# YuliangXiu/ICON

Hardware: AMD Instinct MI355X
Metric: query-points/sec at 256^3 grid (higher is better)
Workload: dtype f32 via 3x f16 split MFMA (22-bit operands, f32 accumulate)

## Files before the change

### icon_amd/_lib.py

```python
from __future__ import annotations

import ctypes as C
import os
import subprocess

_HERE = os.path.dirname(os.path.abspath(__file__))
LIB_PATH = os.environ.get("ICON_AMD_LIB") or os.path.join(_HERE, "libicon_amd.so")
CSRC = os.path.join(_HERE, "csrc")

PRIOR = {"icon": 0, "pamir": 1, "pifu": 2}
CMAP = {"reference": 0, "local": 1}
SEARCH = {"bvh": 0, "brute": 1}
PRECISION = {"f32": 0, "f16x3": 1}

SYMBOLS = [
    "icon_last_error", "icon_version", "icon_device_count",
    "icon_mesh_create", "icon_mesh_destroy", "icon_mesh_vertex_normals", "icon_mesh_stats",
    "icon_mesh_arena_bytes", "icon_mesh_create_arena", "icon_mesh_status", "icon_debug_set_mesh_build", "icon_debug_mesh_layout", "icon_debug_host_mesh_build",
    "icon_sdf_query",
    "icon_feat_create", "icon_feat_destroy", "icon_feat_set_smpl_feats",
    "icon_mlp_create", "icon_mlp_destroy", "icon_mlp_forward", "icon_mlp_set_last_op",
    "icon_work_create", "icon_work_destroy", "icon_work_profile", "icon_work_stage_ms", "icon_work_profile_detail", "icon_work_profile_workgroups", "icon_work_set_steal", "icon_work_set_reserve_cus",
    "icon_query_points", "icon_query_points_dcalib", "icon_query_rows", "icon_grid_rows",
    "icon_volume_any_above", "icon_adaptive_eval", "icon_adaptive_counts", "icon_adaptive_reruns", "icon_grid_eval_slab", "icon_grid_slab_features", "icon_grid_slab_finish", "icon_grid_slab_features_msg",
    "icon_grid_slab_finish_gathered", "icon_debug_set_shell_skip", "icon_debug_set_option", "icon_work_status", "icon_sdf_query_ties", "icon_work_set_tie_rule",
    "icon_export_mesh", "icon_mc_count", "icon_mc_emit", "icon_mc_count_range", "icon_mc_emit_keyed", "icon_debug_traversal_stats", "icon_debug_set_unfused",
    "icon_visibility", "icon_mesh_components", "icon_clean_mesh", "icon_semantic_voxelize",
    "icon_mesh_batch_create", "icon_mesh_batch_destroy", "icon_mesh_batch_status", "icon_feat_create_batch", "icon_query_points_batch",
    "icon_feat_batch_set_volume", "icon_semantic_voxelize_batch",
]

_lib = None


class IconAmdError(RuntimeError):
    pass


def build(force: bool = False) -> str:
    args = ["make", "-j8", "-C", CSRC] + (["-B"] if force else [])
    proc = subprocess.run(args, stdout=subprocess.PIPE, stderr=subprocess.STDOUT, text=True)
    if proc.returncode != 0:
        raise IconAmdError("building libicon_amd.so failed:\n" + proc.stdout[-4000:])
    return LIB_PATH


def lib():
    global _lib
    if _lib is not None:
        return _lib
    if not os.path.exists(LIB_PATH):
        raise IconAmdError(f"{LIB_PATH} not found - run `python -c 'import __graft_entry__ as g; g.build()'` "
                           "or `make -C icon_amd/csrc` (needs hipcc); there is no CPU fallback")
    import torch
    L = C.CDLL(LIB_PATH)
    L.icon_last_error.restype = C.c_char_p
    for name in SYMBOLS:
        if name != "icon_last_error":
            getattr(L, name).restype = C.c_int
    _lib = L
    return L


def check(rc: int, what: str = "") -> None:
    if rc != 0:
        msg = lib().icon_last_error().decode("utf-8", "replace")
        raise IconAmdError(f"{what or 'icon_amd'} failed (code {rc}): {msg}")


def device_count() -> int:
    return int(lib().icon_device_count())


def require_device() -> None:
    if device_count() < 1:
        raise IconAmdError("icon_amd needs a HIP device (MI355X); none is visible and there is no CPU fallback")


def ptr(t) -> C.c_void_p:
    if t is None:
        return C.c_void_p(0)
    if hasattr(t, "data_ptr"):
# ... 4 lines not shown
```

### icon_amd/csrc/adaptive.hip

```cpp
#pragma clang fp contract(off)

#include "geom_device.h"

#include <algorithm>
#include <vector>

constexpr int kAdMaxLevels = 8;

struct icon_adaptive {
    int n_levels = 0;
    int res[kAdMaxLevels] = {0};
    float *occ[kAdMaxLevels] = {nullptr};
    uint8_t *P = nullptr;
    uint8_t *M1 = nullptr;
    uint8_t *D[kAdMaxLevels] = {nullptr};
    int32_t *map = nullptr;
    float *pts = nullptr;
    int32_t *blk_count = nullptr;
    int32_t *blk_list = nullptr;
    int *h_counters = nullptr;
    int *h_counters_dev = nullptr;
    int *counters = nullptr;
    int *counters_base = nullptr;
    int cur_set = 0;
// ... 410 lines not shown
        bk.P = examined ? a->P : nullptr;
        bk.D = (examined && l >= 2) ? a->D[l - 1] : nullptr;
        bk.C = a->M1;
        bk.Dprev = l >= 3 ? a->D[l - 2] : nullptr;
        bk.rpp = l >= 2 ? resolutions[l - 2] : 0;
        bk.balance = balance;
        bk.any_pos = l == 1 ? a->counters + 9 : nullptr;
        bk.zero = examined ? a->blk_count : nullptr;
        bk.n_zero = examined ? nb_l + nsup_l : 0;
        if (l == n_levels - 1) {
            bk.zero_set = other_set;
            a->other_clean = true;
            if (n_levels >= 3 && h_counts) { bk.mirror_src = a->counters; bk.mirror_dst = a->h_counters_dev; mirrored = true; }
        }
        const int64_t book = (bk.P || bk.any_pos) ? (nsrc + 255) / 256 : 0;
        const int64_t grid_up = std::max<int64_t>(std::max<int64_t>(((int64_t)r * r + 3) / 4, book), (bk.n_zero + 255) / 256);
        hipLaunchKernelGGL(k_ad_up, dim3((unsigned)grid_up), dim3(256), 0, st, a->occ[l - 1], rp, a->occ[l], r,
                           examined ? a->counters + 8 : (int *)nullptr, bk);
        if (!examined) break;
        const int rad = l == 1 ? 4 : (l == 2 ? 3 : 1);
        const unsigned nt = (unsigned)((r + kMaskTX - 1) / kMaskTX) * (unsigned)((r + kMaskTY - 1) / kMaskTY) * (unsigned)((r + kMaskTZ - 1) / kMaskTZ);
        uint8_t *C = a->M1;
        const bool icon_prior = prior_type == ICON_PRIOR_ICON;
        const int P = lattice_packet();
        const int shift = P == 4 ? 2 : 1;
        const int nbk = (r + P - 1) / P;
        hipLaunchKernelGGL(k_ad_mask, dim3(nt), dim3(256), 0, st, a->P, rp, (const uint8_t *)(l >= 2 ? a->D[l - 1] : nullptr), C, r, rad,
                           shift, nbk, icon_prior ? a->blk_list : (int32_t *)nullptr, a->counters + 8, a->blk_count, a->blk_count + nb_l);
        hipLaunchKernelGGL(k_ad_scatter, dim3(nbv), dim3(256), 0, st, C, r, a->blk_count, a->blk_count + nb_l, nsup_l, a->map, a->pts, a->counters + l);
        ICON_HIP(hipGetLastError());
        debug_sync("adaptive: upsample + boundary + dilate + compact", st);
        if ((rc = ensure_work_points(work, std::max<int64_t>(n, 1)))) return rc;
        work->q_map = a->map; work->q_n_dev = a->counters + l;
        Calib cal;
        memcpy(cal.m, ident, sizeof(ident)); cal.d = nullptr;
        const bool icon = icon_prior;
        const bool needs_list = icon && cmap_mode == ICON_CMAP_REFERENCE && (feat->dev.smpl_mask & kSmplCmap);
        if (icon) {
            if (mesh->F > kNearLoSlots && work->cap_points_hi < work->cap_points) {
                (void)hipFree(work->d_near_hi); work->d_near_hi = nullptr; work->cap_points_hi = 0;
                ICON_HIP(hipMalloc((void **)&work->d_near_hi, (size_t)work->cap_points));
                work->cap_points_hi = work->cap_points;
            }
            NearRef raw = work_near(work, mesh);
            raw.map = nullptr;
            int n_cu = 0;
            if ((rc = device_cu_count(&n_cu))) return rc;
            const int share_env = share_waves_override();
            const int by_level = r <= 65 ? kShareWavesFew : (r <= 129 ? kShareWavesMany : 4);
            const int nw = (share_env == 1 || share_env == 4 || share_env == 8 || share_env == 16) ? share_env : by_level;
            ShareDbg dbg{};
            if ((rc = work_share_dbg(work, &dbg))) return rc;
#define ICON_AD_NEAREST(PP, NW) hipLaunchKernelGGL((k_ad_nearest<PP, NW>), dim3((unsigned)(n_cu * 32 / (NW == 1 ? 4 : NW))), dim3(NW == 1 ? 256 : NW * 64), 0, st, \
                                                   mesh->dev, r, nbk, a->blk_list, a->counters + 8, C, raw, sdf_clip, dbg)
            if (P == 4 && nw == 16) ICON_AD_NEAREST(4, 16);
            else if (P == 4 && nw == 8) ICON_AD_NEAREST(4, 8);
            else if (P == 4 && nw == 4) ICON_AD_NEAREST(4, 4);
            else if (P == 4) ICON_AD_NEAREST(4, 1);
            else if (nw == 16) ICON_AD_NEAREST(2, 16);
            else if (nw == 8) ICON_AD_NEAREST(2, 8);
            else ICON_AD_NEAREST(2, 1);
#undef ICON_AD_NEAREST
            ICON_HIP(hipGetLastError());
            debug_sync("adaptive: k_ad_nearest", st);
            if ((rc = launch_sign(mesh, cal, r, 0, a->pts, n, sdf_clip, work, false, st))) return rc;
            if (needs_list && (rc = outlier_list_dev(work, a->counters + l, n, st))) return rc;
        }
        FusedSigns fs{};
        fs.mode = needs_list ? kSignSelf : kSignNone;
        fs.list = work->d_signs; fs.k_dev = work->d_total;
        LatticeMap L{};
        rc = launch_fused_f16x3(mesh, feat, mlp, prior_type, cal, L, 0, 0, a->pts, n, sdf_clip, cmap_mode == ICON_CMAP_LOCAL ? 1 : 0, work, fs,
                                a->occ[l], false, st);
        work->q_map = nullptr; work->q_n_dev = nullptr;
        if (rc) return rc;
        debug_sync("adaptive: sign + list + fused", st);
        ICON_HIP(hipGetLastError());
    }
    ICON_HIP(hipGetLastError());
    if (!a->other_clean) {
        ICON_HIP(hipMemsetAsync(other_set, 0, 16 * sizeof(int), st));
        a->other_clean = true;
    }
    if (h_counts) {
        int *host = a->h_counters;
        if (!mirrored) ICON_HIP(hipMemcpyAsync(host, a->counters, 16 * sizeof(int), hipMemcpyDeviceToHost, st));
        ICON_HIP(hipStreamSynchronize(st));
        for (int l = 0; l < n_levels; ++l) h_counts[l] = host[l];
        h_counts[0] = (int64_t)r0 * r0 * r0;
        h_counts[n_levels] = host[9];
        if ((rc = work_check_err(work))) return rc;
    }
    return ICON_OK;
}

extern "C" int icon_adaptive_counts(icon_work_t *work, int n_levels, int64_t *h_counts, void *stream)
{
    ICON_ARG(work && work->ad && h_counts && n_levels == work->ad->n_levels, "icon_adaptive_counts: no matching icon_adaptive_eval on this workspace");
    int *host = work->ad->h_counters;
    ICON_HIP(hipMemcpyAsync(host, work->ad->counters, 16 * sizeof(int), hipMemcpyDeviceToHost, (hipStream_t)stream));
    ICON_HIP(hipStreamSynchronize((hipStream_t)stream));
    for (int l = 0; l < n_levels; ++l) h_counts[l] = host[l];
    h_counts[0] = (int64_t)work->ad->res[0] * work->ad->res[0] * work->ad->res[0];
    h_counts[n_levels] = host[9];
    return work_check_err(work);
}
```

### icon_amd/csrc/batch_query.hip

```cpp
#pragma clang fp contract(off)

#include "batch_device.h"

#include <algorithm>

namespace icon {

constexpr int kBatchBlock = 256;
constexpr int kBatchChecked = 0x100;

__global__ void k_pack_planes_batch(const float *__restrict__ src, int C, int H, int W, int n_select, int csel, int cpad, int64_t stride,
                                    float *__restrict__ dst)
{
    const int64_t n = (int64_t)n_select * H * W * cpad;
    const float *s = src + (int64_t)blockIdx.z * C * H * W;
    float *d = dst + (int64_t)blockIdx.z * stride;
    for (int64_t i = (int64_t)blockIdx.x * blockDim.x + threadIdx.x; i < n; i += (int64_t)gridDim.x * blockDim.x) {
        const int c = (int)(i % cpad);
        const int64_t pix = (i / cpad) % ((int64_t)H * W);
        const int sel = (int)(i / ((int64_t)cpad * H * W));
        d[i] = (c < csel) ? s[((int64_t)(sel * csel + c)) * H * W + pix] : 0.0f;
    }
}

// ... 130 lines not shown
        if (f.smpl_mask & kSmplNorm) { row[hh] = o.nrm.x; row[hh + 1] = o.nrm.y; row[hh + 2] = o.nrm.z; }
    } else {
        gather_planes_dyn(f, 0, p.x, p.y, g);
        const int h = f.csel;
        for (int k = 0; k < h; ++k) row[k] = g[k];
        if (PRIOR == ICON_PRIOR_PAMIR) {
            float v[8];
            if (f.vpad == 8) gather_volume<2>(f, p.x, p.y, p.z, v); else gather_volume<1>(f, p.x, p.y, p.z, v);
            for (int k = 0; k < f.Cv; ++k) row[h + k] = v[k];
        } else {
            row[h] = p.z;
        }
    }
    row[kCodeSlot] = __int_as_float((int)code);
    if (live) { store_row(X, i, row); code8[i] = (uint8_t)code; }
}

}

using namespace icon;

extern "C" int icon_mesh_batch_destroy(icon_mesh_batch_t *mb)
{
    if (!mb) return ICON_OK;
    if (mb->done) (void)hipEventDestroy(mb->done);
    (void)hipFree(mb->d_table);
    if (mb->h_table) (void)hipHostFree(mb->h_table);
    if (mb->h_status) (void)hipHostFree(mb->h_status);
    delete mb;
    return ICON_OK;
}

extern "C" int icon_mesh_batch_create(const icon_mesh_t *const *meshes, int B, void *stream, icon_mesh_batch_t **out)
{
    ICON_ARG(out != nullptr, "icon_mesh_batch_create: out is null");
    *out = nullptr;
    ICON_ARG(meshes != nullptr && B >= 1, "icon_mesh_batch_create: no meshes");
    for (int b = 0; b < B; ++b) {
        ICON_ARG(meshes[b] != nullptr, "icon_mesh_batch_create: a mesh is null");
        ICON_ARG(meshes[b]->V == meshes[0]->V && meshes[b]->F == meshes[0]->F,
                 "icon_mesh_batch_create: the subjects' vertex / face counts differ (check_sign takes subject 0's faces for every subject, "
                 "lib/dataset/mesh_util.py:393)");
    }
    hipStream_t st = (hipStream_t)stream;
    icon_mesh_batch *mb = new icon_mesh_batch();
    mb->B = B; mb->V = meshes[0]->V; mb->F = meshes[0]->F;
    for (int b = 0; b < B; ++b) { mb->subj.push_back(meshes[b]); mb->depth_bound = std::max(mb->depth_bound, meshes[b]->depth_bound); }
    const size_t tab_bytes = (size_t)B * sizeof(MeshDev), bytes = tab_bytes + sizeof(int);
    hipError_t e = hipMalloc((void **)&mb->d_table, bytes);
    if (e == hipSuccess) e = hipHostMalloc((void **)&mb->h_table, bytes, hipHostMallocPortable);
    if (e == hipSuccess) e = hipHostMalloc((void **)&mb->h_status, sizeof(int), hipHostMallocPortable);
    if (e == hipSuccess) e = hipEventCreateWithFlags(&mb->done, hipEventDisableTiming);
    if (e != hipSuccess) { icon_mesh_batch_destroy(mb); return fail(ICON_ERR_HIP, std::string("icon_mesh_batch_create: ") + hipGetErrorString(e)); }
    for (int b = 0; b < B; ++b) mb->h_table[b] = meshes[b]->dev;
    int *h_word = reinterpret_cast<int *>(reinterpret_cast<char *>(mb->h_table) + tab_bytes);
    int *d_word = reinterpret_cast<int *>(reinterpret_cast<char *>(mb->d_table) + tab_bytes);
    *h_word = kBatchChecked;
    *(volatile int *)mb->h_status = 0;
    e = hipMemcpyAsync(mb->d_table, mb->h_table, bytes, hipMemcpyHostToDevice, st);
    if (e == hipSuccess && B > 1 && mb->F > 0) {
        const int64_t n = (int64_t)(B - 1) * mb->F;
        hipLaunchKernelGGL(k_faces_match, dim3((unsigned)((n + kBatchBlock - 1) / kBatchBlock)), dim3(kBatchBlock), 0, st, mb->d_table, B, mb->F, d_word);
        e = hipGetLastError();
    }
    if (e == hipSuccess) e = hipMemcpyAsync(mb->h_status, d_word, sizeof(int), hipMemcpyDeviceToHost, st);
    if (e == hipSuccess) e = hipEventRecord(mb->done, st);
    if (e != hipSuccess) { icon_mesh_batch_destroy(mb); return fail(ICON_ERR_HIP, std::string("icon_mesh_batch_create: ") + hipGetErrorString(e)); }
    *out = mb;
    return ICON_OK;
}

extern "C" int icon_mesh_batch_status(const icon_mesh_batch_t *mb, int wait, int *bits)
{
    ICON_ARG(mb != nullptr, "icon_mesh_batch_status: batch is null");
    if (wait) ICON_HIP(hipEventSynchronize(mb->done));
    const int st = *reinterpret_cast<const volatile int *>(mb->h_status);
    if (!(st & kBatchChecked)) { if (bits) *bits = -1; return ICON_OK; }
    if (bits) *bits = st & ~kBatchChecked;
    if (st & ICON_MESH_BATCH_FACES_DIFFER)
        return fail(ICON_ERR_ARG, "icon_mesh_batch: the subjects' faces differ - check_sign(verts, faces[0], points) (lib/dataset/mesh_util.py:393) "
                                  "tests every subject against subject 0's faces; bind subjects of one topology");
    return ICON_OK;
}

extern "C" int icon_feat_create_batch(const float *d_planes, int B, int C, int H, int W, int n_select, void *stream, icon_feat_t **out)
{
    ICON_ARG(out != nullptr, "icon_feat_create_batch: out is null");
    *out = nullptr;
    ICON_ARG(d_planes && B >= 1 && C > 0 && H > 1 && W > 1, "icon_feat_create_batch: bad planes");
    ICON_ARG(n_select == 1 || n_select == 2, "icon_feat_create_batch: n_select must be 1 or 2");
    ICON_ARG(C % n_select == 0, "icon_feat_create_batch: C not divisible by n_select");
    ICON_ARG(B <= 65535, "icon_feat_create_batch: more than 65,535 subjects");
    const int csel = C / n_select;
    const int cpad = (csel + 3) & ~3;
    if (cpad > 16) return fail(ICON_ERR_UNSUPPORTED, "icon_feat_create_batch: more than 16 channels per tap");
    hipStream_t st = (hipStream_t)stream;
    icon_feat *f = new icon_feat();
    const int64_t stride = (int64_t)n_select * H * W * cpad;
    hipError_t e = hipMalloc((void **)&f->d_planes, (size_t)stride * B * sizeof(float));
    if (e != hipSuccess) { delete f; return fail(ICON_ERR_HIP, std::string("hipMalloc planes: ") + hipGetErrorString(e)); }
    hipLaunchKernelGGL(k_pack_planes_batch, dim3((unsigned)std::max(1, 1024 / B), 1, (unsigned)B), dim3(256), 0, st, d_planes, C, H, W, n_select,
                       csel, cpad, stride, f->d_planes);
    FeatDev &d = f->dev;
    d.planes = f->d_planes; d.C = C; d.H = H; d.W = W; d.n_select = n_select; d.csel = csel; d.cpad = cpad;
    d.smpl_mask = kSmplCmap | kSmplNorm;
    d.vol = nullptr; d.Cv = 0; d.Dv = d.Hv = d.Wv = 0; d.vpad = 0;
    f->batch = B; f->plane_stride = stride;
// ... 131 lines not shown
```

### icon_amd/csrc/common.h

```cpp
#pragma once
#include <hip/hip_runtime.h>
#include <stdint.h>
#include <functional>
#include <string>
#include <vector>

#include "../../include/icon_amd.h"

namespace icon {
constexpr int kWgRec = 6;
constexpr int kMaxProfGrid = 1024;

void set_error(const std::string &msg);
int fail(int code, const std::string &msg);

#define ICON_HIP(expr)                                                                          \
    do {                                                                                        \
        hipError_t _e = (expr);                                                                 \
        if (_e != hipSuccess)                                                                   \
            return ::icon::fail(ICON_ERR_HIP, std::string(#expr) + ": " + hipGetErrorString(_e)); \
    } while (0)

#define ICON_ARG(cond, msg)                                                  \
    do {                                                                     \
        if (!(cond)) return ::icon::fail(ICON_ERR_ARG, std::string(msg));    \
    } while (0)

struct alignas(64) BvhNode {
    float lo[3][2], hi[3][2];
    int32_t child0, child1;
    int32_t pad[2];
};
static_assert(sizeof(BvhNode) == 64, "BvhNode must be 64 bytes");

struct alignas(16) TriRec {
    float a[3], b[3], c[3];
    int32_t ia, ib, ic;
};
static_assert(sizeof(TriRec) == 48, "TriRec must be 48 bytes");

struct alignas(16) TriAttr {
    float n[3][3];
    float cm[3][3];
    float vis[3];
    int32_t face;
    int32_t pad[2];
};
static_assert(sizeof(TriAttr) == 96, "TriAttr must be 96 bytes");

struct alignas(32) TriPre {
    float a[3], b[3], ab[3], ac[3], bc[3];
    float i00, i11, ibc, a00, a01, a11, inn;
    int32_t face;
    int32_t pad;
};
static_assert(sizeof(TriPre) == 96, "TriPre must be 96 bytes");

struct alignas(32) LeafRec {
    float pair[2][24][2];
};
static_assert(sizeof(LeafRec) == 384, "LeafRec must be 384 bytes");

constexpr int kLeafMax = 4;
constexpr int kShareWavesMany = 8, kShareWavesFew = 16;
inline int share_waves(int64_t packets) { return packets <= 1500 ? kShareWavesFew : (packets <= 8000 ? kShareWavesMany : 1); }
constexpr int kStackDepth = 48;
constexpr int kXRow = 16;
constexpr int kCodeSlot = 15;

constexpr uint32_t kCodeOutlier = 1u;
constexpr uint32_t kCodeSignShift = 1;
constexpr uint32_t kCodeInCube = 8u;
constexpr uint32_t kCodeInside = 16u;

constexpr int kScanBlock = 256;
constexpr int kMaxWorld = 64;

struct MeshDyn {
    int32_t root;
    int32_t gy, gz;
    float bin_y0, bin_z0, bin_y1, bin_z1, bin_inv_y, bin_inv_z;
    float box_lo[3], box_hi[3];
    int32_t n_nodes, n_leaves, depth, bin_entries, max_bin;
    int32_t status;
    int32_t pad[11];
};
static_assert(sizeof(MeshDyn) == 128, "MeshDyn layout");
constexpr int kMeshBadFace = 1;
constexpr int kMeshBadVertex = 2;
constexpr int kMeshBinOverflow = 4;
constexpr int kMeshInternal = 8;
constexpr int kMeshBuilt = 0x100;

struct MeshDev {
    const BvhNode *nodes;
    const TriRec *tris;
    const TriAttr *attr;
    const int32_t *slot2face;
    const int32_t *face2slot;
    const LeafRec *leaves;
    const MeshDyn *dyn;
    int32_t n_tris;
    const int32_t *bin_start;
    const int32_t *bin_slots;
};

struct FeatDev {
    const float *planes;
    const float *vol;
    int32_t C, H, W, n_select, csel, cpad;
    int32_t Cv, Dv, Hv, Wv, vpad;
    int32_t smpl_mask;
};
constexpr int kSmplCmap = 1, kSmplNorm = 2;

struct Calib { float m[12]; const float *d; };

struct Lattice {
    int32_t res, z0, z1;
};

struct LatticeMap {
    int res, z0, nz;
    int tx, ty, tz;
    int remap;
    int off;
    int zs, nzi;
    int sx0, sx1, sy0, sy1;
    int sz0, sz1;
    int trim;
    float trim_need;
    int pk;
};

__device__ __forceinline__ bool not_finite(float y)
{
    uint32_t u = __float_as_uint(y);
    asm volatile("" : "+v"(u));
    return (u & 0x7f800000u) == 0x7f800000u;
}

__device__ __forceinline__ float apply_last_op(float y, int last_op)
{
    return last_op == ICON_LASTOP_SIGMOID ? 1.0f / (1.0f + expf(-y)) : y;
}

struct NearRef { uint16_t *lo; uint8_t *hi; float *d2; const int32_t *map; };

enum { kSignNone = 0, kSignSelf = 1, kSignGlobal = 2, kSignSeg = 3 };
struct FusedSigns {
    int mode;
    const int8_t *list;
    const int64_t *k_dev;
// ... 64 lines not shown
namespace icon {
void parallel_for(int n, const std::function<void(int)> &fn);
void debug_sync(const char *what, hipStream_t st);
struct MeshLayout;
int mesh_host_state_get(MeshDyn **h, hipEvent_t *ev);
void mesh_host_state_put(MeshDyn *h, hipEvent_t ev);
void mesh_bind_arena(icon_mesh *m, const MeshLayout &L);
int mesh_build_device(icon_mesh *m, const float *d_verts, const int64_t *d_faces, const float *d_cmap, const float *d_vis, hipStream_t st);
void adaptive_destroy(icon_adaptive *a);
inline int lattice_packet()
{
    static const int pk_env = getenv("ICON_AMD_PACKET") ? atoi(getenv("ICON_AMD_PACKET")) : 0;
    return pk_env == 2 ? 2 : 4;
}
int outlier_list_dev(icon_work *w, const int *n_dev, int64_t n_max, hipStream_t st);
int ensure_work_points(icon_work *w, int64_t n_points);
struct McDevState;
void mc_destroy(McDevState *s);
struct CleanState;
void clean_destroy(CleanState *s);
int morton_order(icon_work *w, const float *d_points, const float *calib12, const float *d_calib12, int64_t N, hipStream_t st, const int32_t **perm);
int mlp_launch(const icon_mlp *mlp, const float *d_x, int64_t N, float *d_out, int precision, hipStream_t st);
int mlp_launch_ex(const icon_mlp *mlp, const float *d_x, int64_t N, float *d_out, bool mask, hipStream_t st);
int mlp_rescue_rows(const icon_mlp *mlp, const float *d_x, int64_t N, float *d_out, hipStream_t st);
int mlp_flag_reset(const icon_mlp *mlp, hipStream_t st);
int rescue_always();
int mlp_pack_f16x3(icon_mlp *m, const std::vector<std::vector<float>> &W, const std::vector<std::vector<float>> &B, hipStream_t st);
int mlp_launch_f16x3(const icon_mlp *mlp, const float *d_x, int64_t N, float *d_out, bool mask, hipStream_t st);
uint16_t f32_to_f16_rtn(float f);
float f16_to_f32(uint16_t h);
float pick_scale(const std::vector<float> &W);
int launch_sign(const icon_mesh *mesh, const Calib &cal, int res, int z0, const float *d_points, int64_t N, float sdf_clip,
                const icon_work *work, bool lattice, hipStream_t st);
int launch_fused_f16x3(const icon_mesh *mesh, const icon_feat *feat, const icon_mlp *mlp, int prior, const Calib &cal,
                       const LatticeMap &L, int za, int zb, const float *d_points, int64_t N, float sdf_clip, int cmap_local,
                       const icon_work *work, const FusedSigns &fs, float *d_occ, bool lattice, hipStream_t st,
                       const BatchDev *bd = nullptr);
int morton_order_batch(icon_work *w, const float *d_points, const float *d_calibs, int64_t n, int B, hipStream_t st, const int32_t **perm);
int ensure_work_rows(icon_work *w, int64_t n_points, bool need_x);
int outlier_list_counted(icon_work *w, int64_t N, hipStream_t st);
int patch_self_rows(icon_work *w, int64_t N, int cmap_slot, hipStream_t st);
bool fused_path(int precision, int search);
void work_mark(icon_work *w, int k, hipStream_t st);
int device_cu_count(int *n_cu);
int once_per_device(int kernel_id, const std::function<hipError_t()> &set);
struct LatticeFast;
struct ShareDbg {
    int *err;
    int ring, lose, spin_log2;
};
int work_share_dbg(icon_work *w, ShareDbg *out);
int work_check_err(icon_work *w);
int share_waves_override();
}

struct icon_work {
    float *d_x = nullptr;
    int64_t cap_x = 0;
    uint16_t *d_near16 = nullptr;
    uint8_t *d_near_hi = nullptr;
    float *d_near_d2 = nullptr;
    int64_t cap_points_hi = 0;
    uint8_t *d_code8 = nullptr;
    int64_t cap_points = 0;
    uint64_t *d_grp_mask = nullptr;
    int32_t *d_block_counts = nullptr;
    int64_t *d_block_offsets = nullptr;
    int32_t *d_scan_local = nullptr;
    int64_t *d_scan_part = nullptr;
    int64_t cap_blocks = 0;
    int8_t *d_signs = nullptr;
    int64_t cap_signs = 0;
    int64_t *d_total = nullptr;
    int *d_flag = nullptr;
    mutable bool flag_clean = false;
    int64_t *d_seg = nullptr;
    int32_t *d_row_count = nullptr;
    int32_t *d_row_slots = nullptr;
    int64_t cap_rows = 0;
    int *h_err = nullptr;
    icon::LatticeFast *d_lfast = nullptr;
    uint32_t *d_sort_keys = nullptr;
    int32_t *d_sort_idx = nullptr;
    void *d_sort_tmp = nullptr;
    size_t sort_tmp_bytes = 0;
    int64_t cap_sort = 0;
    int slab_res = 0, slab_z0 = 0, slab_z1 = 0, slab_c0 = 0, slab_cmap_slot = 0;
    bool slab_ready = false, slab_needs_patch = false, slab_patched = false;
    int tie_rule = 0, tie_ulps = 0;
    const icon_mesh *q_mesh = nullptr;
    const icon_feat *q_feat = nullptr;
    int q_prior = 0, q_cmap_mode = 0, q_search = 0;
    float q_sdf_clip = 0.f;
    icon::Calib q_cal{};
    icon::LatticeMap q_L{};
    const float *q_points = nullptr;
    int64_t q_N = 0;
    bool q_lattice = false, q_rows_ready = false;
    const int32_t *q_map = nullptr;
    const int *q_n_dev = nullptr;
    int reserve_cus = 0;
    int *h_any = nullptr;
    int *defer_range_flag = nullptr;
    int range_reruns = 0;
    struct icon_adaptive *ad = nullptr;
    icon::McDevState *mc = nullptr;
    icon::CleanState *clean = nullptr;
    bool prof = false;
    hipEvent_t ev[6] = {nullptr, nullptr, nullptr, nullptr, nullptr, nullptr};
    bool ev_search = false;
    unsigned long long *d_clock = nullptr;
    mutable int clock_grid = 0;
    double clock_kernel_ms = 0.0;
    unsigned int *d_steal = nullptr;
    int steal_permille = 150, steal_grp = 2;
    bool ev_valid = false;
};

namespace icon {
constexpr int kNearLoSlots = 32768;
inline NearRef work_near(const icon_work *w, const icon_mesh *mesh)
{
    NearRef r;
    r.lo = w->d_near16; r.d2 = w->d_near_d2;
    r.hi = (mesh && mesh->F > kNearLoSlots) ? w->d_near_hi : nullptr;
    r.map = w->q_map;
    return r;
}
}
```

### icon_amd/csrc/fused_f16x3.hip

```cpp
#pragma clang fp contract(off)

#include "geom_device.h"
#include "batch_device.h"
#include "mlp_f16x3_device.h"
#include "mlp_plain_device.h"

#include <algorithm>
#include <mutex>

namespace icon {

constexpr int kTilePts = kF16Pts;
constexpr int kXsOff = kSideOff + 4352;
constexpr int kFusedLds = kXsOff + kTilePts * kXRow * 4;

struct SignSrc {
    int mode;
    const int8_t *list;
    const int64_t *k_dev;
    int64_t k_host, rank_offset;
    const int8_t *gathered;
    int64_t stride;
    int world, rank;
    const int64_t *seg;
// ... 646 lines not shown
            }
            const float y = mlp_plain_wave(P, s, lane);
            if (lane == b) out[o] = y;
            __builtin_amdgcn_wave_barrier();
        }
    }
}

template <int PRIOR>
__global__ __launch_bounds__(64) void k_rescue_fused_batch(FusedGeom G, float *__restrict__ out, MlpPlain P, const int *flag, int always, BatchDev bd)
{
    __shared__ float s[kPlainLds];
    if (!always && *flag == 0) return;
    const int lane = threadIdx.x;
    int64_t K = 0, rank0 = 0;
    if (PRIOR == ICON_PRIOR_ICON) sign_list_extent(G, K, rank0);
    for (int64_t base = (int64_t)blockIdx.x * 64; base < G.N; base += (int64_t)gridDim.x * 64) {
        const int64_t q = base + lane;
        const int64_t o = q < G.N ? q : 0;
        const float v = q < G.N ? out[o] : 0.0f;
        unsigned long long todo = __ballot(not_finite(v));
        while (todo) {
            const int b = __ffsll((long long)todo) - 1;
            todo &= todo - 1;
            if (lane == b) {
                float row[kXRow];
#pragma unroll
                for (int k = 0; k < kXRow; ++k) row[k] = 0.0f;
                build_row_batch<PRIOR>(G, bd, q, row, K, rank0);
#pragma unroll
                for (int k = 0; k < kXRow; ++k) s[k] = k < P.c0 ? row[k] : 0.0f;
            }
            const float y = mlp_plain_wave(P, s, lane);
            if (lane == b) out[o] = y;
            __builtin_amdgcn_wave_barrier();
        }
    }
}

__global__ void k_seg_offsets(const int8_t *__restrict__ gathered, int64_t stride, int world, int64_t *__restrict__ seg)
{
    if (threadIdx.x != 0 || blockIdx.x != 0) return;
    int64_t a = 0;
    for (int r = 0; r < world; ++r) { seg[r] = a; a += *reinterpret_cast<const int64_t *>(gathered + (int64_t)r * stride); }
    seg[world] = a;
}

int launch_sign(const icon_mesh *mesh, const Calib &cal, int res, int z0, const float *d_points, int64_t N, float sdf_clip,
                const icon_work *work, bool lattice, hipStream_t st)
{
    const int64_t nb = (N + 255) / 256;
    ICON_ARG(nb > 0 && nb < (1ll << 31), "too many workgroups for one launch");
    const float far_box2 = far_box_dist2(sdf_clip);
    if (lattice) hipLaunchKernelGGL(k_sign<true>, dim3((unsigned)nb), dim3(256), 0, st, mesh->dev, cal, res, z0, d_points, N, sdf_clip,
                                    work->d_row_count, work->d_row_slots, work_near(work, mesh), work->d_code8, work->d_block_counts,
                                    (unsigned long long *)work->d_grp_mask, far_box2, (const int *)nullptr, work->d_flag);
    else if (work->q_n_dev || N <= 262144)
        hipLaunchKernelGGL(k_sign_wide, dim3((unsigned)nb), dim3(1024), 0, st, mesh->dev, cal, d_points, N, sdf_clip, work_near(work, mesh), work->d_code8,
                           work->d_block_counts, (unsigned long long *)work->d_grp_mask, far_box2, work->q_n_dev, work->d_flag);
    else hipLaunchKernelGGL(k_sign<false>, dim3((unsigned)nb), dim3(256), 0, st, mesh->dev, cal, res, z0, d_points, N, sdf_clip,
                            (const int32_t *)nullptr, (const int32_t *)nullptr, work_near(work, mesh), work->d_code8, work->d_block_counts,
                            (unsigned long long *)work->d_grp_mask, far_box2, work->q_n_dev, work->d_flag);
    ICON_HIP(hipGetLastError());
    work->flag_clean = work->d_flag != nullptr;
    return ICON_OK;
}

namespace {
constexpr int kMaxDevices = 64, kMaxKernelIds = 16;
std::mutex g_dev_mutex;
int g_n_cu[kMaxDevices];
bool g_attr_set[kMaxKernelIds][kMaxDevices];
}

int device_cu_count(int *n_cu)
{
    int dev = 0;
    ICON_HIP(hipGetDevice(&dev));
    ICON_ARG(dev >= 0 && dev < kMaxDevices, "device index out of range");
    std::lock_guard<std::mutex> lk(g_dev_mutex);
    if (!g_n_cu[dev]) {
        int n = 0;
        ICON_HIP(hipDeviceGetAttribute(&n, hipDeviceAttributeMultiprocessorCount, dev));
        g_n_cu[dev] = n > 0 ? n : 256;
    }
    *n_cu = g_n_cu[dev];
    return ICON_OK;
}

int once_per_device(int kernel_id, const std::function<hipError_t()> &set)
{
    int dev = 0;
    if (hipGetDevice(&dev) != hipSuccess || dev < 0 || dev >= kMaxDevices || kernel_id < 0 || kernel_id >= kMaxKernelIds) {
        const hipError_t e = set();
        return e == hipSuccess ? ICON_OK : fail(ICON_ERR_HIP, std::string("hipFuncSetAttribute: ") + hipGetErrorString(e));
    }
    std::lock_guard<std::mutex> lk(g_dev_mutex);
    if (g_attr_set[kernel_id][dev]) return ICON_OK;
    const hipError_t e = set();
    if (e != hipSuccess) return fail(ICON_ERR_HIP, std::string("hipFuncSetAttribute: ") + hipGetErrorString(e));
    g_attr_set[kernel_id][dev] = true;
    return ICON_OK;
}

int launch_fused_f16x3(const icon_mesh *mesh, const icon_feat *feat, const icon_mlp *mlp, int prior, const Calib &cal,
                       const LatticeMap &L, int za, int zb, const float *d_points, int64_t N, float sdf_clip, int cmap_local,
                       const icon_work *work, const FusedSigns &fs, float *d_occ, bool lattice, hipStream_t st, const BatchDev *bd)
{
    FusedGeom G{};
    if (mesh) G.m = mesh->dev;
    G.f = feat->dev; G.cal = cal; G.pts = d_points; G.sdf_clip = sdf_clip; G.cmap_local = cmap_local;
    if (lattice) {
        const int zs = std::max(za, L.off), ze = std::min(zb, L.res - L.off);
        if (L.off) {
            const int64_t rows = (int64_t)(zb - za) * L.res;
            const int row_wgs = (int)((rows + 255) / 256);
            const int64_t face_rows = 2 * (int64_t)(zb - za) + (int64_t)((za == 0 ? 1 : 0) + (zb == L.res ? 1 : 0)) * L.res;
            if (rows > 0) hipLaunchKernelGGL(k_shell_zero, dim3((unsigned)(row_wgs + (face_rows + 3) / 4)), dim3(256), 0, st, d_occ, L.res, L.z0, za, zb, row_wgs);
        }
        G.res = L.res; G.z0 = L.z0; G.off = L.off; G.nx = L.res - 2 * L.off; G.zs = zs;
        N = (ze > zs) ? (int64_t)(ze - zs) * G.nx * G.nx : 0;
    }
    if (N <= 0) { ICON_HIP(hipGetLastError()); return ICON_OK; }
    ICON_ARG(N < (1ll << 31), "fused: more than 2^31 points in one call");
    G.N = N;
    G.near = work_near(work, mesh); G.code8 = work->d_code8;
    if (!lattice) { G.n_dev = work->q_n_dev; G.out_map = work->q_map; }
    G.clock = work->prof ? work->d_clock : nullptr;
    G.steal = nullptr; G.steal_static = 0; G.steal_grp = 1; G.steal_ngrp = 0;
    G.block_offsets = work->d_block_offsets; G.grp_mask = (const unsigned long long *)work->d_grp_mask;
    G.sg.mode = fs.mode; G.sg.list = fs.list; G.sg.k_dev = fs.k_dev; G.sg.k_host = fs.k_host; G.sg.rank_offset = fs.rank_offset;
    G.sg.gathered = fs.gathered; G.sg.stride = fs.stride; G.sg.world = fs.world; G.sg.rank = fs.rank; G.sg.seg = nullptr;
    if (fs.mode == kSignSeg) {
        if (!work->d_seg) return fail(ICON_ERR_STATE, "fused: segment offsets buffer missing");
        hipLaunchKernelGGL(k_seg_offsets, dim3(1), dim3(64), 0, st, fs.gathered, fs.stride, fs.world, work->d_seg);
        G.sg.seg = work->d_seg;
    }
    MlpF16Dev w;
    w.image = mlp->d_f16;
    w.side = reinterpret_cast<const float *>(mlp->d_f16 + kImageBytes);
    w.b3 = mlp->b3; w.inv0 = mlp->f16_inv[0]; w.inv1 = mlp->f16_inv[1]; w.inv2 = mlp->f16_inv[2]; w.c0 = mlp->c0; w.last_op = mlp->last_op;
    w.p0 = 0.505f * w.inv0; w.q0 = 0.495f * w.inv0; w.p1 = 0.505f * w.inv1; w.q1 = 0.495f * w.inv1; w.p2 = 0.505f * w.inv2; w.q2 = 0.495f * w.inv2;
    w.flag = work->d_flag ? work->d_flag : reinterpret_cast<int *>(mlp->d_blob + mlp->off_flag);
    const bool defer = work->defer_range_flag != nullptr;
    if (defer) w.flag = work->defer_range_flag;

    int n_cu = 0;
    int rc = device_cu_count(&n_cu);
    if (rc) return rc;
    if (defer) {}
    else if (work->d_flag) { if (!work->flag_clean) ICON_HIP(hipMemsetAsync(work->d_flag, 0, sizeof(int), st)); }
    else if ((rc = mlp_flag_reset(mlp, st))) return rc;
    work->flag_clean = false;
    const MlpPlain plain = mlp_plain_of(mlp);
    const int64_t n_resc = std::min<int64_t>((N + 63) / 64, 2048);
    const bool small = prior == ICON_PRIOR_ICON && (work->q_n_dev != nullptr || N <= 262144);
    const int64_t ntiles = small ? (N + kTilePts / 2 - 1) / (kTilePts / 2) : (N + kTilePts - 1) / kTilePts;
    const unsigned grid = (unsigned)std::min<int64_t>(ntiles, std::max(n_cu - work->reserve_cus, 1));
    {
        const int per = (int)(ntiles / grid);
        const int pool_len = (int)((int64_t)per * work->steal_permille / 1000);
        if (!small && work->d_steal && pool_len > 0 && ntiles > (int64_t)grid) {
            G.steal = work->d_steal; G.steal_grp = std::min(work->steal_grp, kMaxStealGroup);
// ... 44 lines not shown
```

### icon_amd/csrc/geom_device.h

```cpp
#pragma once
#pragma clang fp contract(off)

#include "common.h"
#include "mesh_rules.h"

#include <cstdlib>
#include <cstring>

namespace icon {

struct f3 { float x, y, z; };
__device__ __forceinline__ f3 mk3(float x, float y, float z) { f3 r; r.x = x; r.y = y; r.z = z; return r; }
__device__ __forceinline__ f3 sub3(f3 a, f3 b) { return mk3(a.x - b.x, a.y - b.y, a.z - b.z); }
__device__ __forceinline__ float dot3(f3 a, f3 b) { return fmaf(a.z, b.z, fmaf(a.y, b.y, a.x * b.x)); }
__device__ __forceinline__ f3 cross3(f3 a, f3 b)
{
    return mk3(fmaf(a.y, b.z, -(a.z * b.y)), fmaf(a.z, b.x, -(a.x * b.z)), fmaf(a.x, b.y, -(a.y * b.x)));
}

struct TriC {
    f3 a, b, ab, ac, bc;
    float i00, i11, ibc, a00, a01, a11, inn;
};

// ... 2 lines not shown
    const float t = fminf(fmaxf(dot_e_po * inv_len2, 0.0f), 1.0f);
    const f3 d = mk3(fmaf(-t, e.x, po.x), fmaf(-t, e.y, po.y), fmaf(-t, e.z, po.z));
    return dot3(d, d);
}

__device__ __forceinline__ float tri_dist2(f3 p, const TriC &t)
{
    const f3 ap = sub3(p, t.a), bp = sub3(p, t.b);
    const float d1 = dot3(t.ab, ap), d2 = dot3(t.ac, ap), d3 = dot3(t.bc, bp);
    const float s = fmaf(t.a11, d1, -(t.a01 * d2)) * t.inn;
    const float u = fmaf(t.a00, d2, -(t.a01 * d1)) * t.inn;
    const bool inside = (s >= 0.0f) & (u >= 0.0f) & (s + u <= 1.0f);
    const f3 df = mk3(fmaf(-u, t.ac.x, fmaf(-s, t.ab.x, ap.x)), fmaf(-u, t.ac.y, fmaf(-s, t.ab.y, ap.y)),
                      fmaf(-u, t.ac.z, fmaf(-s, t.ab.z, ap.z)));
    float d_face = dot3(df, df);
    const float e0 = seg_dist2(ap, t.ab, d1, t.i00);
    const float e1 = seg_dist2(ap, t.ac, d2, t.i11);
    const float e2 = seg_dist2(bp, t.bc, d3, t.ibc);
    float d_edge = fminf(fminf(e0, e1), e2);
    asm volatile("" : "+v"(d_face), "+v"(d_edge));
    return inside ? d_face : d_edge;
}

template <class Ptr>
__device__ __forceinline__ TriC load_tric(Ptr q)
{
    TriC t;
    t.a = mk3(q[0], q[1], q[2]); t.b = mk3(q[3], q[4], q[5]); t.ab = mk3(q[6], q[7], q[8]);
    t.ac = mk3(q[9], q[10], q[11]); t.bc = mk3(q[12], q[13], q[14]);
    t.i00 = q[15]; t.i11 = q[16]; t.ibc = q[17]; t.a00 = q[18]; t.a01 = q[19]; t.a11 = q[20]; t.inn = q[21];
    return t;
}

typedef float f2 __attribute__((ext_vector_type(2)));
typedef __attribute__((address_space(4))) const f2 cf2;
struct f3x2 { f2 x, y, z; };
__device__ __forceinline__ f2 bc2(float v) { f2 r; r.x = v; r.y = v; return r; }
__device__ __forceinline__ f2 fma2(f2 a, f2 b, f2 c) { return __builtin_elementwise_fma(a, b, c); }
__device__ __forceinline__ f3x2 sub3x2(f3x2 a, f3x2 b) { f3x2 r; r.x = a.x - b.x; r.y = a.y - b.y; r.z = a.z - b.z; return r; }
__device__ __forceinline__ f2 dot3x2(f3x2 a, f3x2 b) { return fma2(a.z, b.z, fma2(a.y, b.y, a.x * b.x)); }
__device__ __forceinline__ f2 clamp01x2(f2 v)
{
    f2 r; r.x = fminf(fmaxf(v.x, 0.0f), 1.0f); r.y = fminf(fmaxf(v.y, 0.0f), 1.0f); return r;
}
__device__ __forceinline__ f2 seg_dist2x2(f3x2 po, f3x2 e, f2 dot_e_po, f2 inv_len2)
{
    f2 t;
    asm("v_pk_mul_f32 %0, %1, %2 clamp" : "=v"(t) : "v"(dot_e_po), "s"(inv_len2));
    const f2 nt = -t;
    f3x2 d; d.x = fma2(nt, e.x, po.x); d.y = fma2(nt, e.y, po.y); d.z = fma2(nt, e.z, po.z);
    return dot3x2(d, d);
}

__device__ __forceinline__ f2 tri_dist2_pair(f3 p1, cf2 *q)
{
    f3x2 p; p.x = bc2(p1.x); p.y = bc2(p1.y); p.z = bc2(p1.z);
    f3x2 a, b, ab, ac, bc;
    a.x = q[0]; a.y = q[1]; a.z = q[2]; b.x = q[3]; b.y = q[4]; b.z = q[5];
    ab.x = q[6]; ab.y = q[7]; ab.z = q[8]; ac.x = q[9]; ac.y = q[10]; ac.z = q[11]; bc.x = q[12]; bc.y = q[13]; bc.z = q[14];
    const f2 i00 = q[15], i11 = q[16], ibc = q[17], a00 = q[18], a01 = q[19], a11 = q[20], inn = q[21];
    const f3x2 ap = sub3x2(p, a), bp = sub3x2(p, b);
    const f2 d1 = dot3x2(ab, ap), d2 = dot3x2(ac, ap), d3 = dot3x2(bc, bp);
    const f2 s = fma2(a11, d1, -(a01 * d2)) * inn;
    const f2 u = fma2(a00, d2, -(a01 * d1)) * inn;
    const f2 su = s + u;
    const bool in0 = (s.x >= 0.0f) & (u.x >= 0.0f) & (su.x <= 1.0f);
    const bool in1 = (s.y >= 0.0f) & (u.y >= 0.0f) & (su.y <= 1.0f);
    const f2 e0 = seg_dist2x2(ap, ab, d1, i00);
    const f2 e1 = seg_dist2x2(ap, ac, d2, i11);
    const f2 e2 = seg_dist2x2(bp, bc, d3, ibc);
    f2 r; r.x = fminf(fminf(e0.x, e1.x), e2.x); r.y = fminf(fminf(e0.y, e1.y), e2.y);
    if (__any(in0 | in1)) {
        const f2 ns = -s, nu = -u;
        f3x2 df; df.x = fma2(nu, ac.x, fma2(ns, ab.x, ap.x)); df.y = fma2(nu, ac.y, fma2(ns, ab.y, ap.y)); df.z = fma2(nu, ac.z, fma2(ns, ab.z, ap.z));
        const f2 d_face = dot3x2(df, df);
        float f0 = d_face.x, f1 = d_face.y, g0 = r.x, g1 = r.y;
        asm volatile("" : "+v"(f0), "+v"(f1), "+v"(g0), "+v"(g1));
        r.x = in0 ? f0 : g0; r.y = in1 ? f1 : g1;
    }
    return r;
}

__device__ __forceinline__ float edge_fn(float yi, float zi, float yj, float zj, float qy, float qz)
{
    const float t1 = (yi - qy) * (zj - qz);
    return fmaf(-(zi - qz), (yj - qy), t1);
}
__device__ __forceinline__ bool edge_side(float yi, float zi, float yj, float zj, float e)
{
    if (e > 0.0f) return true;
    if (e < 0.0f) return false;
    const float dz = zj - zi, dy = yj - yi;
    if (dz != 0.0f) return dz < 0.0f;
    return dy > 0.0f;
}
__device__ __forceinline__ void oriented_edge(int ia, f3 a, int ib, f3 b, float qy, float qz, float &val, bool &pos)
{
    if (ia < ib) { const float e = edge_fn(a.y, a.z, b.y, b.z, qy, qz); val = e; pos = edge_side(a.y, a.z, b.y, b.z, e); }
    else         { const float e = edge_fn(b.y, b.z, a.y, a.z, qy, qz); val = -e; pos = !edge_side(b.y, b.z, a.y, a.z, e); }
}
__device__ __forceinline__ int ray_hit(f3 p, f3 a, f3 b, f3 c, int ia, int ib, int ic)
{
    float e_ab, e_bc, e_ca; bool s_ab, s_bc, s_ca;
    oriented_edge(ia, a, ib, b, p.y, p.z, e_ab, s_ab);
    oriented_edge(ib, b, ic, c, p.y, p.z, e_bc, s_bc);
    oriented_edge(ic, c, ia, a, p.y, p.z, e_ca, s_ca);
    if (!(s_ab == s_bc && s_bc == s_ca)) return 0;
    const float num = fmaf(e_ab, c.x - p.x, fmaf(e_ca, b.x - p.x, e_bc * (a.x - p.x)));
    return s_ab ? (num > 0.0f) : (num < 0.0f);
}

typedef __attribute__((address_space(4))) const float cfloat;
__device__ __forceinline__ cfloat *as_const(const void *p) { return (cfloat *)(uintptr_t)p; }

__device__ __forceinline__ void load_tri_pos_uniform(const TriRec *t, f3 &a, f3 &b, f3 &c)
// ... 10 lines not shown
    a = mk3(q0.x, q0.y, q0.z); b = mk3(q0.w, q1.x, q1.y); c = mk3(q1.z, q1.w, q2);
}
__device__ __forceinline__ void load_tri_full(const TriRec *t, f3 &a, f3 &b, f3 &c, int &ia, int &ib, int &ic)
{
    const float4 *q = reinterpret_cast<const float4 *>(t);
    const float4 q0 = q[0], q1 = q[1], q2 = q[2];
    a = mk3(q0.x, q0.y, q0.z); b = mk3(q0.w, q1.x, q1.y); c = mk3(q1.z, q1.w, q2.x);
    ia = __float_as_int(q2.y); ib = __float_as_int(q2.z); ic = __float_as_int(q2.w);
}

__host__ __device__ inline float far_box_dist2(float sdf_clip)
{
    const float cb = (sdf_clip > 0.0f ? sdf_clip : 0.0f) * 1.7320508f;
    return cb * cb * 1.0001f + 1e-6f;
}

__device__ __forceinline__ float box_dist2(float lx, float ly, float lz, float hx, float hy, float hz, f3 p)
{
    const float dx = fmaxf(fmaxf(lx - p.x, p.x - hx), 0.0f);
    const float dy = fmaxf(fmaxf(ly - p.y, p.y - hy), 0.0f);
    const float dz = fmaxf(fmaxf(lz - p.z, p.z - hz), 0.0f);
    return fmaf(dz, dz, fmaf(dy, dy, dx * dx));
}

__device__ __forceinline__ f2 box_dist2_pair(cf2 *q, f3 p)
{
    const f2 px = bc2(p.x), py = bc2(p.y), pz = bc2(p.z);
    const f2 ax = q[0] - px, bx = px - q[3];
    const f2 ay = q[1] - py, by = py - q[4];
    const f2 az = q[2] - pz, bz = pz - q[5];
    f2 dx, dy, dz;
    dx.x = fmaxf(fmaxf(ax.x, bx.x), 0.0f); dx.y = fmaxf(fmaxf(ax.y, bx.y), 0.0f);
    dy.x = fmaxf(fmaxf(ay.x, by.x), 0.0f); dy.y = fmaxf(fmaxf(ay.y, by.y), 0.0f);
    dz.x = fmaxf(fmaxf(az.x, bz.x), 0.0f); dz.y = fmaxf(fmaxf(az.y, bz.y), 0.0f);
    return fma2(dz, dz, fma2(dy, dy, dx * dx));
}

struct Nearest { float d2; int slot; int face; };

__device__ __forceinline__ int mesh_root(const MeshDev &m)
{
    return __builtin_amdgcn_readfirstlane(*reinterpret_cast<__attribute__((address_space(4))) const int *>((uintptr_t)&m.dyn->root));
}

__device__ __forceinline__ float prune_threshold(float best)
{
    return fmaf(best, 1.000083f, 2.1e-7f);
}

template <bool STATS = false, bool TIES = false>
__device__ __forceinline__ Nearest nearest_packet(const MeshDev &m, f3 p, bool live, int *wstack ,
                                                  int *n_nodes = nullptr, int *n_tris = nullptr, float thr0 = INFINITY,
                                                  unsigned long long *runner_up = nullptr, int center_lane = 21,
                                                  bool have_root = false, int root = 0)
{
    Nearest nr; nr.d2 = INFINITY; nr.slot = 0; nr.face = 0x7fffffff;
    unsigned long long key = 0x7f8000007fffffffull;
    unsigned long long key2 = 0x7f8000007fffffffull;
    float thr = live ? thr0 : -INFINITY;
    int sp = 0;
    int cur = have_root ? root : mesh_root(m);
    while (true) {
        if (cur < 0) {
            const int code = ~cur;
            const int leaf = code >> 2, cnt = (code & 3) + 1;
            if (STATS) *n_tris += cnt;
            const int npairs = __builtin_amdgcn_readfirstlane((cnt + 1) >> 1);
            for (int pr = 0; pr < npairs; ++pr) {
                cf2 *q = reinterpret_cast<cf2 *>(as_const(&m.leaves[leaf].pair[pr]));
                const f2 d2 = tri_dist2_pair(p, q);
                const f2 fc = q[22];
                const unsigned long long k0 = ((unsigned long long)(unsigned)__float_as_int(d2.x) << 32) | (unsigned)__float_as_int(fc.x);
                const unsigned long long k1 = ((unsigned long long)(unsigned)__float_as_int(d2.y) << 32) | (unsigned)__float_as_int(fc.y);
                if (TIES) {
                    if (k0 < key) { key2 = key; key = k0; } else if (k0 != key && k0 < key2) key2 = k0;
                    if (k1 < key) { key2 = key; key = k1; } else if (k1 != key && k1 < key2) key2 = k1;
                } else {
                    key = (k0 < key) ? k0 : key;
                    key = (k1 < key) ? k1 : key;
                }
            }
            nr.d2 = __int_as_float((int)(key >> 32));
            thr = live ? prune_threshold(nr.d2) : thr;
            if (sp == 0) break;
            cur = __builtin_amdgcn_readfirstlane(wstack[--sp]);
        } else {
            if (STATS) ++*n_nodes;
            cf2 *q = reinterpret_cast<cf2 *>(as_const(m.nodes + cur));
            const f2 dd = box_dist2_pair(q, p);
            const float d0 = dd.x, d1 = dd.y;
            const f2 ids = q[6];
            const int c0 = __float_as_int(ids.x), c1 = __float_as_int(ids.y);
            const bool v0 = __any(d0 <= thr), v1 = __any(d1 <= thr);
            if (v0 && v1) {
                const int e0 = __builtin_amdgcn_readlane(__float_as_int(d0), center_lane);
                const int e1 = __builtin_amdgcn_readlane(__float_as_int(d1), center_lane);
                const bool first0 = e0 <= e1;
                wstack[sp++] = first0 ? c1 : c0;
                cur = first0 ? c0 : c1;
            } else if (v0) cur = c0;
            else if (v1) cur = c1;
            else {
                if (sp == 0) break;
                cur = __builtin_amdgcn_readfirstlane(wstack[--sp]);
            }
        }
    }
    nr.d2 = __int_as_float((int)(key >> 32)); nr.face = (int)(key & 0xffffffffu);
    nr.slot = (nr.face != 0x7fffffff) ? m.face2slot[nr.face] : 0;
    if (TIES) *runner_up = key2;
    return nr;
}

constexpr int kRing = 64, kRingEmpty = 0x7fffffff;
constexpr int kShareSpinLog2 = 18;
constexpr int kShareErrPop = 1;
constexpr int kShareErrPush = 2;
constexpr int kShareErrIdle = 3;
struct ShareLds {
    unsigned thr[64];
    int head, tail, avail, active;
    int mask, lose, spins, pad1;
    int pad[8];
// ... 58 lines not shown
    }
    return __builtin_amdgcn_readfirstlane(ok) != 0;
}

template <int NW>
__device__ __forceinline__ Nearest nearest_shared(const MeshDev &m, f3 p, bool live, int *wstack, char *smem , int center_lane,
                                                  const ShareDbg &dbg)
{
    ShareLds &S = *reinterpret_cast<ShareLds *>(smem);
    const int lane = threadIdx.x & 63, wave = threadIdx.x >> 6;
    __syncthreads();
    if (threadIdx.x < 64) { S.thr[lane] = 0x7f800000u; S.ring[lane] = lane == 0 ? mesh_root(m) : kRingEmpty; }
    if (threadIdx.x == 0) {
        S.head = 0; S.tail = 1; S.avail = 1; S.active = NW;
        S.mask = (dbg.ring >= 2 && dbg.ring <= kRing ? dbg.ring : kRing) - 1;
        S.lose = dbg.lose > 0 ? dbg.lose : -1;
        S.spins = 1 << (dbg.spin_log2 > 0 && dbg.spin_log2 < 30 ? dbg.spin_log2 : kShareSpinLog2);
    }
    __syncthreads();
    unsigned long long key = 0x7f8000007fffffffull;
    float thr = live ? INFINITY : -INFINITY;
    int sp = 0;
    while (true) {
        int cur;
        if (sp > 0) cur = __builtin_amdgcn_readfirstlane(wstack[--sp]);
        else {
            cur = share_pop(S, lane, dbg);
            if (cur == kRingEmpty) {
                if (lane == 0) atomicSub(&S.active, 1);
                int spins = 0;
                while (true) {
                    const int av = __builtin_amdgcn_readfirstlane(*(volatile int *)&S.avail);
                    const int ac = __builtin_amdgcn_readfirstlane(*(volatile int *)&S.active);
                    if (av > 0) {
                        if (lane == 0) atomicAdd(&S.active, 1);
                        cur = share_pop(S, lane, dbg);
                        if (cur != kRingEmpty) break;
                        if (lane == 0) atomicSub(&S.active, 1);
                    } else if (ac <= 0) break;
                    if (++spins > (4 << kShareSpinLog2)) { if (lane == 0) share_report(dbg, kShareErrIdle, spins, S); break; }
                    __builtin_amdgcn_s_sleep(2);
                }
                if (cur == kRingEmpty) break;
            }
            thr = live ? prune_threshold(__uint_as_float(S.thr[lane])) : thr;
        }
        while (true) {
            if (cur < 0) {
                const int code = ~cur;
                const int leaf = code >> 2, cnt = (code & 3) + 1;
                const int npairs = __builtin_amdgcn_readfirstlane((cnt + 1) >> 1);
                for (int pr = 0; pr < npairs; ++pr) {
                    cf2 *q = reinterpret_cast<cf2 *>(as_const(&m.leaves[leaf].pair[pr]));
                    const f2 d2 = tri_dist2_pair(p, q);
                    const f2 fc = q[22];
                    const unsigned long long k0 = ((unsigned long long)(unsigned)__float_as_int(d2.x) << 32) | (unsigned)__float_as_int(fc.x);
                    const unsigned long long k1 = ((unsigned long long)(unsigned)__float_as_int(d2.y) << 32) | (unsigned)__float_as_int(fc.y);
                    key = (k0 < key) ? k0 : key;
                    key = (k1 < key) ? k1 : key;
                }
                const unsigned mine = (unsigned)(key >> 32);
                const unsigned old = atomicMin(&S.thr[lane], mine);
                thr = live ? prune_threshold(__uint_as_float(min(old, mine))) : thr;
                break;
            }
            cf2 *q = reinterpret_cast<cf2 *>(as_const(m.nodes + cur));
            const f2 dd = box_dist2_pair(q, p);
            const float d0 = dd.x, d1 = dd.y;
            const f2 ids = q[6];
            const int c0 = __float_as_int(ids.x), c1 = __float_as_int(ids.y);
            const bool v0 = __any(d0 <= thr), v1 = __any(d1 <= thr);
            if (v0 && v1) {
                const int e0 = __builtin_amdgcn_readlane(__float_as_int(d0), center_lane);
                const int e1 = __builtin_amdgcn_readlane(__float_as_int(d1), center_lane);
                const bool first0 = e0 <= e1;
                const int far = first0 ? c1 : c0;
                const int av = __builtin_amdgcn_readfirstlane(*(volatile int *)&S.avail);
                if (av >= NW || !share_push(S, lane, far, dbg)) wstack[sp++] = far;
                cur = first0 ? c0 : c1;
            } else if (v0) cur = c0;
            else if (v1) cur = c1;
            else break;
        }
    }
    S.keys[wave * 64 + lane] = key;
    __syncthreads();
    Nearest nr; nr.d2 = INFINITY; nr.slot = 0; nr.face = 0x7fffffff;
    if (wave == 0) {
#pragma unroll
        for (int w = 1; w < NW; ++w) { const unsigned long long k = S.keys[w * 64 + lane]; key = (k < key) ? k : key; }
        nr.d2 = __int_as_float((int)(key >> 32)); nr.face = (int)(key & 0xffffffffu);
        nr.slot = (nr.face != 0x7fffffff) ? m.face2slot[nr.face] : 0;
    }
    return nr;
}

__device__ __forceinline__ Nearest nearest_packet_alt(const MeshDev &m, f3 p, bool live, int *wstack, uint32_t best_bits, uint32_t ulps)
{
    const float thr = live ? prune_threshold(__int_as_float((int)best_bits)) : -INFINITY;
    const uint32_t lim = best_bits + ulps;
    int face = -1;
    uint32_t fbits = best_bits;
    int sp = 0, cur = mesh_root(m);
    while (true) {
        if (cur < 0) {
            const int code = ~cur;
            const int leaf = code >> 2, cnt = (code & 3) + 1;
            const int npairs = __builtin_amdgcn_readfirstlane((cnt + 1) >> 1);
            for (int pr = 0; pr < npairs; ++pr) {
                cf2 *q = reinterpret_cast<cf2 *>(as_const(&m.leaves[leaf].pair[pr]));
                const f2 d2 = tri_dist2_pair(p, q);
                const f2 fc = q[22];
                const uint32_t b0 = (uint32_t)__float_as_int(d2.x), b1 = (uint32_t)__float_as_int(d2.y);
                const int f0 = __float_as_int(fc.x), f1 = __float_as_int(fc.y);
                if (b0 <= lim && f0 > face) { face = f0; fbits = b0; }
                if (b1 <= lim && f1 > face) { face = f1; fbits = b1; }
            }
            if (sp == 0) break;
            cur = __builtin_amdgcn_readfirstlane(wstack[--sp]);
        } else {
            cf2 *q = reinterpret_cast<cf2 *>(as_const(m.nodes + cur));
            const f2 dd = box_dist2_pair(q, p);
            const f2 ids = q[6];
            const int c0 = __float_as_int(ids.x), c1 = __float_as_int(ids.y);
            const bool v0 = __any(dd.x <= thr), v1 = __any(dd.y <= thr);
            if (v0 && v1) { wstack[sp++] = c1; cur = c0; }
            else if (v0) cur = c0;
            else if (v1) cur = c1;
            else {
                if (sp == 0) break;
                cur = __builtin_amdgcn_readfirstlane(wstack[--sp]);
            }
        }
    }
    Nearest nr;
    nr.face = face >= 0 ? face : 0x7fffffff;
    nr.d2 = __int_as_float((int)fbits);
    nr.slot = face >= 0 ? m.face2slot[face] : 0;
    return nr;
}

constexpr int64_t kPacketMinPoints = 98304;
constexpr int kCoopWaves = 4;
constexpr int kCoopLeaves = 256;
struct CoopLds {
    int *frontier; int cap;
    int *leaf_ref; float *leaf_d;
    unsigned long long *best; int *best_slot;
};
__host__ __device__ inline int coop_cap(int depth) { return 64 * (depth + 3); }
__host__ __device__ inline size_t coop_wave_bytes(int cap) { return (size_t)cap * 4 + kCoopLeaves * 8 + 16; }
__device__ __forceinline__ CoopLds coop_lds(char *smem, int wave, int cap)
{
    char *b = smem + (size_t)wave * coop_wave_bytes(cap);
    CoopLds S;
    S.best = reinterpret_cast<unsigned long long *>(b);
    S.best_slot = reinterpret_cast<int *>(b + 8);
    S.leaf_ref = reinterpret_cast<int *>(b + 16);
    S.leaf_d = reinterpret_cast<float *>(b + 16 + kCoopLeaves * 4);
    S.frontier = reinterpret_cast<int *>(b + 16 + kCoopLeaves * 8);
    S.cap = cap;
    return S;
}

__device__ __forceinline__ Nearest nearest_coop(const MeshDev &m, f3 p, const CoopLds &S)
{
    const int lane = threadIdx.x & 63;
    const unsigned long long lt_mask = (lane == 0) ? 0ull : (~0ull >> (64 - lane));
    unsigned long long key = 0x7f8000007fffffffull;
    int slot = 0;
    auto tri_key = [&](int leaf, int t, int cnt, int &out_slot) -> unsigned long long {
        if (t >= cnt) return 0x7f8000007fffffffull;
        const float *q = reinterpret_cast<const float *>(m.leaves + leaf) + (t >> 1) * 48 + (t & 1);
        TriC tc;
        tc.a = mk3(q[0], q[2], q[4]); tc.b = mk3(q[6], q[8], q[10]); tc.ab = mk3(q[12], q[14], q[16]);
        tc.ac = mk3(q[18], q[20], q[22]); tc.bc = mk3(q[24], q[26], q[28]);
        tc.i00 = q[30]; tc.i11 = q[32]; tc.ibc = q[34]; tc.a00 = q[36]; tc.a01 = q[38]; tc.a11 = q[40]; tc.inn = q[42];
        const float d2 = tri_dist2(p, tc);
        out_slot = leaf + t;
        return ((unsigned long long)(unsigned)__float_as_int(d2) << 32) | (unsigned)__float_as_int(q[44]);
    };
    auto wave_min = [&](unsigned long long k, int sl) {
        if (lane == 0) { *reinterpret_cast<volatile unsigned long long *>(S.best) = key; *reinterpret_cast<volatile int *>(S.best_slot) = slot; }
        __builtin_amdgcn_wave_barrier();
        if (k < key) atomicMin(S.best, k);
        __builtin_amdgcn_wave_barrier();
        const unsigned long long b = *reinterpret_cast<volatile unsigned long long *>(S.best);
        if (k == b && b != key) *reinterpret_cast<volatile int *>(S.best_slot) = sl;
        __builtin_amdgcn_wave_barrier();
        if (b != key) { key = b; slot = *reinterpret_cast<volatile int *>(S.best_slot); }
        __builtin_amdgcn_wave_barrier();
    };

    const int root = mesh_root(m);
    int cur = root;
    while (cur >= 0) {
        const float4 *q4 = reinterpret_cast<const float4 *>(m.nodes + cur);
        const float4 n0 = q4[0], n1 = q4[1], n2 = q4[2];
        const float2 ids = *reinterpret_cast<const float2 *>(reinterpret_cast<const float *>(m.nodes + cur) + 12);
        const float d0 = box_dist2(n0.x, n0.z, n1.x, n1.z, n2.x, n2.z, p);
        const float d1 = box_dist2(n0.y, n0.w, n1.y, n1.w, n2.y, n2.w, p);
        cur = __builtin_amdgcn_readfirstlane(d0 <= d1 ? __float_as_int(ids.x) : __float_as_int(ids.y));
    }
    {
        const int code = ~cur, leaf = code >> 2, cnt = (code & 3) + 1;
        int sl = 0;
        const unsigned long long k = tri_key(leaf, lane & 3, cnt, sl);
        wave_min(k, sl);
    }
    float thr = prune_threshold(__int_as_float((int)(key >> 32)));

    int nf = root >= 0 ? 1 : 0, nl = 0;
    if (lane == 0) S.frontier[0] = root;
    __builtin_amdgcn_wave_barrier();
    while (nf > 0 || nl > 0) {
        if (nl >= 16 || nf == 0) {
            const int take = min(nl, 16);
            const int e = nl - take + (lane >> 2);
            unsigned long long k = 0x7f8000007fffffffull;
            int sl = 0;
            if ((lane >> 2) < take) {
                const int code = ~reinterpret_cast<volatile int *>(S.leaf_ref)[e];
                if (reinterpret_cast<volatile float *>(S.leaf_d)[e] <= thr) k = tri_key(code >> 2, lane & 3, (code & 3) + 1, sl);
            }
            nl -= take;
            const unsigned long long before = key;
            wave_min(k, sl);
            if (key != before) thr = prune_threshold(__int_as_float((int)(key >> 32)));
            continue;
        }
        const int take = min(min(nf, 64), min(S.cap - nf, (kCoopLeaves - nl) / 2));
        const int e = nf - take + lane;
        bool v0 = false, v1 = false;
        int c0 = 0, c1 = 0;
        float d0 = 0.f, d1 = 0.f;
        if (lane < take) {
            const int node = reinterpret_cast<volatile int *>(S.frontier)[e];
            const float4 *q4 = reinterpret_cast<const float4 *>(m.nodes + node);
            const float4 n0 = q4[0], n1 = q4[1], n2 = q4[2];
            const float2 ids = *reinterpret_cast<const float2 *>(reinterpret_cast<const float *>(m.nodes + node) + 12);
            d0 = box_dist2(n0.x, n0.z, n1.x, n1.z, n2.x, n2.z, p);
            d1 = box_dist2(n0.y, n0.w, n1.y, n1.w, n2.y, n2.w, p);
            c0 = __float_as_int(ids.x); c1 = __float_as_int(ids.y);
            v0 = d0 <= thr; v1 = d1 <= thr;
        }
        nf -= take;
        __builtin_amdgcn_wave_barrier();
        const unsigned long long bi0 = __ballot(v0 && c0 >= 0), bi1 = __ballot(v1 && c1 >= 0);
        const unsigned long long bl0 = __ballot(v0 && c0 < 0), bl1 = __ballot(v1 && c1 < 0);
        if (v0 && c0 >= 0) S.frontier[nf + __popcll(bi0 & lt_mask)] = c0;
        if (v1 && c1 >= 0) S.frontier[nf + __popcll(bi0) + __popcll(bi1 & lt_mask)] = c1;
        if (v0 && c0 < 0) { const int o = nl + __popcll(bl0 & lt_mask); S.leaf_ref[o] = c0; S.leaf_d[o] = d0; }
        if (v1 && c1 < 0) { const int o = nl + __popcll(bl0) + __popcll(bl1 & lt_mask); S.leaf_ref[o] = c1; S.leaf_d[o] = d1; }
        nf += __popcll(bi0) + __popcll(bi1);
        nl += __popcll(bl0) + __popcll(bl1);
        __builtin_amdgcn_wave_barrier();
    }
    Nearest nr;
    nr.d2 = __int_as_float((int)(key >> 32)); nr.slot = slot; nr.face = (int)(key & 0xffffffffu);
    return nr;
}

constexpr int kBruteTile = 128;
template <int BLOCK>
__device__ __forceinline__ Nearest nearest_brute(const MeshDev &m, f3 p, float *tile )
{
    Nearest nr; nr.d2 = INFINITY; nr.slot = 0; nr.face = 0x7fffffff;
    for (int base = 0; base < m.n_tris; base += kBruteTile) {
        __syncthreads();
        const int n = min(kBruteTile, m.n_tris - base);
        for (int k = threadIdx.x; k < n; k += BLOCK) {
            const TriRec &tr = m.tris[base + k];
            TriPre pre;
            tri_setup(tr.a, tr.b, tr.c, m.slot2face[base + k], pre);
            const float *src = reinterpret_cast<const float *>(&pre);
            for (int fld = 0; fld < 24; ++fld) tile[k * 24 + fld] = src[fld];
// ... 415 lines not shown
```

### icon_amd/csrc/mesh_build.cpp

```cpp
#include <algorithm>
#include <chrono>
#include <cmath>
#include <cstdio>
#include <cstdlib>
#include <cstring>
#include <limits>
#include <atomic>
#include <condition_variable>
#include <mutex>
#include <numeric>
#include <thread>

#include "common.h"
#include "mesh_rules.h"

namespace icon {

static thread_local std::string g_err;
void set_error(const std::string &msg) { g_err = msg; }
int fail(int code, const std::string &msg) { g_err = msg; return code; }
const char *last_error_cstr() { return g_err.c_str(); }

void debug_sync(const char *what, hipStream_t st)
{
// ... 144 lines not shown
                    for (int k = 0; k < 3; ++k) {
                        bb[b][k] = fminf(bb[b][k], tbox[6 * (size_t)e + k]); bb[b][3 + k] = fmaxf(bb[b][3 + k], tbox[6 * (size_t)e + 3 + k]);
                        bc[b][k] = fminf(bc[b][k], cen[3 * (size_t)e + k]); bc[b][3 + k] = fmaxf(bc[b][3 + k], cen[3 * (size_t)e + k]);
                    }
                }
                for (int b = 0; b < kSahBins - 1; ++b) {
                    float sb[2][6], sc[2][6];
                    int c2[2] = {0, 0};
                    for (int s = 0; s < 2; ++s)
                        for (int k = 0; k < 3; ++k) { sb[s][k] = INFINITY; sb[s][3 + k] = -INFINITY; sc[s][k] = INFINITY; sc[s][3 + k] = -INFINITY; }
                    for (int q = 0; q < kSahBins; ++q) {
                        if (!cnt[q]) continue;
                        const int s = q <= b ? 0 : 1;
                        c2[s] += cnt[q];
                        for (int k = 0; k < 3; ++k) {
                            sb[s][k] = fminf(sb[s][k], bb[q][k]); sb[s][3 + k] = fmaxf(sb[s][3 + k], bb[q][3 + k]);
                            sc[s][k] = fminf(sc[s][k], bc[q][k]); sc[s][3 + k] = fmaxf(sc[s][3 + k], bc[q][3 + k]);
                        }
                    }
                    if (!c2[0] || !c2[1]) continue;
                    const double cost = box_area(sb[0], sb[0] + 3) * c2[0] + box_area(sb[1], sb[1] + 3) * c2[1];
                    if (cost < best) {
                        best = cost; valid = true; best_axis = ax; best_bin = b; nleft = c2[0];
                        memcpy(cbox, sb, sizeof(sb)); memcpy(ccb, sc, sizeof(sc));
                    }
                }
            }
        }
        if (valid) {
            int l = begin, r = 0;
            for (int i = begin; i < end; ++i) {
                const int e = order[i];
                if (sah_bin(cen[3 * (size_t)e + best_axis], lo[best_axis], ext[best_axis]) <= best_bin) order[l++] = e; else tmp[r++] = e;
            }
            for (int i = 0; i < r; ++i) order[l + i] = tmp[i];
        } else {
            nleft = n / 2;
            bounds(begin, begin + nleft, cbox[0], ccb[0]);
            bounds(begin + nleft, end, cbox[1], ccb[1]);
        }
        const int mid = begin + nleft, id = mid - 1;
        link(parent, side, id, box);
        dyn.n_nodes++;
        build(begin, mid, depth + 1, id, 0, cbox[0], ccb[0]);
        build(mid, end, depth + 1, id, 1, cbox[1], ccb[1]);
    }
};

struct HostArrays {
    MeshDyn dyn{};
    std::vector<float> vn;
    std::vector<BvhNode> nodes;
    std::vector<LeafRec> leafrec;
    std::vector<TriRec> tris;
    std::vector<TriAttr> attr;
    std::vector<int32_t> order, face2slot, bin_start, bin_slots;
};

int host_build(const std::vector<float> &verts, const std::vector<int64_t> &faces, const std::vector<float> &cmap, const std::vector<float> &vis,
               int64_t V, int64_t F, int bound, HostArrays &out)
{
    for (int64_t i = 0; i < 3 * F; ++i)
        ICON_ARG(faces[i] >= 0 && faces[i] < V, "icon_mesh_create: face index out of range");
    for (int64_t i = 0; i < 3 * V; ++i)
        ICON_ARG(!bad_coord(verts[i]), "icon_mesh_create: non-finite (or absurdly large) vertex coordinate");
    HostBuild hb;
    hb.V = V; hb.F = F; hb.bound = bound;

    std::vector<float> &vn = out.vn;
    vn.assign(3 * V, 0.f);
    for (int64_t f = 0; f < F; ++f) {
        const int64_t id[3] = {faces[3 * f], faces[3 * f + 1], faces[3 * f + 2]};
        const V3 a{verts[3 * id[0]], verts[3 * id[0] + 1], verts[3 * id[0] + 2]};
        const V3 b{verts[3 * id[1]], verts[3 * id[1] + 1], verts[3 * id[1] + 2]};
        const V3 c{verts[3 * id[2]], verts[3 * id[2] + 1], verts[3 * id[2] + 2]};
        const V3 n = cross(sub(b, a), sub(c, a));
        for (int k = 0; k < 3; ++k) { vn[3 * id[k]] += n.x; vn[3 * id[k] + 1] += n.y; vn[3 * id[k] + 2] += n.z; }
    }
    for (int64_t v = 0; v < V; ++v) {
        const float x = vn[3 * v], y = vn[3 * v + 1], z = vn[3 * v + 2];
        float len = sqrtf(fmaf(z, z, fmaf(y, y, x * x)));
        if (len < 1e-6f) len = 1e-6f;
        vn[3 * v] = x / len; vn[3 * v + 1] = y / len; vn[3 * v + 2] = z / len;
    }

    hb.tbox.resize(6 * F); hb.cen.resize(3 * F); hb.order.resize(F); hb.tmp.resize(F);
    hb.nodes.assign(F, BvhNode{}); hb.leaf_cnt.assign(F, 0);
    std::iota(hb.order.begin(), hb.order.end(), 0);
    float box[6], cb[6];
    for (int64_t f = 0; f < F; ++f)
        for (int a = 0; a < 3; ++a) {
            const float p0 = verts[3 * faces[3 * f] + a], p1 = verts[3 * faces[3 * f + 1] + a], p2 = verts[3 * faces[3 * f + 2] + a];
            const float lo = canon(fminf(fminf(p0, p1), p2)), hi = canon(fmaxf(fmaxf(p0, p1), p2));
            hb.tbox[6 * f + a] = lo; hb.tbox[6 * f + 3 + a] = hi; hb.cen[3 * f + a] = canon(0.5f * (lo + hi));
        }
    hb.bounds(0, (int)F, box, cb);
    hb.build(0, (int)F, 0, -1, 0, box, cb);
    MeshDyn &dyn = hb.dyn;
    for (int a = 0; a < 3; ++a) { dyn.box_lo[a] = box[a]; dyn.box_hi[a] = box[3 + a]; }
    const BinGrid g = bin_grid(dyn.box_lo, dyn.box_hi, F);
    dyn.gy = g.gy; dyn.gz = g.gz; dyn.bin_y0 = g.y0; dyn.bin_z0 = g.z0; dyn.bin_y1 = g.y1; dyn.bin_z1 = g.z1; dyn.bin_inv_y = g.inv_y; dyn.bin_inv_z = g.inv_z;

    const std::vector<int32_t> &order = hb.order;
    std::vector<TriRec> &tris = out.tris;
    std::vector<TriAttr> &attr = out.attr;
    std::vector<int32_t> &face2slot = out.face2slot;
    std::vector<LeafRec> &leafrec = out.leafrec;
    tris.resize(F); attr.resize(F); face2slot.resize(F); leafrec.resize(F);
    memset((void *)leafrec.data(), 0, sizeof(LeafRec) * F);
    for (int64_t p = 0; p < F; ++p) {
        const int64_t f = order[p];
        const int64_t id[3] = {faces[3 * f], faces[3 * f + 1], faces[3 * f + 2]};
        TriRec &tr = tris[p];
        for (int k = 0; k < 3; ++k) { tr.a[k] = verts[3 * id[0] + k]; tr.b[k] = verts[3 * id[1] + k]; tr.c[k] = verts[3 * id[2] + k]; }
        tr.ia = (int32_t)id[0]; tr.ib = (int32_t)id[1]; tr.ic = (int32_t)id[2];
        TriAttr &a = attr[p];
        for (int c = 0; c < 3; ++c) {
            for (int k = 0; k < 3; ++k) { a.n[c][k] = vn[3 * id[c] + k]; a.cm[c][k] = cmap[3 * id[c] + k]; }
            a.vis[c] = vis[id[c]];
        }
        a.face = (int32_t)f; a.pad[0] = a.pad[1] = 0;
        face2slot[f] = (int32_t)p;
    }
    for (int64_t L = 0; L < F; ++L) {
        const int cnt = hb.leaf_cnt[L];
        for (int t = 0; t < (cnt ? kLeafMax : 0); ++t) {
            const int64_t p = L + std::min(t, cnt - 1);
            TriPre pre;
            tri_setup(tris[p].a, tris[p].b, tris[p].c, order[p], pre);
            const float *src = reinterpret_cast<const float *>(&pre);
            for (int fld = 0; fld < 24; ++fld) leafrec[L].pair[t >> 1][fld][t & 1] = src[fld];
        }
    }

    const int64_t n_cells = (int64_t)g.gy * g.gz;
    std::vector<int32_t> &bin_start = out.bin_start;
    std::vector<int32_t> &bin_slots = out.bin_slots;
    bin_start.assign(n_cells + 1, 0);
    auto range = [&](int64_t p, int &cy0, int &cy1, int &cz0, int &cz1) {
        const float *tb = &hb.tbox[6 * (size_t)order[p]];
        cy0 = bin_cell_of(tb[1] - kBinEps, g.y0, g.inv_y, g.gy); cy1 = bin_cell_of(tb[4] + kBinEps, g.y0, g.inv_y, g.gy);
        cz0 = bin_cell_of(tb[2] - kBinEps, g.z0, g.inv_z, g.gz); cz1 = bin_cell_of(tb[5] + kBinEps, g.z0, g.inv_z, g.gz);
    };
    for (int64_t p = 0; p < F; ++p) {
        int cy0, cy1, cz0, cz1; range(p, cy0, cy1, cz0, cz1);
        for (int cz = cz0; cz <= cz1; ++cz)
            for (int cy = cy0; cy <= cy1; ++cy) bin_start[(size_t)cz * g.gy + cy + 1]++;
    }
    int64_t max_bin = 0, total = 0;
    for (int64_t i = 1; i <= n_cells; ++i) { max_bin = std::max<int64_t>(max_bin, bin_start[i]); total += bin_start[i]; }
    bin_slots.clear();
    if (total <= bin_entries_cap(F)) {
        for (int64_t i = 1; i <= n_cells; ++i) bin_start[i] += bin_start[i - 1];
        bin_slots.resize(total);
        std::vector<int32_t> fill(bin_start.begin(), bin_start.end() - 1);
        for (int64_t p = 0; p < F; ++p) {
            int cy0, cy1, cz0, cz1; range(p, cy0, cy1, cz0, cz1);
            for (int cz = cz0; cz <= cz1; ++cz)
                for (int cy = cy0; cy <= cy1; ++cy) bin_slots[fill[(size_t)cz * g.gy + cy]++] = (int32_t)p;
        }
        dyn.bin_entries = (int32_t)total; dyn.max_bin = (int32_t)max_bin;
    } else {
        std::fill(bin_start.begin(), bin_start.end(), 0);
        dyn.gy = dyn.gz = 0; dyn.status |= kMeshBinOverflow;
    }
    dyn.status |= kMeshBuilt;
    out.dyn = dyn;
    out.nodes.swap(hb.nodes);
    out.order.swap(hb.order);
    return ICON_OK;
}

template <class Put>
int emit_arena(const HostArrays &h, const MeshLayout &Ly, Put put_fn)
{
    int rc;
    std::vector<MeshDyn> dynv(1, h.dyn);
    if ((rc = put_fn(Ly.dyn, dynv.data(), sizeof(MeshDyn))) || (rc = put_fn(Ly.vnormals, h.vn.data(), h.vn.size() * 4)) ||
        (rc = put_fn(Ly.nodes, h.nodes.data(), h.nodes.size() * sizeof(BvhNode))) ||
        (rc = put_fn(Ly.leaves, h.leafrec.data(), h.leafrec.size() * sizeof(LeafRec))) ||
        (rc = put_fn(Ly.tris, h.tris.data(), h.tris.size() * sizeof(TriRec))) || (rc = put_fn(Ly.attr, h.attr.data(), h.attr.size() * sizeof(TriAttr))) ||
        (rc = put_fn(Ly.slot2face, h.order.data(), h.order.size() * 4)) || (rc = put_fn(Ly.face2slot, h.face2slot.data(), h.face2slot.size() * 4)) ||
        (rc = put_fn(Ly.bin_start, h.bin_start.data(), h.bin_start.size() * 4)) || (rc = put_fn(Ly.bin_slots, h.bin_slots.data(), h.bin_slots.size() * 4)))
        return rc;
    return ICON_OK;
}

int mesh_build_host(icon_mesh *m, const float *d_verts, const int64_t *d_faces, const float *d_cmap, const float *d_vis, hipStream_t st)
{
    const int64_t V = m->V, F = m->F;
    std::vector<float> verts(3 * V), cmap(3 * V), vis(V);
    std::vector<int64_t> faces(3 * F);
    ICON_HIP(hipMemcpyAsync(verts.data(), d_verts, sizeof(float) * 3 * V, hipMemcpyDeviceToHost, st));
    ICON_HIP(hipMemcpyAsync(faces.data(), d_faces, sizeof(int64_t) * 3 * F, hipMemcpyDeviceToHost, st));
    ICON_HIP(hipMemcpyAsync(cmap.data(), d_cmap, sizeof(float) * 3 * V, hipMemcpyDeviceToHost, st));
    ICON_HIP(hipMemcpyAsync(vis.data(), d_vis, sizeof(float) * V, hipMemcpyDeviceToHost, st));
    ICON_HIP(hipStreamSynchronize(st));
    HostArrays h;
    int rc = host_build(verts, faces, cmap, vis, V, F, m->depth_bound, h);
    if (rc) return rc;
    char *ar = m->arena;
    rc = emit_arena(h, mesh_layout(V, F), [&](size_t off, const void *src, size_t bytes) -> int {
        if (bytes) ICON_HIP(hipMemcpyAsync(ar + off, src, bytes, hipMemcpyHostToDevice, st));
        return ICON_OK;
    });
    if (rc) return rc;
    ICON_HIP(hipStreamSynchronize(st));
    *m->h_dyn = h.dyn;
    ICON_HIP(hipEventRecord(m->built, st));
    return ICON_OK;
}

int g_mesh_build_host = -1;

int mesh_create_common(const float *d_verts, int64_t V, const int64_t *d_faces, int64_t F, const float *d_cmap, const float *d_vis,
                       void *d_arena, size_t arena_bytes, bool owns, hipStream_t st, icon_mesh_t **out)
{
    icon_mesh *m = new icon_mesh();
    m->V = V; m->F = F; m->arena = (char *)d_arena; m->arena_bytes = arena_bytes; m->owns_arena = owns;
    m->depth_bound = depth_bound(F);
    int rc = mesh_host_state_get(&m->h_dyn, &m->built);
    if (rc) { icon_mesh_destroy(m); return rc; }
    mesh_bind_arena(m, mesh_layout(V, F));
    if (g_mesh_build_host < 0) { const char *e = getenv("ICON_AMD_MESH_BUILD"); g_mesh_build_host = (e && !strcmp(e, "host")) ? 1 : 0; }
    rc = g_mesh_build_host ? mesh_build_host(m, d_verts, d_faces, d_cmap, d_vis, st) : mesh_build_device(m, d_verts, d_faces, d_cmap, d_vis, st);
    if (rc) { icon_mesh_destroy(m); return rc; }
    *out = m;
    return ICON_OK;
}

int mesh_check_args(const float *d_verts, int64_t V, const int64_t *d_faces, int64_t F, const float *d_cmap, const float *d_vis, icon_mesh_t **out)
{
    ICON_ARG(out != nullptr, "icon_mesh_create: out is null");
// ... 59 lines not shown
}

extern "C" int icon_debug_set_mesh_build(int host)
{
    icon::g_mesh_build_host = host ? 1 : 0;
    return ICON_OK;
}

extern "C" int icon_mesh_vertex_normals(const icon_mesh_t *m, float *d_out, void *stream)
{
    ICON_ARG(m && d_out, "icon_mesh_vertex_normals: null argument");
    ICON_HIP(hipMemcpyAsync(d_out, m->d_vnormals, sizeof(float) * 3 * m->V, hipMemcpyDeviceToDevice, (hipStream_t)stream));
    return ICON_OK;
}

extern "C" int icon_mesh_status(const icon_mesh_t *m, int wait, int *bits)
{
    ICON_ARG(m != nullptr, "icon_mesh_status: mesh is null");
    if (wait) ICON_HIP(hipEventSynchronize(m->built));
    const int st = *reinterpret_cast<const volatile int32_t *>(&m->h_dyn->status);
    if (!(st & kMeshBuilt)) { if (bits) *bits = -1; return ICON_OK; }
    if (bits) *bits = st & ~kMeshBuilt;
    if (st & kMeshBadFace) return fail(ICON_ERR_ARG, "icon_mesh_create: face index out of range");
    if (st & kMeshBadVertex) return fail(ICON_ERR_ARG, "icon_mesh_create: non-finite (or absurdly large) vertex coordinate");
    if (st & kMeshInternal) return fail(ICON_ERR_STATE, "icon_mesh_create: the device BVH build failed an internal check");
    return ICON_OK;
}

extern "C" int icon_mesh_stats(const icon_mesh_t *m, int64_t out[6])
{
    ICON_ARG(m && out, "icon_mesh_stats: null argument");
    ICON_HIP(hipEventSynchronize(m->built));
    const MeshDyn &d = *m->h_dyn;
    out[0] = d.n_nodes; out[1] = d.depth; out[2] = d.bin_entries; out[3] = d.max_bin; out[4] = d.n_leaves; out[5] = m->F;
    return ICON_OK;
}

extern "C" int icon_debug_host_mesh_build(const float *h_verts, int64_t V, const int64_t *h_faces, int64_t F,
                                          const float *h_cmap, const float *h_vis, void *h_arena, int64_t arena_bytes)
{
    ICON_ARG(h_verts && h_faces && h_cmap && h_vis && h_arena, "icon_debug_host_mesh_build: null argument");
    ICON_ARG(V >= 3 && F >= 1 && F <= (1 << 23), "icon_debug_host_mesh_build: bad sizes");
    const MeshLayout Ly = mesh_layout(V, F);
    ICON_ARG(arena_bytes >= (int64_t)Ly.total, "icon_debug_host_mesh_build: arena too small");
    std::vector<float> verts(h_verts, h_verts + 3 * V), cmap(h_cmap, h_cmap + 3 * V), vis(h_vis, h_vis + V);
    std::vector<int64_t> faces(h_faces, h_faces + 3 * F);
    HostArrays h;
    int rc = host_build(verts, faces, cmap, vis, V, F, depth_bound(F), h);
    if (rc) return rc;
    char *ar = (char *)h_arena;
    return emit_arena(h, Ly, [&](size_t off, const void *src, size_t bytes) -> int { if (bytes) memcpy(ar + off, src, bytes); return ICON_OK; });
}

extern "C" int icon_debug_mesh_layout(int64_t V, int64_t F, int64_t out[12])
{
    ICON_ARG(out && V >= 3 && F >= 1 && F <= (1 << 23), "icon_debug_mesh_layout: bad argument");
    const MeshLayout L = mesh_layout(V, F);
    const size_t v[12] = {L.dyn, L.vnormals, L.nodes, L.leaves, L.tris, L.attr, L.slot2face, L.face2slot, L.bin_start, L.bin_slots, L.tbox, L.total};
    for (int k = 0; k < 12; ++k) out[k] = (int64_t)v[k];
    return ICON_OK;
}
```

### icon_amd/csrc/mesh_device.hip

```cpp
#pragma clang fp contract(off)

#include "common.h"
#include "mesh_rules.h"

#include <cstring>
#include <mutex>
#include <vector>

namespace icon {

namespace {

struct BuildCtx {
    const float *verts; const int64_t *faces; const float *cmap; const float *vis;
    int32_t V, F, bound;
    MeshDyn *dyn; BuildHdr *hdr;
    int32_t *valence; uint8_t *leaf_cnt; BTask *tasks; uint32_t *hist; int32_t *cell_count, *cell_cursor;
    float *vnormals; BvhNode *nodes; LeafRec *leaves; TriRec *tris; TriAttr *attr; int32_t *slot2face, *face2slot;
    int32_t *bin_start, *bin_slots;
    float *tbox, *cen; int32_t *order[2]; int32_t *adj; int32_t *chunkcnt; int32_t *subq; struct STask *sublist; uint32_t *bounds_part;
    int32_t nck; int64_t cells_cap, entries_cap;
};

__device__ __forceinline__ uint32_t enc(float f) { const uint32_t u = __float_as_uint(f); return (u & 0x80000000u) ? ~u : (u | 0x80000000u); }
__device__ __forceinline__ float dec(uint32_t u) { return __uint_as_float((u & 0x80000000u) ? (u & 0x7fffffffu) : ~u); }
__device__ __forceinline__ uint32_t enc_min(float f) { return ~enc(f); }
__device__ __forceinline__ float dec_min(uint32_t u) { return dec(~u); }

template <bool GLOBAL = false>
__device__ __forceinline__ void wave_sync()
{
    if (GLOBAL) asm volatile("s_waitcnt vmcnt(0) lgkmcnt(0)" ::: "memory");
    else asm volatile("s_waitcnt lgkmcnt(0)" ::: "memory");
    __builtin_amdgcn_wave_barrier();
}

__device__ __forceinline__ float sane(float v, int *bad) { if (bad_coord(v)) { *bad = 1; return 0.0f; } return v; }

__device__ __forceinline__ void load_face(const BuildCtx &c, int f, int id[3], float p[3][3], int *bad_face, int *bad_vert)
{
    for (int k = 0; k < 3; ++k) {
        int64_t v = c.faces[3 * (int64_t)f + k];
        if (v < 0 || v >= c.V) { *bad_face = 1; v = 0; }
        id[k] = (int)v;
        for (int a = 0; a < 3; ++a) p[k][a] = sane(c.verts[3 * v + a], bad_vert);
    }
}

__global__ __launch_bounds__(256) void k_face_prep(BuildCtx c)
{
    const int f = blockIdx.x * 256 + threadIdx.x;
    const bool live = f < c.F;
    float lo[3] = {INFINITY, INFINITY, INFINITY}, hi[3] = {-INFINITY, -INFINITY, -INFINITY}, ce[3] = {0.f, 0.f, 0.f};
    int bf = 0, bv = 0;
    if (live) {
        int id[3]; float p[3][3];
        load_face(c, f, id, p, &bf, &bv);
        for (int a = 0; a < 3; ++a) {
            lo[a] = canon(fminf(fminf(p[0][a], p[1][a]), p[2][a]));
            hi[a] = canon(fmaxf(fmaxf(p[0][a], p[1][a]), p[2][a]));
            ce[a] = canon(0.5f * (lo[a] + hi[a]));
            c.tbox[6 * f + a] = lo[a]; c.tbox[6 * f + 3 + a] = hi[a]; c.cen[3 * f + a] = ce[a];
        }
        c.order[0][f] = f;
        if (!bf)
            for (int k = 0; k < 3; ++k) {
                const int pos = atomicAdd(&c.valence[id[k]], 1);
                if (pos < kAdjCap) c.adj[(size_t)id[k] * kAdjCap + pos] = 3 * f + k;
            }
        if (bf | bv) atomicOr(&c.dyn->status, (bf ? kMeshBadFace : 0) | (bv ? kMeshBadVertex : 0));
    }
// ... 503 lines not shown
            for (int a = 0; a < 3; ++a) S->cen[i * 3 + a] = c.cen[3 * (size_t)e + a];
            for (int q = 0; q < 6; ++q) S->tbox[i * 6 + q] = c.tbox[6 * (size_t)e + q];
        }
        LdsAcc acc{S, T.begin};
        sub_levels(c, acc, S, S->list[0], S->list[1], kListCap, wave, lane, kSubWaves);
    } else {
        GlbAcc acc{{c.order[0], c.order[1]}, c.cen, c.tbox};
        STask *base = c.sublist + (size_t)(T.begin / 5) * 2;
        const int cap = n / 5;
        sub_levels(c, acc, S, base, base + cap, cap, wave, lane, kSubWaves);
    }
    if (threadIdx.x == 0) {
        if (S->n_nodes) atomicAdd(&c.dyn->n_nodes, S->n_nodes);
        atomicAdd(&c.dyn->n_leaves, S->n_leaves);
        atomicMax(&c.dyn->depth, S->depth);
    }
}

__device__ __forceinline__ BinGrid grid_of(const BuildCtx &c) { return bin_grid(c.dyn->box_lo, c.dyn->box_hi, c.F); }
__device__ __forceinline__ void cell_range(const BinGrid &g, const float *tb, int &cy0, int &cy1, int &cz0, int &cz1)
{
    cy0 = bin_cell_of(tb[1] - kBinEps, g.y0, g.inv_y, g.gy); cy1 = bin_cell_of(tb[4] + kBinEps, g.y0, g.inv_y, g.gy);
    cz0 = bin_cell_of(tb[2] - kBinEps, g.z0, g.inv_z, g.gz); cz1 = bin_cell_of(tb[5] + kBinEps, g.z0, g.inv_z, g.gz);
}

__global__ __launch_bounds__(256) void k_tri_records(BuildCtx c)
{
    const int p = blockIdx.x * 256 + threadIdx.x;
    if (p >= c.F) return;
    const int f = c.slot2face[p];
    int id[3]; float v[3][3]; int bf = 0, bv = 0;
    load_face(c, f, id, v, &bf, &bv);
    c.face2slot[f] = p;
    TriRec &tr = c.tris[p];
    for (int k = 0; k < 3; ++k) { tr.a[k] = v[0][k]; tr.b[k] = v[1][k]; tr.c[k] = v[2][k]; }
    tr.ia = id[0]; tr.ib = id[1]; tr.ic = id[2];
    TriAttr &at = c.attr[p];
    for (int q = 0; q < 3; ++q) {
        for (int k = 0; k < 3; ++k) { at.n[q][k] = c.vnormals[3 * (size_t)id[q] + k]; at.cm[q][k] = c.cmap[3 * (size_t)id[q] + k]; }
        at.vis[q] = c.vis[id[q]];
    }
    at.face = f; at.pad[0] = at.pad[1] = 0;
    int leaf = -1, myt = 0, cnt = 0;
    for (int t = 0; t < kLeafMax; ++t) {
        const int q = p - t;
        if (q >= 0 && c.leaf_cnt[q] > t) { leaf = q; myt = t; cnt = c.leaf_cnt[q]; break; }
    }
    if (leaf < 0) { atomicOr(&c.dyn->status, kMeshInternal); return; }
    TriPre pre;
    tri_setup(v[0], v[1], v[2], f, pre);
    const float *src = reinterpret_cast<const float *>(&pre);
    LeafRec &lr = c.leaves[leaf];
    const int tend = (myt == cnt - 1) ? kLeafMax : myt + 1;
    for (int t = myt; t < tend; ++t)
        for (int fld = 0; fld < 24; ++fld) lr.pair[t >> 1][fld][t & 1] = src[fld];
    const BinGrid g = grid_of(c);
    int cy0, cy1, cz0, cz1;
    cell_range(g, c.tbox + 6 * (size_t)f, cy0, cy1, cz0, cz1);
    for (int cz = cz0; cz <= cz1; ++cz)
        for (int cy = cy0; cy <= cy1; ++cy) atomicAdd(&c.cell_count[(size_t)cz * g.gy + cy], 1);
}

__global__ __launch_bounds__(1024) void k_scan_cells(BuildCtx c)
{
    __shared__ int wtot[16];
    const BinGrid g = grid_of(c);
    const int n = g.gy * g.gz;
    const int lane = threadIdx.x & 63, w = threadIdx.x >> 6;
    int64_t carry = 0;
    for (int base = 0; base < n; base += 4096) {
        const int i = base + (int)threadIdx.x * 4;
        int v[4];
#pragma unroll
        for (int k = 0; k < 4; ++k) v[k] = (i + k < n) ? c.cell_count[i + k] : 0;
        const int mine = v[0] + v[1] + v[2] + v[3];
        int incl = mine;
        for (int d = 1; d < 64; d <<= 1) { const int up = __shfl_up(incl, d); if (lane >= d) incl += up; }
        __syncthreads();
        if (lane == 63) wtot[w] = incl;
        __syncthreads();
        int before = 0, all = 0;
#pragma unroll
        for (int q = 0; q < 16; ++q) { const int t = wtot[q]; before += q < w ? t : 0; all += t; }
        int64_t run = carry + before + incl - mine;
#pragma unroll
        for (int k = 0; k < 4; ++k) { if (i + k < n) c.bin_start[i + k] = (int32_t)run; run += v[k]; }
        carry += all;
    }
    const bool fits = carry <= c.entries_cap;
    __syncthreads();
    if (!fits)
        for (int i = threadIdx.x; i <= n; i += 1024) c.bin_start[i] = 0;
    if (threadIdx.x == 0) {
        if (fits) c.bin_start[n] = (int32_t)carry;
        c.dyn->bin_entries = fits ? (int32_t)carry : 0;
        if (!fits) { c.dyn->gy = 0; c.dyn->gz = 0; atomicOr(&c.dyn->status, kMeshBinOverflow); }
    }
}

__global__ __launch_bounds__(256) void k_bin_fill(BuildCtx c)
{
    const int t = blockIdx.x * 256 + threadIdx.x;
    const int p = t >> 3, sub = t & 7;
    if (p >= c.F || (c.dyn->status & kMeshBinOverflow)) return;
    const BinGrid g = grid_of(c);
    int cy0, cy1, cz0, cz1;
    cell_range(g, c.tbox + 6 * (size_t)c.slot2face[p], cy0, cy1, cz0, cz1);
    int q = 0;
// ... 58 lines not shown
std::vector<hipEvent_t> g_free_ev;
std::vector<std::pair<MeshDyn *, hipEvent_t>> g_in_flight;

}

int mesh_host_state_get(MeshDyn **h, hipEvent_t *ev)
{
    std::lock_guard<std::mutex> lk(g_pool_mu);
    for (size_t i = 0; i < g_in_flight.size();) {
        if (hipEventQuery(g_in_flight[i].second) != hipErrorNotReady) {
            g_free_dyn.push_back(g_in_flight[i].first); g_free_ev.push_back(g_in_flight[i].second);
            g_in_flight[i] = g_in_flight.back(); g_in_flight.pop_back();
        } else ++i;
    }
    (void)hipGetLastError();
    if (g_free_dyn.empty()) {
        constexpr int kBatch = 32;
        MeshDyn *blk = nullptr;
        ICON_HIP(hipHostMalloc((void **)&blk, sizeof(MeshDyn) * kBatch, hipHostMallocDefault));
        for (int i = 0; i < kBatch; ++i) g_free_dyn.push_back(blk + i);
    }
    if (g_free_ev.empty()) {
        hipEvent_t e;
        ICON_HIP(hipEventCreateWithFlags(&e, hipEventDisableTiming));
        g_free_ev.push_back(e);
    }
    *h = g_free_dyn.back(); g_free_dyn.pop_back();
    *ev = g_free_ev.back(); g_free_ev.pop_back();
    memset(*h, 0, sizeof(MeshDyn));
    return ICON_OK;
}

void mesh_host_state_put(MeshDyn *h, hipEvent_t ev)
{
    std::lock_guard<std::mutex> lk(g_pool_mu);
    if (h && ev && hipEventQuery(ev) == hipErrorNotReady) { g_in_flight.emplace_back(h, ev); (void)hipGetLastError(); return; }
    (void)hipGetLastError();
    if (h) g_free_dyn.push_back(h);
    if (ev) g_free_ev.push_back(ev);
}

void mesh_bind_arena(icon_mesh *m, const MeshLayout &L)
{
    char *b = m->arena;
    m->d_dyn = reinterpret_cast<MeshDyn *>(b + L.dyn);
    m->d_vnormals = reinterpret_cast<float *>(b + L.vnormals);
    MeshDev &d = m->dev;
    d.nodes = reinterpret_cast<const BvhNode *>(b + L.nodes);
    d.tris = reinterpret_cast<const TriRec *>(b + L.tris);
    d.attr = reinterpret_cast<const TriAttr *>(b + L.attr);
    d.slot2face = reinterpret_cast<const int32_t *>(b + L.slot2face);
    d.face2slot = reinterpret_cast<const int32_t *>(b + L.face2slot);
    d.leaves = reinterpret_cast<const LeafRec *>(b + L.leaves);
    d.dyn = m->d_dyn;
    d.n_tris = (int32_t)m->F;
    d.bin_start = reinterpret_cast<const int32_t *>(b + L.bin_start);
    d.bin_slots = reinterpret_cast<const int32_t *>(b + L.bin_slots);
}

int mesh_build_device(icon_mesh *m, const float *d_verts, const int64_t *d_faces, const float *d_cmap, const float *d_vis, hipStream_t st)
{
    const MeshLayout L = mesh_layout(m->V, m->F);
    char *b = m->arena;
    BuildCtx c{};
    c.verts = d_verts; c.faces = d_faces; c.cmap = d_cmap; c.vis = d_vis;
    c.V = (int32_t)m->V; c.F = (int32_t)m->F; c.bound = m->depth_bound;
    c.dyn = reinterpret_cast<MeshDyn *>(b + L.dyn); c.hdr = reinterpret_cast<BuildHdr *>(b + L.hdr);
    c.valence = reinterpret_cast<int32_t *>(b + L.valence); c.leaf_cnt = reinterpret_cast<uint8_t *>(b + L.leaf_cnt);
    c.tasks = reinterpret_cast<BTask *>(b + L.tasks); c.hist = reinterpret_cast<uint32_t *>(b + L.hist);
    c.cell_count = reinterpret_cast<int32_t *>(b + L.cell_count); c.cell_cursor = reinterpret_cast<int32_t *>(b + L.cell_cursor);
    c.vnormals = reinterpret_cast<float *>(b + L.vnormals); c.nodes = reinterpret_cast<BvhNode *>(b + L.nodes);
    c.leaves = reinterpret_cast<LeafRec *>(b + L.leaves); c.tris = reinterpret_cast<TriRec *>(b + L.tris);
    c.attr = reinterpret_cast<TriAttr *>(b + L.attr); c.slot2face = reinterpret_cast<int32_t *>(b + L.slot2face);
    c.face2slot = reinterpret_cast<int32_t *>(b + L.face2slot); c.bin_start = reinterpret_cast<int32_t *>(b + L.bin_start);
    c.bin_slots = reinterpret_cast<int32_t *>(b + L.bin_slots); c.tbox = reinterpret_cast<float *>(b + L.tbox);
    c.cen = reinterpret_cast<float *>(b + L.cen); c.order[0] = reinterpret_cast<int32_t *>(b + L.order0);
    c.order[1] = reinterpret_cast<int32_t *>(b + L.order1); c.adj = reinterpret_cast<int32_t *>(b + L.adj);
    c.chunkcnt = reinterpret_cast<int32_t *>(b + L.chunkcnt); c.subq = reinterpret_cast<int32_t *>(b + L.subq);
    c.sublist = reinterpret_cast<STask *>(b + L.sublist); c.bounds_part = reinterpret_cast<uint32_t *>(b + L.bounds_part);
    c.nck = (int32_t)L.nck; c.cells_cap = bin_cells_cap(m->F); c.entries_cap = bin_entries_cap(m->F);

    ICON_HIP(hipMemsetAsync(b + L.dyn, 0, L.zero_end - L.dyn, st));
    const unsigned nbF = (unsigned)((m->F + 255) / 256), nbV = (unsigned)((m->V + 255) / 256);
    hipLaunchKernelGGL(k_face_prep, dim3(nbF), dim3(256), 0, st, c);
    debug_sync("k_face_prep", st);
    hipLaunchKernelGGL(k_vertex_normals, dim3(nbV), dim3(256), 0, st, c);
    debug_sync("k_vertex_normals", st);
    if (m->F > kSubMax) {
        for (int lv = 0; lv < kTopLevels; ++lv) {
            const unsigned nb = (unsigned)(m->F / kChunk + (1 << lv) + 1);
            hipLaunchKernelGGL(k_bvh_bin, dim3(nb), dim3(kChunk), 0, st, c, lv);
            hipLaunchKernelGGL(k_bvh_part, dim3(nb), dim3(kChunk), 0, st, c, lv);
            debug_sync("k_bvh_bin + k_bvh_part", st);
        }
    }
    static_assert(sizeof(SubLds) <= 160 * 1024 - 2048, "k_bvh_sub: LDS");
    {
        const int rc = once_per_device(8, [] { return hipFuncSetAttribute(reinterpret_cast<const void *>(k_bvh_sub), hipFuncAttributeMaxDynamicSharedMemorySize, (int)sizeof(SubLds)); });
        if (rc) return rc;
    }
    hipLaunchKernelGGL(k_bvh_sub, dim3((unsigned)(m->F > kSubMax ? kTaskSlots + 1 : 1)), dim3(kSubWaves * 64), sizeof(SubLds), st, c);
    debug_sync("k_bvh_sub", st);
    hipLaunchKernelGGL(k_tri_records, dim3(nbF), dim3(256), 0, st, c);
    debug_sync("k_tri_records", st);
    hipLaunchKernelGGL(k_scan_cells, dim3(1), dim3(1024), 0, st, c);
    hipLaunchKernelGGL(k_bin_fill, dim3((unsigned)((m->F * 8 + 255) / 256)), dim3(256), 0, st, c);
    hipLaunchKernelGGL(k_bin_sort, dim3((unsigned)((c.cells_cap + 255) / 256)), dim3(256), 0, st, c);
    debug_sync("ray bins", st);
    ICON_HIP(hipGetLastError());
    ICON_HIP(hipMemcpyAsync(m->h_dyn, c.dyn, sizeof(MeshDyn), hipMemcpyDeviceToHost, st));
    ICON_HIP(hipEventRecord(m->built, st));
    return ICON_OK;
}

}
```

### icon_amd/csrc/mesh_rules.h

```cpp
#pragma once
#include "common.h"

namespace icon {

__host__ __device__ inline int ilog2_ceil(int64_t n) { int l = 0; while (((int64_t)1 << l) < n) ++l; return l; }
__host__ __device__ inline int median_levels(int n) { int l = 0; while (n > kLeafMax) { n = (n + 1) / 2; ++l; } return l; }
__host__ __device__ inline int depth_bound(int64_t F)
{
    const int b = ilog2_ceil(F < 2 ? 2 : F) + 10;
    return b < kStackDepth - 2 ? b : kStackDepth - 2;
}
__host__ __device__ inline bool force_median(int depth, int n, int bound) { return depth + 1 + median_levels(n - 1) > bound; }

__host__ __device__ inline bool bad_coord(float v) { return !(v >= -1e6f && v <= 1e6f); }
__host__ __device__ inline float canon(float v) { return v + 0.0f; }

constexpr int kSahBins = 16;
__host__ __device__ inline int sah_bin(float c, float lo, float ext)
{
    int b = (int)((c - lo) / ext * (float)kSahBins);
    return b < 0 ? 0 : (b > kSahBins - 1 ? kSahBins - 1 : b);
}
struct BoxD { float lo[3], hi[3]; };
__host__ __device__ inline double box_area(const float lo[3], const float hi[3])
{
    const double dx0 = (double)hi[0] - lo[0], dy0 = (double)hi[1] - lo[1], dz0 = (double)hi[2] - lo[2];
    const double dx = dx0 > 0.0 ? dx0 : 0.0, dy = dy0 > 0.0 ? dy0 : 0.0, dz = dz0 > 0.0 ? dz0 : 0.0;
    return 2.0 * (dx * dy + dy * dz + dz * dx);
}

struct BinGrid { float y0, z0, y1, z1, inv_y, inv_z; int gy, gz; };
constexpr float kBinEps = 1e-5f;
__host__ __device__ inline BinGrid bin_grid(const float box_lo[3], const float box_hi[3], int64_t F)
{
    BinGrid g;
    g.y0 = box_lo[1] - 4 * kBinEps; g.y1 = box_hi[1] + 4 * kBinEps;
    g.z0 = box_lo[2] - 4 * kBinEps; g.z1 = box_hi[2] + 4 * kBinEps;
    const float ey = g.y1 - g.y0, ez = g.z1 - g.z0;
    float a = ey * ez;
    if (!(a > 1e-12f)) a = 1e-12f;
    const float cell = sqrtf(a / (2.0f * (float)F));
    int gy = (int)ceilf(ey / cell), gz = (int)ceilf(ez / cell);
    g.gy = gy < 1 ? 1 : (gy > 2048 ? 2048 : gy);
    g.gz = gz < 1 ? 1 : (gz > 2048 ? 2048 : gz);
    g.inv_y = (float)g.gy / ey; g.inv_z = (float)g.gz / ez;
    return g;
}
__host__ __device__ inline int bin_cell_of(float v, float v0, float inv, int g)
{
    const int c = (int)floorf((v - v0) * inv);
    return c < 0 ? 0 : (c > g - 1 ? g - 1 : c);
}
__host__ __device__ inline int64_t bin_cells_cap(int64_t F) { return 2 * F + 4100; }
__host__ __device__ inline int64_t bin_entries_cap(int64_t F) { return 48 * F + 2 * bin_cells_cap(F); }

__host__ __device__ inline float dot3r(const float *a, const float *b) { return fmaf(a[2], b[2], fmaf(a[1], b[1], a[0] * b[0])); }
__host__ __device__ inline void tri_setup(const float *a, const float *b, const float *c, int32_t face, TriPre &t)
{
    for (int k = 0; k < 3; ++k) { t.a[k] = a[k]; t.b[k] = b[k]; t.ab[k] = b[k] - a[k]; t.ac[k] = c[k] - a[k]; t.bc[k] = c[k] - b[k]; }
    t.a00 = dot3r(t.ab, t.ab); t.a01 = dot3r(t.ab, t.ac); t.a11 = dot3r(t.ac, t.ac);
    const float b11 = dot3r(t.bc, t.bc);
    t.i00 = (t.a00 > 0.0f) ? 1.0f / t.a00 : 0.0f;
    t.i11 = (t.a11 > 0.0f) ? 1.0f / t.a11 : 0.0f;
    t.ibc = (b11 > 0.0f) ? 1.0f / b11 : 0.0f;
    const float nn = fmaf(t.a00, t.a11, -(t.a01 * t.a01));
    t.inn = (nn > 0.0f) ? 1.0f / nn : __builtin_nanf("");
    t.face = face; t.pad = 0;
}

constexpr int kTopLevels = 7;
constexpr int kSubMax = 256;
constexpr int kChunk = 256;
constexpr int kAdjCap = 16;
constexpr int kHistWords = 3 * kSahBins * 13;
constexpr int kTaskSlots = (1 << (kTopLevels + 1)) - 1;

struct BTask {
    int32_t begin, end, depth, parent, side, kind, buf, from_atomics;
    float box[6], cb[6];
    uint32_t ubox[12];
};
static_assert(sizeof(BTask) == 128, "BTask layout");

struct BuildHdr {
    int32_t n_sub;
    int32_t pad[3];
};

struct MeshLayout {
    size_t dyn, hdr, valence, leaf_cnt, tasks, hist, cell_count, cell_cursor, zero_end;
    size_t vnormals, nodes, leaves, tris, attr, slot2face, face2slot, bin_start, bin_slots;
    size_t tbox, cen, order0, order1, adj, chunkcnt, subq, sublist, bounds_part, total;
    int64_t nck;
};
inline size_t align_up(size_t v, size_t a = 256) { return (v + a - 1) / a * a; }
inline MeshLayout mesh_layout(int64_t V, int64_t F)
{
    MeshLayout L{};
    size_t o = 0;
    auto take = [&](size_t bytes) { const size_t at = o; o = align_up(o + bytes); return at; };
    const int64_t cells = bin_cells_cap(F);
    L.nck = F / kChunk + (1 << kTopLevels) + 2;
    L.dyn = take(sizeof(MeshDyn));
    L.hdr = take(sizeof(BuildHdr));
    L.valence = take(sizeof(int32_t) * V);
    L.leaf_cnt = take((size_t)F);
    L.tasks = take(sizeof(BTask) * kTaskSlots);
    L.hist = take(sizeof(uint32_t) * kHistWords * ((1 << kTopLevels) - 1));
    L.cell_count = take(sizeof(int32_t) * (cells + 1));
    L.cell_cursor = take(sizeof(int32_t) * cells);
    L.zero_end = o;
    L.vnormals = take(sizeof(float) * 3 * V);
    L.nodes = take(sizeof(BvhNode) * F);
    L.leaves = take(sizeof(LeafRec) * F);
    L.tris = take(sizeof(TriRec) * F);
    L.attr = take(sizeof(TriAttr) * F);
    L.slot2face = take(sizeof(int32_t) * F);
    L.face2slot = take(sizeof(int32_t) * F);
    L.bin_start = take(sizeof(int32_t) * (cells + 1));
    L.bin_slots = take(sizeof(int32_t) * bin_entries_cap(F));
    L.tbox = take(sizeof(float) * 6 * F);
    L.cen = take(sizeof(float) * 3 * F);
    L.order0 = take(sizeof(int32_t) * F);
    L.order1 = take(sizeof(int32_t) * F);
    L.adj = take(sizeof(int32_t) * kAdjCap * V);
    L.chunkcnt = take(sizeof(int32_t) * 3 * kSahBins * L.nck * kTopLevels);
    L.subq = take(sizeof(int32_t) * (kTaskSlots + 1));
    L.sublist = take((size_t)80 * 2 * (F / 5 + 4));
    L.bounds_part = take(sizeof(uint32_t) * 12 * ((size_t)F / 256 + 1));
    L.total = o;
    return L;
}

}
```

### icon_amd/csrc/query_kernels.hip

```cpp
#pragma clang fp contract(off)

#include "geom_device.h"

namespace icon {

constexpr int kBlock = 256;

template <bool BRUTE>
__global__ __launch_bounds__(kBlock) void k_sdf_query(MeshDev m, const float *__restrict__ pts, int64_t N,
                                                      float *sdf, float *nrm, float *cm, float *vis,
                                                      int64_t *face, uint8_t *inside_out, const int32_t *__restrict__ perm)
{
    __shared__ int lds[kBruteTile * 24];
    int64_t i = (int64_t)blockIdx.x * kBlock + threadIdx.x;
    const bool live = i < N;
    if (live && perm) i = perm[i];
    const int64_t ic = live ? i : (N - 1);
    const f3 p = clamp_raw(mk3(pts[3 * ic], pts[3 * ic + 1], pts[3 * ic + 2]));
    Nearest nr;
    bool ins;
    if (BRUTE) { nr = nearest_brute<kBlock>(m, p, reinterpret_cast<float *>(lds)); ins = inside_brute(m, p); }
    else       { nr = nearest_packet(m, p, live, lds + (threadIdx.x >> 6) * kStackDepth); ins = inside_bins(m, p); }
    if (!live) return;
    const SdfOut o = sdf_attrs(m, p, nr, ins);
// ... 157 lines not shown
        f3 cmv;
        SdfOut o;
        if (BRUTE) {
            nr = nearest_brute<kBlock>(m, p, reinterpret_cast<float *>(lds)); ins = inside_brute(m, p);
            o = sdf_attrs(m, p, nr, ins);
            code = sign_code(p, nr.d2, ins, sdf_clip);
        } else {
            code = code8[i];
            nr.slot = near_slot_of(near, i); nr.face = 0;
            nr.d2 = (code & kCodeOutlier) ? 0.0f : near_d2(near, i);
            ins = (code & kCodeInside) != 0;
            o = sdf_attrs(m, p, nr, ins);
        }
        s = o.sdf;
        cmv = o.cm;
        if (code & kCodeOutlier) {
            s = (float)((int)((code >> kCodeSignShift) & 3u) - 1);
            if (cmap_local) cmv = mk3(s, s, s);
        }
        float g[16];
        gather_planes_dyn(f, (f.n_select == 2 && o.vis == 0.0f) ? 1 : 0, p.x, p.y, g);
        const int h = f.csel;
        for (int k = 0; k < h; ++k) row[k] = g[k];
        int hh = h;
        row[hh++] = s;
        if (f.smpl_mask & kSmplCmap) { row[hh] = cmv.x; row[hh + 1] = cmv.y; row[hh + 2] = cmv.z; hh += 3; }
        if (f.smpl_mask & kSmplNorm) { row[hh] = o.nrm.x; row[hh + 1] = o.nrm.y; row[hh + 2] = o.nrm.z; }
    } else {
        float g[16];
        gather_planes_dyn(f, 0, p.x, p.y, g);
        const int h = f.csel;
        for (int k = 0; k < h; ++k) row[k] = g[k];
        if (PRIOR == ICON_PRIOR_PAMIR) {
            float v[8];
            if (f.vpad == 8) gather_volume<2>(f, p.x, p.y, p.z, v); else gather_volume<1>(f, p.x, p.y, p.z, v);
            for (int k = 0; k < f.Cv; ++k) row[h + k] = v[k];
        } else {
            row[h] = p.z;
        }
    }
    row[kCodeSlot] = __int_as_float((int)code);
    if (live) { store_row(X, i, row); code8[i] = (uint8_t)code; }
}

__global__ __launch_bounds__(kBlock) void k_traversal_stats(MeshDev m, LatticeMap L, unsigned long long *out , int seeded)
{
    __shared__ int lds[(kBlock / 64) * kStackDepth];
    L = lattice_trim(L, m);
    if ((int)blockIdx.x >= L.tx * L.ty * L.tz) return;
    int ix, iy, iz, cx, cy, cz;
    const bool live = lattice_point(L, ix, iy, iz);
    lattice_clamp(L, ix, iy, iz, cx, cy, cz);
    const f3 p = lattice_world(L.res, cx, cy, cz + L.z0);
    int nn = 0, nt = 0;
    Nearest nr = nearest_packet<true>(m, p, live, lds + (threadIdx.x >> 6) * kStackDepth, &nn, &nt);
    if (seeded) {
        nn = 0; nt = 0;
        float thr0 = prune_threshold(nr.d2);
        if (seeded == 2) {
            const float dc = sqrtf(__int_as_float(__builtin_amdgcn_readlane(__float_as_int(nr.d2), 21)));
            const float h = 2.0f / (float)(L.res - 1);
            const float rad = 2.6f * h;
            thr0 = prune_threshold((dc + rad) * (dc + rad));
        }
        if (seeded == 3) {
            const float h = 2.0f / (float)(L.res - 1);
            int na = 0, nb = 0;
            const Nearest pv = nearest_packet<true>(m, mk3(p.x - 4.0f * h, p.y, p.z), live, lds + (threadIdx.x >> 6) * kStackDepth, &na, &nb);
            const float dn = sqrtf(pv.d2) + 4.0001f * h;
            thr0 = prune_threshold(dn * dn);
        }
        nr = nearest_packet<true>(m, p, live, lds + (threadIdx.x >> 6) * kStackDepth, &nn, &nt, thr0);
    }
    if ((threadIdx.x & 63) == 0) {
        atomicAdd(&out[0], 1ull); atomicAdd(&out[1], (unsigned long long)nn); atomicAdd(&out[2], (unsigned long long)nt);
    }
    if (live && nr.slot < 0) atomicAdd(&out[3], 1ull);
    if ((threadIdx.x & 63) == 0) atomicMax(&out[4], (unsigned long long)(nn + nt));
}

__global__ __launch_bounds__(kBlock) void k_row_crossings(MeshDev m, LatticeMap L, int32_t *row_count, int32_t *row_slots, LatticeFast *lf)
{
    if (lf && blockIdx.x == 0 && threadIdx.x == 0) lattice_fast_write(lf, L, m);
    if (lf) lattice_fast_coords(lf, L.res, (int64_t)blockIdx.x * kBlock + threadIdx.x);
    const int64_t row = (int64_t)blockIdx.x * kBlock + threadIdx.x;
    if (row >= (int64_t)L.nz * L.res) return;
    const int iy = (int)(row % L.res), iz = (int)(row / L.res);
    const f3 p = lattice_world(L.res, 0, iy, iz + L.z0);
    int n = 0;
    const MeshDyn &d = *m.dyn;
    if (d.gy == 0) { row_count[row] = -1; return; }
    if (p.y >= d.bin_y0 && p.y <= d.bin_y1 && p.z >= d.bin_z0 && p.z <= d.bin_z1) {
        const int cy = bin_cell(p.y, d.bin_y0, d.bin_inv_y, d.gy);
        const int cz = bin_cell(p.z, d.bin_z0, d.bin_inv_z, d.gz);
        const int cell = cz * d.gy + cy;
        const int beg = m.bin_start[cell], end = m.bin_start[cell + 1];
        for (int k = beg; k < end; ++k) {
            const int slot = m.bin_slots[k];
            f3 a, b, c; int ia, ib, ic;
            load_tri_full(m.tris + slot, a, b, c, ia, ib, ic);
            if (ray_covers(p, a, b, c, ia, ib, ic)) {
                if (n < kRowCap) row_slots[row * kRowCap + n] = slot;
                ++n;
            }
        }
    }
    row_count[row] = (n <= kRowCap) ? n : -1;
}


__device__ __forceinline__ uint32_t row_code(const float *X, int64_t i)
{
    return (uint32_t)__float_as_int(X[i * kXRow + kCodeSlot]);
}

__global__ __launch_bounds__(kScanBlock) void k_outlier_count(const uint8_t *__restrict__ code8, int64_t N, int32_t *block_counts)
{
    __shared__ int wsum[kScanBlock / 64];
    const int64_t i = (int64_t)blockIdx.x * kScanBlock + threadIdx.x;
    const bool o = (i < N) && (code8[i] & kCodeOutlier);
    const unsigned long long b = __ballot(o);
    if ((threadIdx.x & 63) == 0) wsum[threadIdx.x >> 6] = __popcll(b);
    __syncthreads();
    if (threadIdx.x == 0) {
        int s = 0;
        for (int w = 0; w < kScanBlock / 64; ++w) s += wsum[w];
        block_counts[blockIdx.x] = s;
    }
// ... 182 lines not shown
        for (int k = 0; k < 3; ++k) {
            int64_t mm = 3 * j + k;
            if (mm >= K) mm -= K;
            if (mm >= K) mm -= K;
            int r = 0;
            while (mm >= off[r + 1]) ++r;
            const int64_t e = mm - off[r];
            const uint32_t byte = (uint8_t)gathered[(int64_t)r * stride + 8 + (e >> 2)];
            row[k] = (float)((int)((byte >> (2 * (int)(e & 3))) & 3u) - 1);
        }
    }
}

__global__ __launch_bounds__(256) void k_pack_signs(const int8_t *__restrict__ signs, const int64_t *__restrict__ k_dev, uint8_t *__restrict__ msg, int64_t cap_bytes)
{
    const int64_t K = *k_dev;
    const int64_t t = (int64_t)blockIdx.x * 256 + threadIdx.x;
    if (t == 0) *reinterpret_cast<int64_t *>(msg) = K;
    if (t >= cap_bytes || 4 * t >= K) return;
    uint32_t b = 0;
#pragma unroll
    for (int j = 0; j < 4; ++j)
        if (4 * t + j < K) b |= (uint32_t)(signs[4 * t + j] + 1) << (2 * j);
    msg[8 + t] = (uint8_t)b;
}

__global__ void k_pack_planes(const float *__restrict__ src, int C, int H, int W, int n_select, int csel, int cpad, float *dst)
{
    const int64_t n = (int64_t)n_select * H * W * cpad;
    for (int64_t i = (int64_t)blockIdx.x * blockDim.x + threadIdx.x; i < n; i += (int64_t)gridDim.x * blockDim.x) {
        const int c = (int)(i % cpad);
        const int64_t pix = (i / cpad) % ((int64_t)H * W);
        const int sel = (int)(i / ((int64_t)cpad * H * W));
        dst[i] = (c < csel) ? src[((int64_t)(sel * csel + c)) * H * W + pix] : 0.0f;
    }
}

}

using namespace icon;


extern "C" int icon_sdf_query(const icon_mesh_t *mesh, const float *d_points, int64_t N,
                              float *d_sdf, float *d_norm, float *d_cmap, float *d_vis,
                              int64_t *d_face, uint8_t *d_inside, int search, void *stream)
{
    ICON_ARG(mesh && d_points && d_sdf && d_norm && d_cmap && d_vis, "icon_sdf_query: null argument");
    ICON_ARG(N >= 0, "icon_sdf_query: negative N");
    if (N == 0) return ICON_OK;
    const int64_t nb = (N + kBlock - 1) / kBlock;
    ICON_ARG(nb < (1ll << 31), "icon_sdf_query: N too large for one launch");
    hipStream_t st = (hipStream_t)stream;
    if (search == ICON_SEARCH_BRUTE) {
        hipLaunchKernelGGL(k_sdf_query<true>, dim3((unsigned)nb), dim3(kBlock), 0, st, mesh->dev, d_points, N, d_sdf, d_norm,
                           d_cmap, d_vis, d_face, d_inside, nullptr);
    } else if (N < kPacketMinPoints) {
        const int cap = coop_cap(mesh->depth_bound);
        hipLaunchKernelGGL(k_sdf_query_coop, dim3((unsigned)((N + kCoopWaves - 1) / kCoopWaves)), dim3(kCoopWaves * 64), kCoopWaves * coop_wave_bytes(cap), st,
                           mesh->dev, d_points, N, d_sdf, d_norm, d_cmap, d_vis, d_face, d_inside, cap);
    } else {
        icon_work tmp;
        static const float ident[12] = {1, 0, 0, 0, 0, 1, 0, 0, 0, 0, 1, 0};
        const int32_t *perm = nullptr;
        int rc = morton_order(&tmp, d_points, ident, nullptr, N, st, &perm);
        if (!rc) {
            hipLaunchKernelGGL(k_sdf_query<false>, dim3((unsigned)nb), dim3(kBlock), 0, st, mesh->dev, d_points, N, d_sdf, d_norm,
                               d_cmap, d_vis, d_face, d_inside, perm);
            if (hipGetLastError() != hipSuccess || hipStreamSynchronize(st) != hipSuccess) rc = fail(ICON_ERR_HIP, "icon_sdf_query: launch failed");
        }
        (void)hipFree(tmp.d_sort_keys); (void)hipFree(tmp.d_sort_idx); (void)hipFree(tmp.d_sort_tmp);
        return rc;
    }
    ICON_HIP(hipGetLastError());
    return ICON_OK;
}

extern "C" int icon_feat_create(const float *d_planes, int C, int H, int W, int n_select,
                                const float *d_vol, int Cv, int Dv, int Hv, int Wv,
                                void *stream, icon_feat_t **out)
{
    ICON_ARG(out != nullptr, "icon_feat_create: out is null");
    *out = nullptr;
    ICON_ARG(d_planes && C > 0 && H > 1 && W > 1, "icon_feat_create: bad planes");
    ICON_ARG(n_select == 1 || n_select == 2, "icon_feat_create: n_select must be 1 or 2");
    ICON_ARG(C % n_select == 0, "icon_feat_create: C not divisible by n_select");
    const int csel = C / n_select;
    const int cpad = (csel + 3) & ~3;
    if (cpad > 16) return fail(ICON_ERR_UNSUPPORTED, "icon_feat_create: more than 16 channels per tap");
    if (d_vol) {
        ICON_ARG(Cv > 0 && Dv > 1 && Hv > 1 && Wv > 1, "icon_feat_create: bad volume");
        if (Cv > 8) return fail(ICON_ERR_UNSUPPORTED, "icon_feat_create: more than 8 volume channels");
    }
    hipStream_t st = (hipStream_t)stream;
    icon_feat *f = new icon_feat();
    const size_t n = (size_t)n_select * H * W * cpad;
    hipError_t e = hipMalloc((void **)&f->d_planes, n * sizeof(float));
    if (e != hipSuccess) { delete f; return fail(ICON_ERR_HIP, std::string("hipMalloc planes: ") + hipGetErrorString(e)); }
    hipLaunchKernelGGL(k_pack_planes, dim3(1024), dim3(256), 0, st, d_planes, C, H, W, n_select, csel, cpad, f->d_planes);
    FeatDev &d = f->dev;
    d.planes = f->d_planes; d.C = C; d.H = H; d.W = W; d.n_select = n_select; d.csel = csel; d.cpad = cpad;
    d.smpl_mask = kSmplCmap | kSmplNorm;
    d.vol = nullptr; d.Cv = 0; d.Dv = d.Hv = d.Wv = 0; d.vpad = 0;
    if (d_vol) {
        const int vpad = (Cv + 3) & ~3;
        const size_t nv = (size_t)Dv * Hv * Wv * vpad;
        e = hipMalloc((void **)&f->d_vol, nv * sizeof(float));
        if (e != hipSuccess) { icon_feat_destroy(f); return fail(ICON_ERR_HIP, std::string("hipMalloc vol: ") + hipGetErrorString(e)); }
        hipLaunchKernelGGL(k_pack_planes, dim3(1024), dim3(256), 0, st, d_vol, Cv, Dv * Hv, Wv, 1, Cv, vpad, f->d_vol);
        d.vol = f->d_vol; d.Cv = Cv; d.Dv = Dv; d.Hv = Hv; d.Wv = Wv; d.vpad = vpad;
    }
    e = hipGetLastError();
    if (e != hipSuccess) { icon_feat_destroy(f); return fail(ICON_ERR_HIP, std::string("pack planes: ") + hipGetErrorString(e)); }
    *out = f;
    return ICON_OK;
}

extern "C" int icon_feat_set_smpl_feats(icon_feat_t *f, int has_cmap, int has_norm)
{
    ICON_ARG(f != nullptr, "icon_feat_set_smpl_feats: feat is null");
// ... 132 lines not shown
{
    ICON_ARG(w != nullptr, "icon_work_profile: work is null");
    if (enable && !w->ev[0])
        for (int k = 0; k < 6; ++k) ICON_HIP(hipEventCreate(&w->ev[k]));
    if (enable && !w->d_clock) {
        const size_t bytes = (size_t)(4 + kWgRec * kMaxProfGrid) * sizeof(unsigned long long);
        ICON_HIP(hipMalloc((void **)&w->d_clock, bytes));
        ICON_HIP(hipMemset(w->d_clock, 0, bytes));
    }
    w->clock_grid = 0;
    w->ev_search = false;
    w->prof = enable != 0;
    w->ev_valid = false;
    return ICON_OK;
}

extern "C" int icon_work_stage_ms(icon_work_t *w, float out_ms[3])
{
    ICON_ARG(w && out_ms, "icon_work_stage_ms: null argument");
    if (!w->prof || !w->ev_valid) return fail(ICON_ERR_STATE, "icon_work_stage_ms: no profiled call on this workspace");
    ICON_HIP(hipEventSynchronize(w->ev[3]));
    for (int k = 0; k < 3; ++k) ICON_HIP(hipEventElapsedTime(&out_ms[k], w->ev[k], w->ev[k + 1]));
    return ICON_OK;
}

namespace icon {
__global__ __launch_bounds__(kScanBlock) void k_outlier_patch_self(float *__restrict__ X, const uint8_t *__restrict__ code8, int64_t N, int cmap_slot,
                                                                   const int64_t *block_offsets, const int8_t *signs,
                                                                   const int64_t *k_total_dev)
{
    __shared__ int wsum[kScanBlock / 64];
    const int64_t K = *k_total_dev;
    const int64_t i = (int64_t)blockIdx.x * kScanBlock + threadIdx.x;
    const uint32_t code = (i < N) ? code8[i] : 0u;
    const bool o = code & kCodeOutlier;
    const int64_t j = outlier_rank(o, block_offsets, wsum);
    if (o) {
        float *row = X + i * kXRow + cmap_slot;
#pragma unroll
        for (int k = 0; k < 3; ++k) {
            int64_t mm = 3 * j + k;
            if (mm >= K) mm -= K;
            if (mm >= K) mm -= K;
            row[k] = (float)signs[mm];
        }
    }
}
}

namespace icon {
int g_share_ring = 0, g_share_lose = 0, g_share_spin_log2 = 0;
int g_lattice_fast = -1;
int g_share_waves = -2;
int share_waves_override()
{
    if (g_share_waves == -2) g_share_waves = getenv("ICON_AMD_SHARE") ? atoi(getenv("ICON_AMD_SHARE")) : -1;
    return g_share_waves;
}

int work_share_dbg(icon_work *w, ShareDbg *out)
{
    if (!w->h_err) {
        ICON_HIP(hipHostMalloc((void **)&w->h_err, 8 * sizeof(int), hipHostMallocMapped | hipHostMallocPortable));
        memset(w->h_err, 0, 8 * sizeof(int));
    }
    void *dev = nullptr;
    ICON_HIP(hipHostGetDevicePointer(&dev, w->h_err, 0));
    out->err = (int *)dev;
    out->ring = g_share_ring; out->lose = g_share_lose; out->spin_log2 = g_share_spin_log2;
    return ICON_OK;
}

int work_check_err(icon_work *w)
{
    if (!w || !w->h_err) return ICON_OK;
    volatile int *e = w->h_err;
    const int code = e[0];
    if (code == 0 || code == kShareErrClaimed) return ICON_OK;
    char buf[320];
    static const char *what[] = {"", "a wave waited in vain for the node of its queue ticket (lost or abandoned push)",
                                 "a wave waited in vain for its ring slot to be cleared (ring a full turn behind)",
                                 "an idle wave outlasted its bound while the workgroup was still active"};
    snprintf(buf, sizeof(buf), "shared-walk search: %s [code %d, workgroup %d, wave %d, ticket %d, head %d, tail %d, avail %d, active %d]; the results of "
             "that launch are not to be trusted", what[code >= 1 && code <= 3 ? code : 0], code, e[1], e[7], e[2], e[3], e[4], e[5], e[6]);
    for (int k = 0; k < 8; ++k) e[k] = 0;
    return fail(ICON_ERR_STATE, buf);
}

}

namespace {

inline void mark(icon_work *w, int k, hipStream_t st)
{
    if (w->prof) { (void)hipEventRecord(w->ev[k], st); if (k == 3) w->ev_valid = true; }
}

int ensure_work(icon_work *w, int64_t n_points, bool need_x)
{
    { const int rc = work_check_err(w); if (rc) return rc; }
    if (n_points > w->cap_points) {
        (void)hipFree(w->d_near16); (void)hipFree(w->d_near_d2); w->d_near16 = nullptr; w->d_near_d2 = nullptr; w->cap_points = 0;
        ICON_HIP(hipMalloc((void **)&w->d_near16, (size_t)n_points * sizeof(uint16_t)));
        ICON_HIP(hipMalloc((void **)&w->d_near_d2, (size_t)n_points * sizeof(float)));
        (void)hipFree(w->d_code8); w->d_code8 = nullptr;
        ICON_HIP(hipMalloc((void **)&w->d_code8, (size_t)n_points));
// ... 21 lines not shown
        ICON_HIP(hipMalloc((void **)&w->d_signs, (size_t)n_points));
        w->cap_signs = n_points;
    }
    if (!w->d_total) ICON_HIP(hipMalloc((void **)&w->d_total, sizeof(int64_t)));
    if (!w->d_flag) ICON_HIP(hipMalloc((void **)&w->d_flag, sizeof(int)));
    if (!w->d_steal) {
        ICON_HIP(hipMalloc((void **)&w->d_steal, 9 * sizeof(unsigned int)));
        ICON_HIP(hipMemset(w->d_steal, 0, 9 * sizeof(unsigned int)));
    }
    if (!w->d_seg) ICON_HIP(hipMalloc((void **)&w->d_seg, (kMaxWorld + 1) * sizeof(int64_t)));
    return ICON_OK;
}

int check_prior(const icon_mesh_t *mesh, const icon_feat_t *feat, int prior, int *c0)
{
    ICON_ARG(feat != nullptr, "feature handle is null");
    const FeatDev &f = feat->dev;
    if (prior == ICON_PRIOR_ICON) {
        ICON_ARG(mesh != nullptr, "icon prior needs a mesh handle");
        *c0 = f.csel + 1 + ((f.smpl_mask & kSmplCmap) ? 3 : 0) + ((f.smpl_mask & kSmplNorm) ? 3 : 0);
    } else if (prior == ICON_PRIOR_PAMIR) {
        ICON_ARG(f.n_select == 1 && f.vol != nullptr, "pamir prior needs n_select = 1 and a volume");
        *c0 = f.csel + f.Cv;
    } else if (prior == ICON_PRIOR_PIFU) {
        ICON_ARG(f.n_select == 1, "pifu prior needs n_select = 1");
        *c0 = f.csel + 1;
    } else {
        return fail(ICON_ERR_ARG, "unknown prior_type");
    }
    if (*c0 > kCodeSlot) return fail(ICON_ERR_UNSUPPORTED, "more than 15 MLP input channels");
    return ICON_OK;
}

template <bool LATTICE>
int launch_nearest(const icon_mesh_t *mesh, const Calib &cal, const LatticeMap &L, const float *d_points, int64_t N, float sdf_clip,
                   icon_work *work, hipStream_t st)
{
    LatticeFast *lf = nullptr;
    if (LATTICE) {
        const int64_t rows = (int64_t)L.nz * L.res;
        if (rows > work->cap_rows) {
            (void)hipFree(work->d_row_count); (void)hipFree(work->d_row_slots);
            work->d_row_count = nullptr; work->d_row_slots = nullptr; work->cap_rows = 0;
            ICON_HIP(hipMalloc((void **)&work->d_row_count, (size_t)rows * sizeof(int32_t)));
            ICON_HIP(hipMalloc((void **)&work->d_row_slots, (size_t)rows * kRowCap * sizeof(int32_t)));
            work->cap_rows = rows;
        }
        if (g_lattice_fast < 0) g_lattice_fast = getenv("ICON_AMD_LATTICE_FAST") ? (atoi(getenv("ICON_AMD_LATTICE_FAST")) != 0) : 1;
        if (g_lattice_fast && (L.pk == 0 || L.pk == 4) && L.remap == 0 && L.res <= kLatticeFastMaxRes) {
            if (!work->d_lfast) ICON_HIP(hipMalloc((void **)&work->d_lfast, kLatticeFastBytes));
            lf = work->d_lfast;
        }
        if (rows <= 20000)
            hipLaunchKernelGGL(k_row_crossings_wide, dim3((unsigned)((rows * 16 + kBlock - 1) / kBlock)), dim3(kBlock), 0, st, mesh->dev, L,
                               work->d_row_count, work->d_row_slots, lf);
        else
            hipLaunchKernelGGL(k_row_crossings, dim3((unsigned)((rows + kBlock - 1) / kBlock)), dim3(kBlock), 0, st, mesh->dev, L,
                               work->d_row_count, work->d_row_slots, lf);
    }
    int64_t nb;
    if (LATTICE) nb = (int64_t)L.tx * L.ty * L.tz; else nb = (N + kBlock - 1) / kBlock;
    ICON_ARG(nb >= 0 && nb < (1ll << 31), "too many workgroups for one launch");
    if (mesh->F > kNearLoSlots && work->cap_points_hi < work->cap_points) {
        (void)hipFree(work->d_near_hi); work->d_near_hi = nullptr; work->cap_points_hi = 0;
        ICON_HIP(hipMalloc((void **)&work->d_near_hi, (size_t)work->cap_points));
        work->cap_points_hi = work->cap_points;
    }
    const NearRef near = work_near(work, mesh);
    const int32_t *perm = nullptr;
    static const int mode = getenv("ICON_AMD_POINT_SEARCH") ? atoi(getenv("ICON_AMD_POINT_SEARCH")) : 0;
    const bool alt = work->tie_rule != 0;
    if (!LATTICE && !alt && mode != 3 && (N < kPacketMinPoints || mode == 2)) {
        const int cap = coop_cap(mesh->depth_bound);
        hipLaunchKernelGGL(k_nearest_coop, dim3((unsigned)((N + kCoopWaves - 1) / kCoopWaves)), dim3(kCoopWaves * 64),
                           kCoopWaves * coop_wave_bytes(cap), st, mesh->dev, cal, d_points, N, near, cap, sdf_clip);
    } else if (nb > 0) {
        if (!LATTICE) {
            const int rc = morton_order(work, d_points, cal.m, cal.d, N, st, &perm);
            if (rc) return rc;
        }
        const int share_env = share_waves_override();
        const int nw = (!LATTICE || alt) ? 1 : ((share_env == 1 || share_env == 8 || share_env == 16) ? share_env : share_waves(nb * 4));
        ShareDbg dbg{};
        if (nw > 1) { const int rc = work_share_dbg(work, &dbg); if (rc) return rc; }
        if (work->prof) (void)hipEventRecord(work->ev[4], st);
        if (nw == 16) hipLaunchKernelGGL(k_nearest_shared<16>, dim3((unsigned)nb * 4), dim3(16 * 64), 0, st, mesh->dev, L, near, sdf_clip, dbg);
        else if (nw == 8) hipLaunchKernelGGL(k_nearest_shared<8>, dim3((unsigned)nb * 4), dim3(8 * 64), 0, st, mesh->dev, L, near, sdf_clip, dbg);
        else if (alt) hipLaunchKernelGGL((k_nearest<LATTICE, true>), dim3((unsigned)nb), dim3(kBlock), 0, st, mesh->dev, cal, L, d_points, N, near, perm, sdf_clip, work->tie_ulps, lf);
        else hipLaunchKernelGGL((k_nearest<LATTICE, false>), dim3((unsigned)nb), dim3(kBlock), 0, st, mesh->dev, cal, L, d_points, N, near, perm, sdf_clip, 0, lf);
        if (work->prof) { (void)hipEventRecord(work->ev[5], st); work->ev_search = true; }
    }
    ICON_HIP(hipGetLastError());
    debug_sync(LATTICE ? "k_row_crossings + k_nearest<lattice>" : "nearest (points)", st);
    const int rc_sign = launch_sign(mesh, cal, L.res, L.z0, d_points, N, sdf_clip, work, LATTICE, st);
    debug_sync("k_sign", st);
    return rc_sign;
}

template <bool LATTICE>
int launch_features(const icon_mesh_t *mesh, const icon_feat_t *feat, int prior, float sdf_clip, int cmap_mode,
                    const Calib &cal, const LatticeMap &L, const float *d_points, int64_t N, int search,
                    icon_work *work, hipStream_t st)
{
    LatticeMap Lf = L;
    const int skip_shell = L.off;
    if (LATTICE) {
        Lf.sx0 = Lf.sy0 = Lf.sz0 = 0; Lf.sx1 = Lf.sy1 = L.res; Lf.sz1 = L.nz;
        Lf.tx = (L.res + 15) / 16; Lf.ty = (L.res + 3) / 4; Lf.tz = (L.nz + 3) / 4; Lf.pk = 4; Lf.trim = 0;
    }
    int64_t nb;
    if (LATTICE) nb = (int64_t)Lf.tx * Lf.ty * Lf.tz; else nb = (N + kBlock - 1) / kBlock;
    ICON_ARG(nb > 0 && nb < (1ll << 31), "too many workgroups for one launch");
    const dim3 grid((unsigned)nb), block(kBlock);
    const MeshDev md = mesh ? mesh->dev : MeshDev{};
    const int local = (cmap_mode == ICON_CMAP_LOCAL) ? 1 : 0;
    const bool brute = (search == ICON_SEARCH_BRUTE);
#define ICON_LAUNCH(P, B) hipLaunchKernelGGL((k_features<P, LATTICE, B>), grid, block, 0, st, md, feat->dev, cal, Lf, d_points, N, sdf_clip, local, work->d_row_count, work->d_row_slots, work_near(work, mesh), work->d_x, work->d_code8, skip_shell)
    if (prior == ICON_PRIOR_ICON) { if (brute) ICON_LAUNCH(ICON_PRIOR_ICON, true); else ICON_LAUNCH(ICON_PRIOR_ICON, false); }
    else if (prior == ICON_PRIOR_PAMIR) ICON_LAUNCH(ICON_PRIOR_PAMIR, false);
    else ICON_LAUNCH(ICON_PRIOR_PIFU, false);
#undef ICON_LAUNCH
    ICON_HIP(hipGetLastError());
    return ICON_OK;
}

int outlier_list(icon_work *w, int64_t N, int8_t *signs, bool counted, hipStream_t st)
{
    const int64_t nblk = (N + kScanBlock - 1) / kScanBlock;
    if (!counted) hipLaunchKernelGGL(k_outlier_count, dim3((unsigned)nblk), dim3(kScanBlock), 0, st, w->d_code8, N, w->d_block_counts);
    if (nblk <= 1024) {
        hipLaunchKernelGGL(k_outlier_small, dim3((unsigned)std::max<int64_t>(nblk, 1)), dim3(kScanBlock), 0, st, w->d_block_counts, w->d_code8, N, w->d_block_offsets, w->d_total,
                           signs, (const int *)nullptr);
        ICON_HIP(hipGetLastError());
        debug_sync("outlier list (one launch)", st);
        return ICON_OK;
    }
    const int64_t nchunks = (nblk + 1023) / 1024;
    hipLaunchKernelGGL(k_scan_local, dim3((unsigned)nchunks), dim3(1024), 0, st, w->d_block_counts, nblk, w->d_scan_local, w->d_scan_part, (const int *)nullptr);
    hipLaunchKernelGGL(k_scan_apply, dim3((unsigned)nchunks), dim3(1024), 0, st, w->d_scan_local, w->d_scan_part, nchunks, nblk, w->d_block_offsets, w->d_total, (const int *)nullptr);
    hipLaunchKernelGGL(k_outlier_compact, dim3((unsigned)nblk), dim3(kScanBlock), 0, st, w->d_code8, N, w->d_block_offsets, signs, (const int *)nullptr);
    ICON_HIP(hipGetLastError());
    debug_sync("outlier scan + compact", st);
    return ICON_OK;
}

}

namespace icon {
int outlier_list_dev(icon_work *w, const int *n_dev, int64_t n_max, hipStream_t st)
{
    const int64_t nblk = (n_max + kScanBlock - 1) / kScanBlock;
    if (nblk <= kSmallListBlocks) {
        hipLaunchKernelGGL(k_outlier_small, dim3((unsigned)std::max<int64_t>(nblk, 1)), dim3(kScanBlock), 0, st, w->d_block_counts, w->d_code8, n_max, w->d_block_offsets,
                           w->d_total, w->d_signs, n_dev);
        ICON_HIP(hipGetLastError());
        return ICON_OK;
    }
    const int64_t nchunks = (nblk + 1023) / 1024;
    hipLaunchKernelGGL(k_scan_local, dim3((unsigned)nchunks), dim3(1024), 0, st, w->d_block_counts, nblk, w->d_scan_local, w->d_scan_part, n_dev);
    hipLaunchKernelGGL(k_scan_apply, dim3((unsigned)nchunks), dim3(1024), 0, st, w->d_scan_local, w->d_scan_part, nchunks, nblk, w->d_block_offsets, w->d_total, n_dev);
    hipLaunchKernelGGL(k_outlier_compact, dim3((unsigned)nblk), dim3(kScanBlock), 0, st, w->d_code8, n_max, w->d_block_offsets, w->d_signs, n_dev);
    ICON_HIP(hipGetLastError());
    return ICON_OK;
}
int ensure_work_points(icon_work *w, int64_t n_points) { return ensure_work(w, n_points, false); }
}

// ... 285 lines not shown
    }
    return phase2(mlp, fs, d_occ, precision, work, (hipStream_t)stream, za, zb);
}

static int copy_rows_out(icon_work *work, float *d_rows, hipStream_t st)
{
    int rc = materialise_rows(work, self_signs(work), st);
    if (rc) return rc;
    ICON_HIP(hipMemcpyAsync(d_rows, work->d_x, (size_t)work->q_N * kXRow * sizeof(float), hipMemcpyDeviceToDevice, st));
    return ICON_OK;
}

extern "C" int icon_query_rows(const icon_mesh_t *mesh, const icon_feat_t *feat, int prior_type, float sdf_clip, int cmap_mode,
                               const float *h_calib, const float *d_calib, const float *d_points, int64_t N, float *d_rows,
                               int search, icon_work_t *work, void *stream)
{
    ICON_ARG(work && d_points && d_rows, "icon_query_rows: null argument");
    ICON_ARG(N >= 0, "icon_query_rows: negative N");
    int c0 = 0;
    int rc = check_prior(mesh, feat, prior_type, &c0);
    if (rc) return rc;
    if (N == 0) return ICON_OK;
    hipStream_t st = (hipStream_t)stream;
    if ((rc = ensure_work(work, N, false))) return rc;
    Calib cal;
    static const float ident[12] = {1, 0, 0, 0, 0, 1, 0, 0, 0, 0, 1, 0};
    memcpy(cal.m, h_calib ? h_calib : ident, sizeof(cal.m));
    cal.d = d_calib;
    LatticeMap L{};
    work->slab_ready = false;
    if ((rc = phase1<false>(mesh, feat, prior_type, sdf_clip, cmap_mode, cal, L, d_points, N, search, nullptr, work, st))) return rc;
    return copy_rows_out(work, d_rows, st);
}

extern "C" int icon_grid_rows(const icon_mesh_t *mesh, const icon_feat_t *feat, int prior_type, float sdf_clip, int cmap_mode,
                              int res, int z0, int z1, float *d_rows, int search, icon_work_t *work, void *stream)
{
    ICON_ARG(work && d_rows, "icon_grid_rows: null argument");
    int c0 = 0;
    int rc = check_prior(mesh, feat, prior_type, &c0);
    if (rc) return rc;
    LatticeMap L;
    if ((rc = lattice_map(res, z0, z1, nullptr, sdf_clip, false, &L))) return rc;
    hipStream_t st = (hipStream_t)stream;
    const int64_t N = (int64_t)L.nz * res * res;
    ICON_ARG(N < (1ll << 31), "icon_grid_rows: more than 2^31 points in one slab");
    if ((rc = ensure_work(work, N, false))) return rc;
    Calib cal{};
    work->slab_ready = false;
    if ((rc = phase1<true>(mesh, feat, prior_type, sdf_clip, cmap_mode, cal, L, nullptr, N, search, nullptr, work, st))) return rc;
    return copy_rows_out(work, d_rows, st);
}

extern "C" int icon_debug_traversal_stats(const icon_mesh_t *mesh, int res, int z0, int z1, uint64_t out[4])
{
    ICON_ARG(mesh && out, "icon_debug_traversal_stats: null argument");
    LatticeMap L;
    int rc = lattice_map(res, z0, z1, mesh, 0.05f, true, &L);
    if (rc) return rc;
    unsigned long long *d = nullptr;
    ICON_HIP(hipMalloc((void **)&d, 8 * sizeof(unsigned long long)));
    ICON_HIP(hipMemset(d, 0, 8 * sizeof(unsigned long long)));
    hipLaunchKernelGGL(k_traversal_stats, dim3((unsigned)(L.tx * L.ty * L.tz)), dim3(kBlock), 0, 0, mesh->dev, L, d,
                       getenv("ICON_AMD_STATS_SEEDED") ? atoi(getenv("ICON_AMD_STATS_SEEDED")) : 0);
    unsigned long long h[8];
    hipError_t e = hipMemcpy(h, d, sizeof(h), hipMemcpyDeviceToHost);
    (void)hipFree(d);
    if (e != hipSuccess) return fail(ICON_ERR_HIP, std::string("traversal stats: ") + hipGetErrorString(e));
    out[0] = h[0]; out[1] = h[1]; out[2] = h[2]; out[3] = h[4];
    return ICON_OK;
}

extern "C" int icon_grid_eval_slab(const icon_mesh_t *mesh, const icon_feat_t *feat, const icon_mlp_t *mlp,
                                   int prior_type, float sdf_clip, int cmap_mode,
                                   int res, int z0, int z1, float *d_occ,
                                   int search, int precision, icon_work_t *work, void *stream)
{
    ICON_ARG(mlp && work && d_occ, "icon_grid_eval_slab: null argument");
    int rc = icon_grid_slab_features(mesh, feat, prior_type, sdf_clip, cmap_mode, res, z0, z1, nullptr, nullptr, search, work, stream);
    if (rc) return rc;
    ICON_ARG(work->slab_c0 == mlp->c0, "icon_grid_eval_slab: MLP input width does not match the feature layout");
    work->slab_ready = false;
    return phase2(mlp, self_signs(work), d_occ, precision, work, (hipStream_t)stream, z0, z1);
}

extern "C" int icon_work_status(icon_work_t *work)
{
    ICON_ARG(work != nullptr, "icon_work_status: work is null");
    return work_check_err(work);
}

extern "C" int icon_debug_set_option(const char *key, int value)
{
    ICON_ARG(key != nullptr, "icon_debug_set_option: key is null");
    const std::string k(key);
    if (k == "lattice_fast") g_lattice_fast = value ? 1 : 0;
    else if (k == "share_waves") { ICON_ARG(value == -1 || value == 1 || value == 4 || value == 8 || value == 16, "share_waves: -1 (by launch size), 1, 4, 8 or 16"); g_share_waves = value; }
    else if (k == "share_ring") { ICON_ARG(value == 0 || (value >= 2 && value <= 64 && (value & (value - 1)) == 0), "share_ring: 0 or a power of two in 2..64"); g_share_ring = value; }
    else if (k == "share_lose_push") { ICON_ARG(value >= 0, "share_lose_push: a ticket >= 1, or 0"); g_share_lose = value; }
    else if (k == "share_spin_log2") { ICON_ARG(value >= 0 && value < 30, "share_spin_log2: 0..29"); g_share_spin_log2 = value; }
    else return fail(ICON_ERR_ARG, "icon_debug_set_option: unknown key " + k);
    return ICON_OK;
}

extern "C" int icon_debug_set_shell_skip(int on)
{
    g_shell_skip = on ? 1 : 0;
    return ICON_OK;
}

extern "C" int icon_work_set_tie_rule(icon_work_t *work, int rule, int ulps)
{
    ICON_ARG(work != nullptr, "icon_work_set_tie_rule: work is null");
    ICON_ARG(rule == 0 || rule == 1, "icon_work_set_tie_rule: rule must be 0 (definition) or 1 (highest index within ulps)");
    ICON_ARG(ulps >= 0 && ulps <= 255, "icon_work_set_tie_rule: ulps must be 0..255");
    work->tie_rule = rule; work->tie_ulps = ulps;
    return ICON_OK;
}

extern "C" int icon_sdf_query_ties(const icon_mesh_t *mesh, const float *d_points, int64_t N,
                                   int32_t *d_face, int32_t *d_face2, uint8_t *d_ulps, void *stream)
{
    ICON_ARG(mesh && d_points && d_face && d_face2 && d_ulps, "icon_sdf_query_ties: null argument");
    ICON_ARG(N >= 0, "icon_sdf_query_ties: negative N");
    if (N == 0) return ICON_OK;
    const int64_t nb = (N + kBlock - 1) / kBlock;
    ICON_ARG(nb < (1ll << 31), "icon_sdf_query_ties: N too large for one launch");
    hipStream_t st = (hipStream_t)stream;
    icon_work tmp;
    static const float ident[12] = {1, 0, 0, 0, 0, 1, 0, 0, 0, 0, 1, 0};
    const int32_t *perm = nullptr;
    int rc = morton_order(&tmp, d_points, ident, nullptr, N, st, &perm);
    if (!rc) {
        hipLaunchKernelGGL(k_nearest_ties, dim3((unsigned)nb), dim3(kBlock), 0, st, mesh->dev, d_points, N, perm, d_face, d_face2, d_ulps);
        if (hipGetLastError() != hipSuccess || hipStreamSynchronize(st) != hipSuccess) rc = fail(ICON_ERR_HIP, "icon_sdf_query_ties: launch failed");
    }
    (void)hipFree(tmp.d_sort_keys); (void)hipFree(tmp.d_sort_idx); (void)hipFree(tmp.d_sort_tmp);
    return rc;
}
```

### icon_amd/engine.py

```python
from __future__ import annotations

import contextlib
import ctypes as C
from typing import Optional, Sequence

import numpy as np
import torch
import torch.nn as nn

from . import _lib
from ._lib import IconAmdError, check, ptr


def _stream() -> C.c_void_p:
    return C.c_void_p(torch.cuda.current_stream().cuda_stream)


def _on(t: torch.Tensor):
    return torch.cuda.device(t.device) if t.is_cuda else contextlib.nullcontext()


def _key(*tensors) -> tuple:
    return tuple((t.data_ptr(), t._version, t.shape, t.device) for t in tensors)

# ... 23 lines not shown


class MeshHandle(_Handle):
    _destroy = "icon_mesh_destroy"

    def __init__(self, smpl_verts, smpl_faces, smpl_cmap, smpl_vis, validate: bool = True):
        super().__init__()
        _lib.require_device()
        for t, what in ((smpl_verts, "smpl_verts"), (smpl_faces, "smpl_faces"), (smpl_cmap, "smpl_cmap"), (smpl_vis, "smpl_vis")):
            if t.dim() == 3 and t.shape[0] > 1:
                raise IconAmdError(f"{what} has batch size {t.shape[0]}: a MeshHandle holds one subject (MeshBatchHandle for [B,...])")
        v = _dev_f32(smpl_verts, "smpl_verts").reshape(-1, 3)
        f = smpl_faces.detach()
        if not f.is_cuda:
            raise IconAmdError("smpl_faces must be on the HIP device")
        f = f.to(torch.int64).reshape(-1, 3).contiguous()
        cm = _dev_f32(smpl_cmap, "smpl_cmap").reshape(-1, 3)
        vs = _dev_f32(smpl_vis, "smpl_vis").reshape(-1)
        if cm.shape[0] != v.shape[0] or vs.shape[0] != v.shape[0]:
            raise IconAmdError("smpl_cmap / smpl_vis do not match smpl_verts")
        self.V, self.F = int(v.shape[0]), int(f.shape[0])
        self.device = v.device
        self.checked = False
        nbytes = C.c_int64(0)
        check(_lib.lib().icon_mesh_arena_bytes(C.c_int64(self.V), C.c_int64(self.F), C.byref(nbytes)), "icon_mesh_arena_bytes")
        with _on(v):
            self.arena = torch.empty(int(nbytes.value), dtype=torch.uint8, device=v.device)
            check(_lib.lib().icon_mesh_create_arena(ptr(v), C.c_int64(self.V), ptr(f), C.c_int64(self.F), ptr(cm), ptr(vs),
                                                    ptr(self.arena), nbytes, _stream(), C.byref(self.h)), "icon_mesh_create")
        if validate:
            self.status(wait=True)

    def status(self, wait: bool = False) -> Optional[int]:
        if self.checked:
            return 0
        bits = C.c_int(0)
        check(_lib.lib().icon_mesh_status(self.h, C.c_int(int(wait)), C.byref(bits)), "icon_mesh_create")
        if bits.value < 0:
            return None
        self.checked = True
        return int(bits.value)

    def vertex_normals(self) -> torch.Tensor:
        out = torch.empty((self.V, 3), dtype=torch.float32, device=self.device)
        check(_lib.lib().icon_mesh_vertex_normals(self.h, ptr(out), _stream()), "icon_mesh_vertex_normals")
        return out

    def stats(self) -> dict:
        arr = (C.c_int64 * 6)()
        check(_lib.lib().icon_mesh_stats(self.h, arr), "icon_mesh_stats")
        return dict(nodes=arr[0], depth=arr[1], bin_entries=arr[2], max_bin=arr[3], leaves=arr[4], slots=arr[5])

    def traversal_stats(self, res: int, z0: int = 0, z1: Optional[int] = None) -> dict:
        arr = (C.c_uint64 * 4)()
        check(_lib.lib().icon_debug_traversal_stats(self.h, C.c_int(res), C.c_int(z0), C.c_int(res if z1 is None else z1), arr),
              "icon_debug_traversal_stats")
        return dict(waves=arr[0], nodes=arr[1], tris=arr[2], nodes_per_wave=arr[1] / max(arr[0], 1),
                    tris_per_wave=arr[2] / max(arr[0], 1), longest_walk=arr[3])

    def sdf_query(self, points: torch.Tensor, search: str = "bvh"):
        p = _dev_f32(points, "points").reshape(-1, 3)
        n = p.shape[0]
        dev = p.device
        out = dict(sdf=torch.empty(n, device=dev), norm=torch.empty((n, 3), device=dev),
                   cmap=torch.empty((n, 3), device=dev), vis=torch.empty(n, device=dev),
                   face=torch.empty(n, dtype=torch.int64, device=dev),
                   inside=torch.empty(n, dtype=torch.uint8, device=dev))
        check(_lib.lib().icon_sdf_query(self.h, ptr(p), C.c_int64(n), ptr(out["sdf"]), ptr(out["norm"]),
                                        ptr(out["cmap"]), ptr(out["vis"]), ptr(out["face"]), ptr(out["inside"]),
                                        C.c_int(_lib.SEARCH[search]), _stream()), "icon_sdf_query")
        out["inside"] = out["inside"].bool()
        return out


    def sdf_query_ties(self, points: torch.Tensor) -> dict:
        p = _dev_f32(points, "points").reshape(-1, 3)
        n, dev = p.shape[0], p.device
        out = dict(face=torch.empty(n, dtype=torch.int32, device=dev), face2=torch.empty(n, dtype=torch.int32, device=dev),
                   ulps=torch.empty(n, dtype=torch.uint8, device=dev))
        check(_lib.lib().icon_sdf_query_ties(self.h, ptr(p), C.c_int64(n), ptr(out["face"]), ptr(out["face2"]), ptr(out["ulps"]),
                                             _stream()), "icon_sdf_query_ties")
        return out


class MeshBatchHandle(_Handle):
    _destroy = "icon_mesh_batch_destroy"

    def __init__(self, smpl_verts, smpl_faces, smpl_cmap, smpl_vis):
        super().__init__()
        ts = (smpl_verts, smpl_faces, smpl_cmap, smpl_vis)
        if any(t.dim() != 3 for t in ts):
            raise IconAmdError("smpl_feat_dict tensors must be [B,V,3] / [B,F,3] / [B,V,3] / [B,V,1] for a batched query")
        self.B = int(smpl_verts.shape[0])
        if any(int(t.shape[0]) != self.B for t in ts):
            raise IconAmdError(f"smpl_feat_dict batch sizes disagree: {[int(t.shape[0]) for t in ts]}")
        self.subjects = [MeshHandle(smpl_verts[b], smpl_faces[b], smpl_cmap[b], smpl_vis[b], validate=False) for b in range(self.B)]
        arr = (C.c_void_p * self.B)(*[m.h.value for m in self.subjects])
        with _on(smpl_verts):
            check(_lib.lib().icon_mesh_batch_create(arr, C.c_int(self.B), _stream(), C.byref(self.h)), "icon_mesh_batch_create")
        self.checked = False

    @property
    def V(self):
        return self.subjects[0].V

    def status(self, wait: bool = False) -> Optional[int]:
        if self.checked:
            return 0
        pending = False
        for m in self.subjects:
            if m.status(wait) is None:
# ... 924 lines not shown
```

### include/icon_amd.h

```cpp
#ifndef ICON_AMD_H
#define ICON_AMD_H

#include <stdint.h>

#ifdef __cplusplus
extern "C" {
#endif

#define ICON_AMD_VERSION 100

enum {
    ICON_OK = 0,
    ICON_ERR_ARG = 1,
    ICON_ERR_HIP = 2,
    ICON_ERR_UNSUPPORTED = 3,
    ICON_ERR_STATE = 4
};

enum { ICON_PRIOR_ICON = 0, ICON_PRIOR_PAMIR = 1, ICON_PRIOR_PIFU = 2 };

enum { ICON_CMAP_REFERENCE = 0, ICON_CMAP_LOCAL = 1 };

enum { ICON_PRECISION_F32 = 0, ICON_PRECISION_F16X3 = 1 };

// ... 62 lines not shown

typedef struct icon_mesh_batch icon_mesh_batch_t;
int icon_mesh_batch_create(const icon_mesh_t *const *meshes, int B, void *stream, icon_mesh_batch_t **out);
int icon_mesh_batch_destroy(icon_mesh_batch_t *mb);
#define ICON_MESH_BATCH_FACES_DIFFER 0x10
int icon_mesh_batch_status(const icon_mesh_batch_t *mb, int wait, int *bits);

int icon_feat_create_batch(const float *d_planes, int B, int C, int H, int W, int n_select, void *stream, icon_feat_t **out);

int icon_feat_batch_set_volume(icon_feat_t *feat, const float *d_vol, int B, int Cv, int Dv, int Hv, int Wv, void *stream);

int icon_query_points_batch(const icon_mesh_batch_t *mb, const icon_feat_t *feat, const icon_mlp_t *mlp,
                            int prior_type, float sdf_clip, int cmap_mode, const float *d_calibs,
                            const float *d_points, int64_t N, int B, float *d_occ,
                            int search, int precision, icon_work_t *work, void *stream);

int icon_grid_eval_slab(const icon_mesh_t *mesh, const icon_feat_t *feat, const icon_mlp_t *mlp,
                        int prior_type, float sdf_clip, int cmap_mode,
                        int res, int z0, int z1, float *d_occ,
                        int search, int precision, icon_work_t *work, void *stream);

int icon_grid_slab_features(const icon_mesh_t *mesh, const icon_feat_t *feat,
                            int prior_type, float sdf_clip, int cmap_mode,
                            int res, int z0, int z1, int8_t *d_signs_local, int64_t *d_count_local,
                            int search, icon_work_t *work, void *stream);
int icon_grid_slab_finish(const icon_mlp_t *mlp, int res, int z0, int z1,
                          const int8_t *d_signs_global, int64_t k_total, int64_t rank_offset,
                          float *d_occ, int precision, icon_work_t *work, void *stream);
int icon_grid_slab_features_msg(const icon_mesh_t *mesh, const icon_feat_t *feat,
                                int prior_type, float sdf_clip, int cmap_mode,
                                int res, int z0, int z1, void *d_msg, int64_t msg_bytes,
                                int search, icon_work_t *work, void *stream);
int icon_grid_slab_finish_gathered(const icon_mlp_t *mlp, int res, int z0, int z1, int za, int zb,
                                   const void *d_gathered, int64_t stride, int world, int rank,
                                   float *d_occ, int precision, icon_work_t *work, void *stream);

int icon_adaptive_eval(const icon_mesh_t *mesh, const icon_feat_t *feat, const icon_mlp_t *mlp, int prior_type, float sdf_clip,
                       int cmap_mode, const int *resolutions, int n_levels, float balance, float *d_out, int64_t *h_counts,
                       int search, int precision, icon_work_t *work, void *stream);
int icon_adaptive_counts(icon_work_t *work, int n_levels, int64_t *h_counts, void *stream);
int icon_adaptive_reruns(icon_work_t *work, int *n);

int icon_query_rows(const icon_mesh_t *mesh, const icon_feat_t *feat, int prior_type, float sdf_clip, int cmap_mode,
                    const float *h_calib, const float *d_calib, const float *d_points, int64_t N, float *d_rows,
                    int search, icon_work_t *work, void *stream);
int icon_grid_rows(const icon_mesh_t *mesh, const icon_feat_t *feat, int prior_type, float sdf_clip, int cmap_mode,
                   int res, int z0, int z1, float *d_rows, int search, icon_work_t *work, void *stream);

int icon_debug_set_unfused(int on);
int icon_debug_set_mesh_build(int host);
int icon_debug_mesh_layout(int64_t V, int64_t F, int64_t out[12]);
int icon_debug_host_mesh_build(const float *h_verts, int64_t V, const int64_t *h_faces, int64_t F,
                               const float *h_cmap, const float *h_vis, void *h_arena, int64_t arena_bytes);
int icon_debug_set_shell_skip(int on);
int icon_debug_set_option(const char *key, int value);
int icon_work_status(icon_work_t *work);

int icon_sdf_query_ties(const icon_mesh_t *mesh, const float *d_points, int64_t N,
                        int32_t *d_face, int32_t *d_face2, uint8_t *d_ulps, void *stream);
int icon_work_set_tie_rule(icon_work_t *work, int rule, int ulps);

int icon_debug_traversal_stats(const icon_mesh_t *mesh, int res, int z0, int z1, uint64_t out[4]);

int icon_volume_any_above(const float *d_occ, int res, int sx, int sy, int sz, float level, icon_work_t *work, void *stream, int *h_any);

int icon_export_mesh(const float *h_occ, int res, float level,
                     float *h_verts, int64_t *n_verts, int64_t *h_faces, int64_t *n_faces);

int icon_mc_count(const float *d_occ, int res, float level, icon_work_t *work, void *stream,
                  int64_t *n_verts, int64_t *n_faces);
int icon_mc_emit(float *d_verts, int64_t *d_faces, icon_work_t *work, void *stream);
int icon_mc_count_range(const float *d_occ, int res, float level, int zc0, int zc1, int halo, icon_work_t *work, void *stream,
                        int64_t *n_verts, int64_t *n_faces);
int icon_mc_emit_keyed(float *d_verts, int64_t *d_faces, int64_t *d_keys, icon_work_t *work, void *stream);

int icon_semantic_voxelize(const float *d_verts, int64_t V, int64_t V_surf, const float *d_code,
                           const int64_t *d_tets, int64_t T, int res, float sigma, float *d_out, void *stream);

int icon_semantic_voxelize_batch(const float *d_verts, int B, int64_t V, int64_t V_surf, const float *d_code,
                                 const int64_t *d_tets, int64_t T, int res, float sigma, uint8_t *d_occ, float *d_out, void *stream);

int icon_mesh_components(const int64_t *d_faces, int64_t F, int64_t V, int32_t *d_labels, void *stream);

int icon_clean_mesh(const float *d_verts, int64_t V, const int64_t *d_faces, int64_t F, float *d_out_verts, int32_t *d_out_faces,
                    int64_t *h_counts, icon_work_t *work, void *stream);

int icon_visibility(const float *d_xy, const float *d_z, int64_t V, const int64_t *d_faces, int64_t F,
                    int image_size, float *d_vis, void *stream);

#ifdef __cplusplus
}
#endif
#endif
```

Measured before the change: 997.7 million.

## Add per-triangle slab lower bound to prefilter exact point-triangle distance tests

Precomputes, for each triangle pair in a BVH leaf, a compact bound record (normal, in-plane tangent, edge extents, half-width) stored in a new LeafBound array. During nearest-triangle traversal, a cheap lower bound on squared distance is computed from values shared with the exact test, and pairs whose bound exceeds the current prune threshold for all lanes (wave ballot) are skipped. This aims to cut exact triangle distance work, at the cost of extra memory reads per pair, a wave-wide ballot, and a larger mesh arena. It is toggled by a debug option and routed through a mesh_dev helper at every launch site.

```diff
diff --git a/icon_amd/_lib.py b/icon_amd/_lib.py
--- a/icon_amd/_lib.py
+++ b/icon_amd/_lib.py
@@ -27,7 +27,7 @@
     "icon_export_mesh", "icon_mc_count", "icon_mc_emit", "icon_mc_count_range", "icon_mc_emit_keyed", "icon_debug_traversal_stats", "icon_debug_set_unfused",
     "icon_visibility", "icon_mesh_components", "icon_clean_mesh", "icon_semantic_voxelize",
     "icon_mesh_batch_create", "icon_mesh_batch_destroy", "icon_mesh_batch_status", "icon_feat_create_batch", "icon_query_points_batch",
-    "icon_feat_batch_set_volume", "icon_semantic_voxelize_batch",
+    "icon_feat_batch_set_volume", "icon_semantic_voxelize_batch", "icon_debug_tri_bound", "icon_debug_traversal_stats_ex",
 ]
 
 _lib = None
diff --git a/icon_amd/csrc/adaptive.hip b/icon_amd/csrc/adaptive.hip
--- a/icon_amd/csrc/adaptive.hip
+++ b/icon_amd/csrc/adaptive.hip
@@ -486,7 +486,7 @@
             ShareDbg dbg{};
             if ((rc = work_share_dbg(work, &dbg))) return rc;
 #define ICON_AD_NEAREST(PP, NW) hipLaunchKernelGGL((k_ad_nearest<PP, NW>), dim3((unsigned)(n_cu * 32 / (NW == 1 ? 4 : NW))), dim3(NW == 1 ? 256 : NW * 64), 0, st, \
-                                                   mesh->dev, r, nbk, a->blk_list, a->counters + 8, C, raw, sdf_clip, dbg)
+                                                   mesh_dev(mesh), r, nbk, a->blk_list, a->counters + 8, C, raw, sdf_clip, dbg)
             if (P == 4 && nw == 16) ICON_AD_NEAREST(4, 16);
             else if (P == 4 && nw == 8) ICON_AD_NEAREST(4, 8);
             else if (P == 4 && nw == 4) ICON_AD_NEAREST(4, 4);
diff --git a/icon_amd/csrc/batch_query.hip b/icon_amd/csrc/batch_query.hip
--- a/icon_amd/csrc/batch_query.hip
+++ b/icon_amd/csrc/batch_query.hip
@@ -206,7 +206,7 @@
     if (e == hipSuccess) e = hipHostMalloc((void **)&mb->h_status, sizeof(int), hipHostMallocPortable);
     if (e == hipSuccess) e = hipEventCreateWithFlags(&mb->done, hipEventDisableTiming);
     if (e != hipSuccess) { icon_mesh_batch_destroy(mb); return fail(ICON_ERR_HIP, std::string("icon_mesh_batch_create: ") + hipGetErrorString(e)); }
-    for (int b = 0; b < B; ++b) mb->h_table[b] = meshes[b]->dev;
+    for (int b = 0; b < B; ++b) mb->h_table[b] = mesh_dev(meshes[b]);
     int *h_word = reinterpret_cast<int *>(reinterpret_cast<char *>(mb->h_table) + tab_bytes);
     int *d_word = reinterpret_cast<int *>(reinterpret_cast<char *>(mb->d_table) + tab_bytes);
     *h_word = kBatchChecked;
diff --git a/icon_amd/csrc/common.h b/icon_amd/csrc/common.h
--- a/icon_amd/csrc/common.h
+++ b/icon_amd/csrc/common.h
@@ -60,6 +60,12 @@
     float pair[2][24][2];
 };
 static_assert(sizeof(LeafRec) == 384, "LeafRec must be 384 bytes");
+
+constexpr int kBoundFields = 12;
+struct alignas(32) LeafBound {
+    float pair[2][kBoundFields][2];
+};
+static_assert(sizeof(LeafBound) == 192, "LeafBound must be 192 bytes");
 
 constexpr int kLeafMax = 4;
 constexpr int kShareWavesMany = 8, kShareWavesFew = 16;
@@ -99,6 +105,7 @@
     const int32_t *slot2face;
     const int32_t *face2slot;
     const LeafRec *leaves;
+    const LeafBound *bounds;
     const MeshDyn *dyn;
     int32_t n_tris;
     const int32_t *bin_start;
@@ -269,6 +276,7 @@
 int work_share_dbg(icon_work *w, ShareDbg *out);
 int work_check_err(icon_work *w);
 int share_waves_override();
+int tri_prefilter();
 }
 
 struct icon_work {
@@ -335,6 +343,12 @@
 };
 
 namespace icon {
+inline MeshDev mesh_dev(const icon_mesh *m)
+{
+    MeshDev d = m->dev;
+    if (!tri_prefilter()) d.bounds = nullptr;
+    return d;
+}
 constexpr int kNearLoSlots = 32768;
 inline NearRef work_near(const icon_work *w, const icon_mesh *mesh)
 {
diff --git a/icon_amd/csrc/fused_f16x3.hip b/icon_amd/csrc/fused_f16x3.hip
--- a/icon_amd/csrc/fused_f16x3.hip
+++ b/icon_amd/csrc/fused_f16x3.hip
@@ -722,13 +722,13 @@
     const int64_t nb = (N + 255) / 256;
     ICON_ARG(nb > 0 && nb < (1ll << 31), "too many workgroups for one launch");
     const float far_box2 = far_box_dist2(sdf_clip);
-    if (lattice) hipLaunchKernelGGL(k_sign<true>, dim3((unsigned)nb), dim3(256), 0, st, mesh->dev, cal, res, z0, d_points, N, sdf_clip,
+    if (lattice) hipLaunchKernelGGL(k_sign<true>, dim3((unsigned)nb), dim3(256), 0, st, mesh_dev(mesh), cal, res, z0, d_points, N, sdf_clip,
                                     work->d_row_count, work->d_row_slots, work_near(work, mesh), work->d_code8, work->d_block_counts,
                                     (unsigned long long *)work->d_grp_mask, far_box2, (const int *)nullptr, work->d_flag);
     else if (work->q_n_dev || N <= 262144)
-        hipLaunchKernelGGL(k_sign_wide, dim3((unsigned)nb), dim3(1024), 0, st, mesh->dev, cal, d_points, N, sdf_clip, work_near(work, mesh), work->d_code8,
+        hipLaunchKernelGGL(k_sign_wide, dim3((unsigned)nb), dim3(1024), 0, st, mesh_dev(mesh), cal, d_points, N, sdf_clip, work_near(work, mesh), work->d_code8,
                            work->d_block_counts, (unsigned long long *)work->d_grp_mask, far_box2, work->q_n_dev, work->d_flag);
-    else hipLaunchKernelGGL(k_sign<false>, dim3((unsigned)nb), dim3(256), 0, st, mesh->dev, cal, res, z0, d_points, N, sdf_clip,
+    else hipLaunchKernelGGL(k_sign<false>, dim3((unsigned)nb), dim3(256), 0, st, mesh_dev(mesh), cal, res, z0, d_points, N, sdf_clip,
                             (const int32_t *)nullptr, (const int32_t *)nullptr, work_near(work, mesh), work->d_code8, work->d_block_counts,
                             (unsigned long long *)work->d_grp_mask, far_box2, work->q_n_dev, work->d_flag);
     ICON_HIP(hipGetLastError());
@@ -778,7 +778,7 @@
                        const icon_work *work, const FusedSigns &fs, float *d_occ, bool lattice, hipStream_t st, const BatchDev *bd)
 {
     FusedGeom G{};
-    if (mesh) G.m = mesh->dev;
+    if (mesh) G.m = mesh_dev(mesh);
     G.f = feat->dev; G.cal = cal; G.pts = d_points; G.sdf_clip = sdf_clip; G.cmap_local = cmap_local;
     if (lattice) {
         const int zs = std::max(za, L.off), ze = std::min(zb, L.res - L.off);
diff --git a/icon_amd/csrc/geom_device.h b/icon_amd/csrc/geom_device.h
--- a/icon_amd/csrc/geom_device.h
+++ b/icon_amd/csrc/geom_device.h
@@ -78,15 +78,44 @@
     return dot3x2(d, d);
 }
 
-__device__ __forceinline__ f2 tri_dist2_pair(f3 p1, cf2 *q)
+__device__ __forceinline__ void tri_ap_d1_pair(f3 p1, cf2 *q, f3x2 &ap, f2 &d1)
 {
     f3x2 p; p.x = bc2(p1.x); p.y = bc2(p1.y); p.z = bc2(p1.z);
-    f3x2 a, b, ab, ac, bc;
-    a.x = q[0]; a.y = q[1]; a.z = q[2]; b.x = q[3]; b.y = q[4]; b.z = q[5];
+    f3x2 a, ab;
+    a.x = q[0]; a.y = q[1]; a.z = q[2]; ab.x = q[6]; ab.y = q[7]; ab.z = q[8];
+    ap = sub3x2(p, a);
+    d1 = dot3x2(ab, ap);
+}
+
+__device__ __forceinline__ f2 tri_bound_pair(f3x2 ap, f2 d1, cf2 *g)
+{
+    f3x2 n, t;
+    n.x = g[0]; n.y = g[1]; n.z = g[2]; t.x = g[3]; t.y = g[4]; t.z = g[5];
+    const f2 inv_ab = g[6], ulo = g[7], uhi = g[8], vlo = g[9], vhi = g[10], hw = g[11];
+    const f2 w = dot3x2(n, ap), v = dot3x2(t, ap);
+    const f2 u0 = ulo - d1, u1 = d1 - uhi, v0 = vlo - v, v1 = v - vhi, w0 = w - hw, w1 = w + hw;
+    f2 eu, ev, ew;
+    eu.x = fmaxf(fmaxf(u0.x, u1.x), 0.0f); eu.y = fmaxf(fmaxf(u0.y, u1.y), 0.0f);
+    ev.x = fmaxf(fmaxf(v0.x, v1.x), 0.0f); ev.y = fmaxf(fmaxf(v0.y, v1.y), 0.0f);
+    ew.x = fmaxf(fmaxf(w0.x, -w1.x), 0.0f); ew.y = fmaxf(fmaxf(w0.y, -w1.y), 0.0f);
+    eu = eu * inv_ab;
+    return fma2(ew, ew, fma2(ev, ev, eu * eu));
+}
+
+__device__ __forceinline__ bool pair_needed(f2 lb, float thr)
+{
+    return (__builtin_amdgcn_ballot_w64(!(lb.x > thr)) | __builtin_amdgcn_ballot_w64(!(lb.y > thr))) != 0;
+}
+
+__device__ __forceinline__ f2 tri_dist2_pair(f3 p1, cf2 *q, f3x2 ap, f2 d1)
+{
+    f3x2 p; p.x = bc2(p1.x); p.y = bc2(p1.y); p.z = bc2(p1.z);
+    f3x2 b, ab, ac, bc;
+    b.x = q[3]; b.y = q[4]; b.z = q[5];
     ab.x = q[6]; ab.y = q[7]; ab.z = q[8]; ac.x = q[9]; ac.y = q[10]; ac.z = q[11]; bc.x = q[12]; bc.y = q[13]; bc.z = q[14];
     const f2 i00 = q[15], i11 = q[16], ibc = q[17], a00 = q[18], a01 = q[19], a11 = q[20], inn = q[21];
-    const f3x2 ap = sub3x2(p, a), bp = sub3x2(p, b);
-    const f2 d1 = dot3x2(ab, ap), d2 = dot3x2(ac, ap), d3 = dot3x2(bc, bp);
+    const f3x2 bp = sub3x2(p, b);
+    const f2 d2 = dot3x2(ac, ap), d3 = dot3x2(bc, bp);
     const f2 s = fma2(a11, d1, -(a01 * d2)) * inn;
     const f2 u = fma2(a00, d2, -(a01 * d1)) * inn;
     const f2 su = s + u;
@@ -203,7 +232,7 @@
 __device__ __forceinline__ Nearest nearest_packet(const MeshDev &m, f3 p, bool live, int *wstack ,
                                                   int *n_nodes = nullptr, int *n_tris = nullptr, float thr0 = INFINITY,
                                                   unsigned long long *runner_up = nullptr, int center_lane = 21,
-                                                  bool have_root = false, int root = 0)
+                                                  bool have_root = false, int root = 0, int *n_pairs = nullptr)
 {
     Nearest nr; nr.d2 = INFINITY; nr.slot = 0; nr.face = 0x7fffffff;
     unsigned long long key = 0x7f8000007fffffffull;
@@ -219,7 +248,15 @@
             const int npairs = __builtin_amdgcn_readfirstlane((cnt + 1) >> 1);
             for (int pr = 0; pr < npairs; ++pr) {
                 cf2 *q = reinterpret_cast<cf2 *>(as_const(&m.leaves[leaf].pair[pr]));
-                const f2 d2 = tri_dist2_pair(p, q);
+                f3x2 ap; f2 d1;
+                tri_ap_d1_pair(p, q, ap, d1);
+                if (m.bounds) {
+                    const f2 lb = tri_bound_pair(ap, d1, reinterpret_cast<cf2 *>(as_const(&m.bounds[leaf].pair[pr])));
+                    const float thr_pair = TIES ? (live ? prune_threshold(__int_as_float((int)(key2 >> 32))) : -INFINITY) : thr;
+                    if (!pair_needed(lb, thr_pair)) continue;
+                }
+                if (STATS) ++*n_pairs;
+                const f2 d2 = tri_dist2_pair(p, q, ap, d1);
                 const f2 fc = q[22];
                 const unsigned long long k0 = ((unsigned long long)(unsigned)__float_as_int(d2.x) << 32) | (unsigned)__float_as_int(fc.x);
                 const unsigned long long k1 = ((unsigned long long)(unsigned)__float_as_int(d2.y) << 32) | (unsigned)__float_as_int(fc.y);
@@ -384,7 +421,10 @@
                 const int npairs = __builtin_amdgcn_readfirstlane((cnt + 1) >> 1);
                 for (int pr = 0; pr < npairs; ++pr) {
                     cf2 *q = reinterpret_cast<cf2 *>(as_const(&m.leaves[leaf].pair[pr]));
-                    const f2 d2 = tri_dist2_pair(p, q);
+                    f3x2 ap; f2 d1;
+                    tri_ap_d1_pair(p, q, ap, d1);
+                    if (m.bounds && !pair_needed(tri_bound_pair(ap, d1, reinterpret_cast<cf2 *>(as_const(&m.bounds[leaf].pair[pr]))), thr)) continue;
+                    const f2 d2 = tri_dist2_pair(p, q, ap, d1);
                     const f2 fc = q[22];
                     const unsigned long long k0 = ((unsigned long long)(unsigned)__float_as_int(d2.x) << 32) | (unsigned)__float_as_int(fc.x);
                     const unsigned long long k1 = ((unsigned long long)(unsigned)__float_as_int(d2.y) << 32) | (unsigned)__float_as_int(fc.y);
@@ -431,6 +471,7 @@
 {
     const float thr = live ? prune_threshold(__int_as_float((int)best_bits)) : -INFINITY;
     const uint32_t lim = best_bits + ulps;
+    const float thr_lim = live ? prune_threshold(lim >= 0x7f800000u ? INFINITY : __uint_as_float(lim)) : -INFINITY;
     int face = -1;
     uint32_t fbits = best_bits;
     int sp = 0, cur = mesh_root(m);
@@ -441,7 +482,10 @@
             const int npairs = __builtin_amdgcn_readfirstlane((cnt + 1) >> 1);
             for (int pr = 0; pr < npairs; ++pr) {
                 cf2 *q = reinterpret_cast<cf2 *>(as_const(&m.leaves[leaf].pair[pr]));
-                const f2 d2 = tri_dist2_pair(p, q);
+                f3x2 ap; f2 d1;
+                tri_ap_d1_pair(p, q, ap, d1);
+                if (m.bounds && !pair_needed(tri_bound_pair(ap, d1, reinterpret_cast<cf2 *>(as_const(&m.bounds[leaf].pair[pr]))), thr_lim)) continue;
+                const f2 d2 = tri_dist2_pair(p, q, ap, d1);
                 const f2 fc = q[22];
                 const uint32_t b0 = (uint32_t)__float_as_int(d2.x), b1 = (uint32_t)__float_as_int(d2.y);
                 const int f0 = __float_as_int(fc.x), f1 = __float_as_int(fc.y);
@@ -501,13 +545,22 @@
     const unsigned long long lt_mask = (lane == 0) ? 0ull : (~0ull >> (64 - lane));
     unsigned long long key = 0x7f8000007fffffffull;
     int slot = 0;
-    auto tri_key = [&](int leaf, int t, int cnt, int &out_slot) -> unsigned long long {
+    auto tri_key = [&](int leaf, int t, int cnt, int &out_slot, float thr) -> unsigned long long {
         if (t >= cnt) return 0x7f8000007fffffffull;
         const float *q = reinterpret_cast<const float *>(m.leaves + leaf) + (t >> 1) * 48 + (t & 1);
         TriC tc;
         tc.a = mk3(q[0], q[2], q[4]); tc.b = mk3(q[6], q[8], q[10]); tc.ab = mk3(q[12], q[14], q[16]);
         tc.ac = mk3(q[18], q[20], q[22]); tc.bc = mk3(q[24], q[26], q[28]);
         tc.i00 = q[30]; tc.i11 = q[32]; tc.ibc = q[34]; tc.a00 = q[36]; tc.a01 = q[38]; tc.a11 = q[40]; tc.inn = q[42];
+        if (m.bounds) {
+            const float *gq = reinterpret_cast<const float *>(m.bounds + leaf) + (t >> 1) * (2 * kBoundFields) + (t & 1);
+            float g[kBoundFields];
+#pragma unroll
+            for (int k = 0; k < kBoundFields; ++k) g[k] = gq[2 * k];
+            const f3 ap = sub3(p, tc.a);
+            const float apv[3] = {ap.x, ap.y, ap.z};
+            if (tri_bound_lb(g, apv, dot3(tc.ab, ap)) > thr) return 0x7f8000007fffffffull;
+        }
         const float d2 = tri_dist2(p, tc);
         out_slot = leaf + t;
         return ((unsigned long long)(unsigned)__float_as_int(d2) << 32) | (unsigned)__float_as_int(q[44]);
@@ -537,7 +590,7 @@
     {
         const int code = ~cur, leaf = code >> 2, cnt = (code & 3) + 1;
         int sl = 0;
-        const unsigned long long k = tri_key(leaf, lane & 3, cnt, sl);
+        const unsigned long long k = tri_key(leaf, lane & 3, cnt, sl, INFINITY);
         wave_min(k, sl);
     }
     float thr = prune_threshold(__int_as_float((int)(key >> 32)));
@@ -553,7 +606,7 @@
             int sl = 0;
             if ((lane >> 2) < take) {
                 const int code = ~reinterpret_cast<volatile int *>(S.leaf_ref)[e];
-                if (reinterpret_cast<volatile float *>(S.leaf_d)[e] <= thr) k = tri_key(code >> 2, lane & 3, (code & 3) + 1, sl);
+                if (reinterpret_cast<volatile float *>(S.leaf_d)[e] <= thr) k = tri_key(code >> 2, lane & 3, (code & 3) + 1, sl, thr);
             }
             nl -= take;
             const unsigned long long before = key;
diff --git a/icon_amd/csrc/mesh_build.cpp b/icon_amd/csrc/mesh_build.cpp
--- a/icon_amd/csrc/mesh_build.cpp
+++ b/icon_amd/csrc/mesh_build.cpp
@@ -220,6 +220,7 @@
     std::vector<float> vn;
     std::vector<BvhNode> nodes;
     std::vector<LeafRec> leafrec;
+    std::vector<LeafBound> leafbound;
     std::vector<TriRec> tris;
     std::vector<TriAttr> attr;
     std::vector<int32_t> order, face2slot, bin_start, bin_slots;
@@ -274,8 +275,10 @@
     std::vector<TriAttr> &attr = out.attr;
     std::vector<int32_t> &face2slot = out.face2slot;
     std::vector<LeafRec> &leafrec = out.leafrec;
-    tris.resize(F); attr.resize(F); face2slot.resize(F); leafrec.resize(F);
+    std::vector<LeafBound> &leafbound = out.leafbound;
+    tris.resize(F); attr.resize(F); face2slot.resize(F); leafrec.resize(F); leafbound.resize(F);
     memset((void *)leafrec.data(), 0, sizeof(LeafRec) * F);
+    memset((void *)leafbound.data(), 0, sizeof(LeafBound) * F);
     for (int64_t p = 0; p < F; ++p) {
         const int64_t f = order[p];
         const int64_t id[3] = {faces[3 * f], faces[3 * f + 1], faces[3 * f + 2]};
@@ -298,6 +301,9 @@
             tri_setup(tris[p].a, tris[p].b, tris[p].c, order[p], pre);
             const float *src = reinterpret_cast<const float *>(&pre);
             for (int fld = 0; fld < 24; ++fld) leafrec[L].pair[t >> 1][fld][t & 1] = src[fld];
+            float g[kBoundFields];
+            tri_bound_setup(pre, g);
+            for (int fld = 0; fld < kBoundFields; ++fld) leafbound[L].pair[t >> 1][fld][t & 1] = g[fld];
         }
     }
 
@@ -347,6 +353,7 @@
     if ((rc = put_fn(Ly.dyn, dynv.data(), sizeof(MeshDyn))) || (rc = put_fn(Ly.vnormals, h.vn.data(), h.vn.size() * 4)) ||
         (rc = put_fn(Ly.nodes, h.nodes.data(), h.nodes.size() * sizeof(BvhNode))) ||
         (rc = put_fn(Ly.leaves, h.leafrec.data(), h.leafrec.size() * sizeof(LeafRec))) ||
+        (rc = put_fn(Ly.bounds, h.leafbound.data(), h.leafbound.size() * sizeof(LeafBound))) ||
         (rc = put_fn(Ly.tris, h.tris.data(), h.tris.size() * sizeof(TriRec))) || (rc = put_fn(Ly.attr, h.attr.data(), h.attr.size() * sizeof(TriAttr))) ||
         (rc = put_fn(Ly.slot2face, h.order.data(), h.order.size() * 4)) || (rc = put_fn(Ly.face2slot, h.face2slot.data(), h.face2slot.size() * 4)) ||
         (rc = put_fn(Ly.bin_start, h.bin_start.data(), h.bin_start.size() * 4)) || (rc = put_fn(Ly.bin_slots, h.bin_slots.data(), h.bin_slots.size() * 4)))
@@ -512,6 +519,26 @@
     return emit_arena(h, Ly, [&](size_t off, const void *src, size_t bytes) -> int { if (bytes) memcpy(ar + off, src, bytes); return ICON_OK; });
 }
 
+extern "C" int icon_debug_tri_bound(const float *h_tris, int64_t n, const float *h_pts, int64_t m, float *h_recs, float *h_lb)
+{
+    ICON_ARG(h_tris && (h_pts || m == 0) && n >= 0 && m >= 0, "icon_debug_tri_bound: bad argument");
+    for (int64_t i = 0; i < n; ++i) {
+        const float *t = h_tris + 9 * i;
+        TriPre pre;
+        tri_setup(t, t + 3, t + 6, 0, pre);
+        float g[kBoundFields];
+        tri_bound_setup(pre, g);
+        if (h_recs) memcpy(h_recs + kBoundFields * i, g, sizeof(g));
+        if (!h_lb) continue;
+        for (int64_t j = 0; j < m; ++j) {
+            const float *p = h_pts + 3 * j;
+            const float ap[3] = {p[0] - pre.a[0], p[1] - pre.a[1], p[2] - pre.a[2]};
+            h_lb[i * m + j] = tri_bound_lb(g, ap, dot3r(pre.ab, ap));
+        }
+    }
+    return ICON_OK;
+}
+
 extern "C" int icon_debug_mesh_layout(int64_t V, int64_t F, int64_t out[12])
 {
     ICON_ARG(out && V >= 3 && F >= 1 && F <= (1 << 23), "icon_debug_mesh_layout: bad argument");
diff --git a/icon_amd/csrc/mesh_device.hip b/icon_amd/csrc/mesh_device.hip
--- a/icon_amd/csrc/mesh_device.hip
+++ b/icon_amd/csrc/mesh_device.hip
@@ -16,7 +16,7 @@
     int32_t V, F, bound;
     MeshDyn *dyn; BuildHdr *hdr;
     int32_t *valence; uint8_t *leaf_cnt; BTask *tasks; uint32_t *hist; int32_t *cell_count, *cell_cursor;
-    float *vnormals; BvhNode *nodes; LeafRec *leaves; TriRec *tris; TriAttr *attr; int32_t *slot2face, *face2slot;
+    float *vnormals; BvhNode *nodes; LeafRec *leaves; LeafBound *bounds; TriRec *tris; TriAttr *attr; int32_t *slot2face, *face2slot;
     int32_t *bin_start, *bin_slots;
     float *tbox, *cen; int32_t *order[2]; int32_t *adj; int32_t *chunkcnt; int32_t *subq; struct STask *sublist; uint32_t *bounds_part;
     int32_t nck; int64_t cells_cap, entries_cap;
@@ -626,8 +626,13 @@
     const float *src = reinterpret_cast<const float *>(&pre);
     LeafRec &lr = c.leaves[leaf];
     const int tend = (myt == cnt - 1) ? kLeafMax : myt + 1;
-    for (int t = myt; t < tend; ++t)
+    float gb[kBoundFields];
+    tri_bound_setup(pre, gb);
+    LeafBound &lb = c.bounds[leaf];
+    for (int t = myt; t < tend; ++t) {
         for (int fld = 0; fld < 24; ++fld) lr.pair[t >> 1][fld][t & 1] = src[fld];
+        for (int fld = 0; fld < kBoundFields; ++fld) lb.pair[t >> 1][fld][t & 1] = gb[fld];
+    }
     const BinGrid g = grid_of(c);
     int cy0, cy1, cz0, cz1;
     cell_range(g, c.tbox + 6 * (size_t)f, cy0, cy1, cz0, cz1);
@@ -792,6 +797,7 @@
     d.slot2face = reinterpret_cast<const int32_t *>(b + L.slot2face);
     d.face2slot = reinterpret_cast<const int32_t *>(b + L.face2slot);
     d.leaves = reinterpret_cast<const LeafRec *>(b + L.leaves);
+    d.bounds = reinterpret_cast<const LeafBound *>(b + L.bounds);
     d.dyn = m->d_dyn;
     d.n_tris = (int32_t)m->F;
     d.bin_start = reinterpret_cast<const int32_t *>(b + L.bin_start);
@@ -810,7 +816,7 @@
     c.tasks = reinterpret_cast<BTask *>(b + L.tasks); c.hist = reinterpret_cast<uint32_t *>(b + L.hist);
     c.cell_count = reinterpret_cast<int32_t *>(b + L.cell_count); c.cell_cursor = reinterpret_cast<int32_t *>(b + L.cell_cursor);
     c.vnormals = reinterpret_cast<float *>(b + L.vnormals); c.nodes = reinterpret_cast<BvhNode *>(b + L.nodes);
-    c.leaves = reinterpret_cast<LeafRec *>(b + L.leaves); c.tris = reinterpret_cast<TriRec *>(b + L.tris);
+    c.leaves = reinterpret_cast<LeafRec *>(b + L.leaves); c.bounds = reinterpret_cast<LeafBound *>(b + L.bounds); c.tris = reinterpret_cast<TriRec *>(b + L.tris);
     c.attr = reinterpret_cast<TriAttr *>(b + L.attr); c.slot2face = reinterpret_cast<int32_t *>(b + L.slot2face);
     c.face2slot = reinterpret_cast<int32_t *>(b + L.face2slot); c.bin_start = reinterpret_cast<int32_t *>(b + L.bin_start);
     c.bin_slots = reinterpret_cast<int32_t *>(b + L.bin_slots); c.tbox = reinterpret_cast<float *>(b + L.tbox);
diff --git a/icon_amd/csrc/mesh_rules.h b/icon_amd/csrc/mesh_rules.h
--- a/icon_amd/csrc/mesh_rules.h
+++ b/icon_amd/csrc/mesh_rules.h
@@ -68,6 +68,50 @@
     t.face = face; t.pad = 0;
 }
 
+constexpr double kBoundShrink = 1.0 - 0x1p-17;
+constexpr double kBoundPad = 0x1p-20;
+__host__ __device__ inline void tri_bound_setup(const TriPre &t, float *g )
+{
+    const double abx = t.ab[0], aby = t.ab[1], abz = t.ab[2], acx = t.ac[0], acy = t.ac[1], acz = t.ac[2];
+    const double nx = aby * acz - abz * acy, ny = abz * acx - abx * acz, nz = abx * acy - aby * acx;
+    const float nnf = (float)(nx * nx + ny * ny + nz * nz);
+    const bool ok = t.a00 > 1e-30f && t.a00 < 1e30f && t.a11 < 1e30f && nnf > 1e-30f && nnf < 1e30f && t.inn == t.inn;
+    if (!ok) {
+        for (int k = 0; k < 7; ++k) g[k] = 0.0f;
+        g[7] = -__builtin_inff(); g[8] = __builtin_inff(); g[9] = -__builtin_inff(); g[10] = __builtin_inff(); g[11] = __builtin_inff();
+        return;
+    }
+    const double sn = (double)(1.0f / sqrtf(nnf)) * kBoundShrink;
+    const float inv_ab = 1.0f / sqrtf(t.a00);
+    const float nh[3] = {(float)(nx * sn), (float)(ny * sn), (float)(nz * sn)};
+    const double n0 = nh[0], n1 = nh[1], n2 = nh[2], ia = (double)inv_ab;
+    const float th[3] = {(float)((n1 * abz - n2 * aby) * ia), (float)((n2 * abx - n0 * abz) * ia), (float)((n0 * aby - n1 * abx) * ia)};
+    const double t0 = th[0], t1 = th[1], t2 = th[2];
+    const double m = (double)sqrtf(t.a00 > t.a11 ? t.a00 : t.a11);
+    const double pad = kBoundPad * m, pad_u = pad * (double)sqrtf(t.a00);
+    const double u_b = abx * abx + aby * aby + abz * abz, u_c = abx * acx + aby * acy + abz * acz;
+    const double v_b = t0 * abx + t1 * aby + t2 * abz, v_c = t0 * acx + t1 * acy + t2 * acz;
+    const double w_b = n0 * abx + n1 * aby + n2 * abz, w_c = n0 * acx + n1 * acy + n2 * acz;
+    const double aw_b = w_b < 0.0 ? -w_b : w_b, aw_c = w_c < 0.0 ? -w_c : w_c;
+    g[0] = nh[0]; g[1] = nh[1]; g[2] = nh[2]; g[3] = th[0]; g[4] = th[1]; g[5] = th[2];
+    g[6] = (float)(ia * kBoundShrink);
+    g[7] = (float)((u_c < 0.0 ? u_c : 0.0) - pad_u);
+    g[8] = (float)((u_c > u_b ? u_c : u_b) + pad_u);
+    g[9] = (float)((v_b < v_c ? (v_b < 0.0 ? v_b : 0.0) : (v_c < 0.0 ? v_c : 0.0)) - pad);
+    g[10] = (float)((v_b > v_c ? (v_b > 0.0 ? v_b : 0.0) : (v_c > 0.0 ? v_c : 0.0)) + pad);
+    g[11] = (float)((aw_b > aw_c ? aw_b : aw_c) + pad);
+}
+
+__host__ __device__ inline float tri_bound_lb(const float *g, const float *ap, float d1)
+{
+    const float w = fmaf(g[2], ap[2], fmaf(g[1], ap[1], g[0] * ap[0]));
+    const float v = fmaf(g[5], ap[2], fmaf(g[4], ap[1], g[3] * ap[0]));
+    const float eu = fmaxf(fmaxf(g[7] - d1, d1 - g[8]), 0.0f) * g[6];
+    const float ev = fmaxf(fmaxf(g[9] - v, v - g[10]), 0.0f);
+    const float ew = fmaxf(fmaxf(w - g[11], -(w + g[11])), 0.0f);
+    return fmaf(ew, ew, fmaf(ev, ev, eu * eu));
+}
+
 constexpr int kTopLevels = 7;
 constexpr int kSubMax = 256;
 constexpr int kChunk = 256;
@@ -89,7 +133,7 @@
 
 struct MeshLayout {
     size_t dyn, hdr, valence, leaf_cnt, tasks, hist, cell_count, cell_cursor, zero_end;
-    size_t vnormals, nodes, leaves, tris, attr, slot2face, face2slot, bin_start, bin_slots;
+    size_t vnormals, nodes, leaves, bounds, tris, attr, slot2face, face2slot, bin_start, bin_slots;
     size_t tbox, cen, order0, order1, adj, chunkcnt, subq, sublist, bounds_part, total;
     int64_t nck;
 };
@@ -113,6 +157,7 @@
     L.vnormals = take(sizeof(float) * 3 * V);
     L.nodes = take(sizeof(BvhNode) * F);
     L.leaves = take(sizeof(LeafRec) * F);
+    L.bounds = take(sizeof(LeafBound) * F);
     L.tris = take(sizeof(TriRec) * F);
     L.attr = take(sizeof(TriAttr) * F);
     L.slot2face = take(sizeof(int32_t) * F);
diff --git a/icon_amd/csrc/query_kernels.hip b/icon_amd/csrc/query_kernels.hip
--- a/icon_amd/csrc/query_kernels.hip
+++ b/icon_amd/csrc/query_kernels.hip
@@ -233,10 +233,10 @@
     const bool live = lattice_point(L, ix, iy, iz);
     lattice_clamp(L, ix, iy, iz, cx, cy, cz);
     const f3 p = lattice_world(L.res, cx, cy, cz + L.z0);
-    int nn = 0, nt = 0;
-    Nearest nr = nearest_packet<true>(m, p, live, lds + (threadIdx.x >> 6) * kStackDepth, &nn, &nt);
+    int nn = 0, nt = 0, np = 0;
+    Nearest nr = nearest_packet<true>(m, p, live, lds + (threadIdx.x >> 6) * kStackDepth, &nn, &nt, INFINITY, nullptr, 21, false, 0, &np);
     if (seeded) {
-        nn = 0; nt = 0;
+        nn = 0; nt = 0; np = 0;
         float thr0 = prune_threshold(nr.d2);
         if (seeded == 2) {
             const float dc = sqrtf(__int_as_float(__builtin_amdgcn_readlane(__float_as_int(nr.d2), 21)));
@@ -246,15 +246,17 @@
         }
         if (seeded == 3) {
             const float h = 2.0f / (float)(L.res - 1);
-            int na = 0, nb = 0;
-            const Nearest pv = nearest_packet<true>(m, mk3(p.x - 4.0f * h, p.y, p.z), live, lds + (threadIdx.x >> 6) * kStackDepth, &na, &nb);
+            int na = 0, nb = 0, nc = 0;
+            const Nearest pv = nearest_packet<true>(m, mk3(p.x - 4.0f * h, p.y, p.z), live, lds + (threadIdx.x >> 6) * kStackDepth, &na, &nb,
+                                                    INFINITY, nullptr, 21, false, 0, &nc);
             const float dn = sqrtf(pv.d2) + 4.0001f * h;
             thr0 = prune_threshold(dn * dn);
         }
-        nr = nearest_packet<true>(m, p, live, lds + (threadIdx.x >> 6) * kStackDepth, &nn, &nt, thr0);
+        nr = nearest_packet<true>(m, p, live, lds + (threadIdx.x >> 6) * kStackDepth, &nn, &nt, thr0, nullptr, 21, false, 0, &np);
     }
     if ((threadIdx.x & 63) == 0) {
         atomicAdd(&out[0], 1ull); atomicAdd(&out[1], (unsigned long long)nn); atomicAdd(&out[2], (unsigned long long)nt);
+        atomicAdd(&out[5], (unsigned long long)np);
     }
     if (live && nr.slot < 0) atomicAdd(&out[3], 1ull);
     if ((threadIdx.x & 63) == 0) atomicMax(&out[4], (unsigned long long)(nn + nt));
@@ -543,19 +545,19 @@
     ICON_ARG(nb < (1ll << 31), "icon_sdf_query: N too large for one launch");
     hipStream_t st = (hipStream_t)stream;
     if (search == ICON_SEARCH_BRUTE) {
-        hipLaunchKernelGGL(k_sdf_query<true>, dim3((unsigned)nb), dim3(kBlock), 0, st, mesh->dev, d_points, N, d_sdf, d_norm,
+        hipLaunchKernelGGL(k_sdf_query<true>, dim3((unsigned)nb), dim3(kBlock), 0, st, mesh_dev(mesh), d_points, N, d_sdf, d_norm,
                            d_cmap, d_vis, d_face, d_inside, nullptr);
     } else if (N < kPacketMinPoints) {
         const int cap = coop_cap(mesh->depth_bound);
         hipLaunchKernelGGL(k_sdf_query_coop, dim3((unsigned)((N + kCoopWaves - 1) / kCoopWaves)), dim3(kCoopWaves * 64), kCoopWaves * coop_wave_bytes(cap), st,
-                           mesh->dev, d_points, N, d_sdf, d_norm, d_cmap, d_vis, d_face, d_inside, cap);
+                           mesh_dev(mesh), d_points, N, d_sdf, d_norm, d_cmap, d_vis, d_face, d_inside, cap);
     } else {
         icon_work tmp;
         static const float ident[12] = {1, 0, 0, 0, 0, 1, 0, 0, 0, 0, 1, 0};
         const int32_t *perm = nullptr;
         int rc = morton_order(&tmp, d_points, ident, nullptr, N, st, &perm);
         if (!rc) {
-            hipLaunchKernelGGL(k_sdf_query<false>, dim3((unsigned)nb), dim3(kBlock), 0, st, mesh->dev, d_points, N, d_sdf, d_norm,
+            hipLaunchKernelGGL(k_sdf_query<false>, dim3((unsigned)nb), dim3(kBlock), 0, st, mesh_dev(mesh), d_points, N, d_sdf, d_norm,
                                d_cmap, d_vis, d_face, d_inside, perm);
             if (hipGetLastError() != hipSuccess || hipStreamSynchronize(st) != hipSuccess) rc = fail(ICON_ERR_HIP, "icon_sdf_query: launch failed");
         }
@@ -794,6 +796,12 @@
 int g_share_ring = 0, g_share_lose = 0, g_share_spin_log2 = 0;
 int g_lattice_fast = -1;
 int g_share_waves = -2;
+int g_tri_prefilter = -1;
+int tri_prefilter()
+{
+    if (g_tri_prefilter < 0) g_tri_prefilter = getenv("ICON_AMD_TRI_PREFILTER") ? (atoi(getenv("ICON_AMD_TRI_PREFILTER")) != 0) : 1;
+    return g_tri_prefilter;
+}
 int share_waves_override()
 {
     if (g_share_waves == -2) g_share_waves = getenv("ICON_AMD_SHARE") ? atoi(getenv("ICON_AMD_SHARE")) : -1;
@@ -921,10 +929,10 @@
             lf = work->d_lfast;
         }
         if (rows <= 20000)
-            hipLaunchKernelGGL(k_row_crossings_wide, dim3((unsigned)((rows * 16 + kBlock - 1) / kBlock)), dim3(kBlock), 0, st, mesh->dev, L,
+            hipLaunchKernelGGL(k_row_crossings_wide, dim3((unsigned)((rows * 16 + kBlock - 1) / kBlock)), dim3(kBlock), 0, st, mesh_dev(mesh), L,
                                work->d_row_count, work->d_row_slots, lf);
         else
-            hipLaunchKernelGGL(k_row_crossings, dim3((unsigned)((rows + kBlock - 1) / kBlock)), dim3(kBlock), 0, st, mesh->dev, L,
+            hipLaunchKernelGGL(k_row_crossings, dim3((unsigned)((rows + kBlock - 1) / kBlock)), dim3(kBlock), 0, st, mesh_dev(mesh), L,
                                work->d_row_count, work->d_row_slots, lf);
     }
     int64_t nb;
@@ -942,7 +950,7 @@
     if (!LATTICE && !alt && mode != 3 && (N < kPacketMinPoints || mode == 2)) {
         const int cap = coop_cap(mesh->depth_bound);
         hipLaunchKernelGGL(k_nearest_coop, dim3((unsigned)((N + kCoopWaves - 1) / kCoopWaves)), dim3(kCoopWaves * 64),
-                           kCoopWaves * coop_wave_bytes(cap), st, mesh->dev, cal, d_points, N, near, cap, sdf_clip);
+                           kCoopWaves * coop_wave_bytes(cap), st, mesh_dev(mesh), cal, d_points, N, near, cap, sdf_clip);
     } else if (nb > 0) {
         if (!LATTICE) {
             const int rc = morton_order(work, d_points, cal.m, cal.d, N, st, &perm);
@@ -953,10 +961,10 @@
         ShareDbg dbg{};
         if (nw > 1) { const int rc = work_share_dbg(work, &dbg); if (rc) return rc; }
         if (work->prof) (void)hipEventRecord(work->ev[4], st);
-        if (nw == 16) hipLaunchKernelGGL(k_nearest_shared<16>, dim3((unsigned)nb * 4), dim3(16 * 64), 0, st, mesh->dev, L, near, sdf_clip, dbg);
-        else if (nw == 8) hipLaunchKernelGGL(k_nearest_shared<8>, dim3((unsigned)nb * 4), dim3(8 * 64), 0, st, mesh->dev, L, near, sdf_clip, dbg);
-        else if (alt) hipLaunchKernelGGL((k_nearest<LATTICE, true>), dim3((unsigned)nb), dim3(kBlock), 0, st, mesh->dev, cal, L, d_points, N, near, perm, sdf_clip, work->tie_ulps, lf);
-        else hipLaunchKernelGGL((k_nearest<LATTICE, false>), dim3((unsigned)nb), dim3(kBlock), 0, st, mesh->dev, cal, L, d_points, N, near, perm, sdf_clip, 0, lf);
+        if (nw == 16) hipLaunchKernelGGL(k_nearest_shared<16>, dim3((unsigned)nb * 4), dim3(16 * 64), 0, st, mesh_dev(mesh), L, near, sdf_clip, dbg);
+        else if (nw == 8) hipLaunchKernelGGL(k_nearest_shared<8>, dim3((unsigned)nb * 4), dim3(8 * 64), 0, st, mesh_dev(mesh), L, near, sdf_clip, dbg);
+        else if (alt) hipLaunchKernelGGL((k_nearest<LATTICE, true>), dim3((unsigned)nb), dim3(kBlock), 0, st, mesh_dev(mesh), cal, L, d_points, N, near, perm, sdf_clip, work->tie_ulps, lf);
+        else hipLaunchKernelGGL((k_nearest<LATTICE, false>), dim3((unsigned)nb), dim3(kBlock), 0, st, mesh_dev(mesh), cal, L, d_points, N, near, perm, sdf_clip, 0, lf);
         if (work->prof) { (void)hipEventRecord(work->ev[5], st); work->ev_search = true; }
     }
     ICON_HIP(hipGetLastError());
@@ -981,7 +989,7 @@
     if (LATTICE) nb = (int64_t)Lf.tx * Lf.ty * Lf.tz; else nb = (N + kBlock - 1) / kBlock;
     ICON_ARG(nb > 0 && nb < (1ll << 31), "too many workgroups for one launch");
     const dim3 grid((unsigned)nb), block(kBlock);
-    const MeshDev md = mesh ? mesh->dev : MeshDev{};
+    const MeshDev md = mesh ? mesh_dev(mesh) : MeshDev{};
     const int local = (cmap_mode == ICON_CMAP_LOCAL) ? 1 : 0;
     const bool brute = (search == ICON_SEARCH_BRUTE);
 #define ICON_LAUNCH(P, B) hipLaunchKernelGGL((k_features<P, LATTICE, B>), grid, block, 0, st, md, feat->dev, cal, Lf, d_points, N, sdf_clip, local, work->d_row_count, work->d_row_slots, work_near(work, mesh), work->d_x, work->d_code8, skip_shell)
@@ -1373,7 +1381,7 @@
     return copy_rows_out(work, d_rows, st);
 }
 
-extern "C" int icon_debug_traversal_stats(const icon_mesh_t *mesh, int res, int z0, int z1, uint64_t out[4])
+static int traversal_stats(const icon_mesh_t *mesh, int res, int z0, int z1, uint64_t *out, int n_out)
 {
     ICON_ARG(mesh && out, "icon_debug_traversal_stats: null argument");
     LatticeMap L;
@@ -1382,14 +1390,25 @@
     unsigned long long *d = nullptr;
     ICON_HIP(hipMalloc((void **)&d, 8 * sizeof(unsigned long long)));
     ICON_HIP(hipMemset(d, 0, 8 * sizeof(unsigned long long)));
-    hipLaunchKernelGGL(k_traversal_stats, dim3((unsigned)(L.tx * L.ty * L.tz)), dim3(kBlock), 0, 0, mesh->dev, L, d,
+    hipLaunchKernelGGL(k_traversal_stats, dim3((unsigned)(L.tx * L.ty * L.tz)), dim3(kBlock), 0, 0, mesh_dev(mesh), L, d,
                        getenv("ICON_AMD_STATS_SEEDED") ? atoi(getenv("ICON_AMD_STATS_SEEDED")) : 0);
     unsigned long long h[8];
     hipError_t e = hipMemcpy(h, d, sizeof(h), hipMemcpyDeviceToHost);
     (void)hipFree(d);
     if (e != hipSuccess) return fail(ICON_ERR_HIP, std::string("traversal stats: ") + hipGetErrorString(e));
     out[0] = h[0]; out[1] = h[1]; out[2] = h[2]; out[3] = h[4];
-    return ICON_OK;
+    if (n_out > 4) out[4] = h[5];
+    return ICON_OK;
+}
+
+extern "C" int icon_debug_traversal_stats(const icon_mesh_t *mesh, int res, int z0, int z1, uint64_t out[4])
+{
+    return traversal_stats(mesh, res, z0, z1, out, 4);
+}
+
+extern "C" int icon_debug_traversal_stats_ex(const icon_mesh_t *mesh, int res, int z0, int z1, uint64_t out[5])
+{
+    return traversal_stats(mesh, res, z0, z1, out, 5);
 }
 
 extern "C" int icon_grid_eval_slab(const icon_mesh_t *mesh, const icon_feat_t *feat, const icon_mlp_t *mlp,
@@ -1416,6 +1435,7 @@
     ICON_ARG(key != nullptr, "icon_debug_set_option: key is null");
     const std::string k(key);
     if (k == "lattice_fast") g_lattice_fast = value ? 1 : 0;
+    else if (k == "tri_prefilter") g_tri_prefilter = value ? 1 : 0;
     else if (k == "share_waves") { ICON_ARG(value == -1 || value == 1 || value == 4 || value == 8 || value == 16, "share_waves: -1 (by launch size), 1, 4, 8 or 16"); g_share_waves = value; }
     else if (k == "share_ring") { ICON_ARG(value == 0 || (value >= 2 && value <= 64 && (value & (value - 1)) == 0), "share_ring: 0 or a power of two in 2..64"); g_share_ring = value; }
     else if (k == "share_lose_push") { ICON_ARG(value >= 0, "share_lose_push: a ticket >= 1, or 0"); g_share_lose = value; }
@@ -1453,7 +1473,7 @@
     const int32_t *perm = nullptr;
     int rc = morton_order(&tmp, d_points, ident, nullptr, N, st, &perm);
     if (!rc) {
-        hipLaunchKernelGGL(k_nearest_ties, dim3((unsigned)nb), dim3(kBlock), 0, st, mesh->dev, d_points, N, perm, d_face, d_face2, d_ulps);
+        hipLaunchKernelGGL(k_nearest_ties, dim3((unsigned)nb), dim3(kBlock), 0, st, mesh_dev(mesh), d_points, N, perm, d_face, d_face2, d_ulps);
         if (hipGetLastError() != hipSuccess || hipStreamSynchronize(st) != hipSuccess) rc = fail(ICON_ERR_HIP, "icon_sdf_query_ties: launch failed");
     }
     (void)hipFree(tmp.d_sort_keys); (void)hipFree(tmp.d_sort_idx); (void)hipFree(tmp.d_sort_tmp);
diff --git a/icon_amd/engine.py b/icon_amd/engine.py
--- a/icon_amd/engine.py
+++ b/icon_amd/engine.py
@@ -99,11 +99,12 @@
         return dict(nodes=arr[0], depth=arr[1], bin_entries=arr[2], max_bin=arr[3], leaves=arr[4], slots=arr[5])
 
     def traversal_stats(self, res: int, z0: int = 0, z1: Optional[int] = None) -> dict:
-        arr = (C.c_uint64 * 4)()
-        check(_lib.lib().icon_debug_traversal_stats(self.h, C.c_int(res), C.c_int(z0), C.c_int(res if z1 is None else z1), arr),
-              "icon_debug_traversal_stats")
+        arr = (C.c_uint64 * 5)()
+        check(_lib.lib().icon_debug_traversal_stats_ex(self.h, C.c_int(res), C.c_int(z0), C.c_int(res if z1 is None else z1), arr),
+              "icon_debug_traversal_stats_ex")
         return dict(waves=arr[0], nodes=arr[1], tris=arr[2], nodes_per_wave=arr[1] / max(arr[0], 1),
-                    tris_per_wave=arr[2] / max(arr[0], 1), longest_walk=arr[3])
+                    tris_per_wave=arr[2] / max(arr[0], 1), longest_walk=arr[3],
+                    pairs=arr[4], pairs_per_wave=arr[4] / max(arr[0], 1))
 
     def sdf_query(self, points: torch.Tensor, search: str = "bvh"):
         p = _dev_f32(points, "points").reshape(-1, 3)
diff --git a/include/icon_amd.h b/include/icon_amd.h
--- a/include/icon_amd.h
+++ b/include/icon_amd.h
@@ -138,6 +138,7 @@
 int icon_debug_mesh_layout(int64_t V, int64_t F, int64_t out[12]);
 int icon_debug_host_mesh_build(const float *h_verts, int64_t V, const int64_t *h_faces, int64_t F,
                                const float *h_cmap, const float *h_vis, void *h_arena, int64_t arena_bytes);
+int icon_debug_tri_bound(const float *h_tris, int64_t n, const float *h_pts, int64_t m, float *h_recs, float *h_lb);
 int icon_debug_set_shell_skip(int on);
 int icon_debug_set_option(const char *key, int value);
 int icon_work_status(icon_work_t *work);
@@ -147,6 +148,7 @@
 int icon_work_set_tie_rule(icon_work_t *work, int rule, int ulps);
 
 int icon_debug_traversal_stats(const icon_mesh_t *mesh, int res, int z0, int z1, uint64_t out[4]);
+int icon_debug_traversal_stats_ex(const icon_mesh_t *mesh, int res, int z0, int z1, uint64_t out[5]);
 
 int icon_volume_any_above(const float *d_occ, int res, int sx, int sy, int sz, float level, icon_work_t *work, void *stream, int *h_any);
 
```

Measured after the change: 1.010 billion, median of 6. 1.2% higher.
